# JohnGoertz/Gumbi

Measured on AMD Instinct MI355X. Metric: fit+predict achieved GFLOP/s (fp64 exact GP: one MAP objective + gradient evaluation at the model's starting hyper-parameters + grid prediction), higher is better.
Workload: dtype f64; 1 GPU; synthetic N=50k d=8 Matern-5/2 ARD fp64, M=10^4 grid; N=50000, d=8, kernel=Matern52, M=10000, parallelism=1 GPU, warmup_step=the same step (untimed)

## Files before the change

gumbi_amd/csrc/engine.hip:

```cpp
#include <hip/hip_runtime.h>

#include <algorithm>
#include <cmath>
#include <cstdarg>
#include <cstdio>
#include <cstdlib>
#include <cstring>
#include <string>
#include <functional>
#include <unordered_map>
#include <mutex>
#include <memory>
#include <vector>

#include "../../include/gumbi_hip.h"
#include "covariance.hpp"
#include "gemm_f64.hpp"
#include "gradient.hpp"
#include "potrf_leaf.hpp"
#include "trsm_strip.hpp"
#include "chol_tiles.hpp"
#include "eval_tiles.hpp"
#include "predict_form.hpp"
#include "joint_predict.hpp"

using namespace gmb;

namespace {

constexpr int DIST_MAX_WORLD = 64;
constexpr int DIST_MAX_PAYLOAD = 7;
constexpr int DIST_HEADER = 3;

inline int64_t round_up(int64_t x, int64_t m) { return (x + m - 1) / m * m; }

enum EvKind : int {
  EV_CHOL_PANEL_GEMM = 0,
  EV_LEAF = 1,
  EV_CHOL_SOLVE_GEMM = 2,
  EV_PREDICT_GEMM = 3,
  EV_GRAD_GEMM = 4,
  EV_CHOL_STRIP = 5,
  EV_SOLVE_STRIP = 6,
  EV_CHOL_UPDATE = 7,
  EV_CHOL_TILES = 8,
  EV_EVAL_TILES = 9,
  EV_CHOL_TILES_PANEL = 10
};

struct EventPair {
  hipEvent_t a, b;
  EvKind kind;
  double flops;
  int mt, nt, k, flags;
  bool masked = false;
};

}

constexpr int GACC_REGION = 64 + MAX_TABS * GMB_MAX_LEVELS * GMB_MAX_LEVELS + 64;
constexpr int GACC_DOUBLES = (1 + GMB_MAX_COREG) * GACC_REGION;
constexpr int SCAL_INFO_AT = 64, SCAL_GACC_AT = 72, SCAL_DOUBLES = SCAL_GACC_AT + GACC_DOUBLES + 64;

struct FactorRef {
  double* A;
  int64_t ld;
  int64_t N, Np, Nr;
  double* dinv16;
  double* scal;
  uint32_t** ct;
  int64_t* cap_ct;
  int32_t* info() const { return reinterpret_cast<int32_t*>(scal + SCAL_INFO_AT); }
};

struct CholResult {
  bool tiles = false;
  bool traced = false;
  bool injected = false;
  int ntasks = 0;
};

struct gmb_engine {
  int device = 0;
  hipStream_t stream = nullptr;
  bool own_stream = false;
  std::string err;

  int64_t N = 0, Np = 0, Nr = 0, ld = 0;
  int32_t D = 0;
  double* dX = nullptr;
  double* dy = nullptr;
  double* dA = nullptr;
  double* dDinv16 = nullptr;
  int64_t cap_A = 0, cap_dinv16 = 0;

  gmb_kernel_spec spec{};
  bool have_spec = false, have_theta = false;
  std::vector<double> theta;
  int nc_pad = 1;
  int periodic = 0;
  double periods[8] = {};
  double* xs = nullptr;
  double* xl = nullptr;
  int32_t* cat = nullptr;
  int64_t cap_pts = 0;
  double* dtabs = nullptr;
  double* dnoise = nullptr;
  CovParams cp{};
  PrepArgs prep_proto{};
  struct Term {
    PrepArgs pa;
    CovParams cp;
    double eta;
    int n_tab_acc;
  };
  std::vector<Term> terms;
  std::vector<double> htabs;
  std::vector<double> hnoise;

  double* dscal = nullptr;
  int32_t* dinfo = nullptr;
  double* dv = nullptr;
  bool factored = false;
  enum { FK_NONE = 0, FK_SINGLE = 1, FK_REPLICATED = 2, FK_CAPACITY = 3 };
  int factor_kind = FK_NONE;
  bool factor_consumed = false;
  bool have_alpha = false;
  double* dDiagSave = nullptr;
  int64_t cap_diag = 0;
  int64_t notpd = -1;
  double logdet = 0.0, vnorm2 = 0.0;

  int64_t Mt_cap = 0;
  double* dV = nullptr;
  bool u_valid = false, linv_valid = false;
  int predict_form = -1;
  double* dV2 = nullptr;
  int64_t Mt2_cap = 0;
  JointState jt;
  double* dXs = nullptr;
  double* txs = nullptr;
  double* txl = nullptr;
  int32_t* tcat = nullptr;
  double* dkss = nullptr;
  double* dpart = nullptr;
  double* dmean = nullptr;
  double* dvar = nullptr;
  int64_t cap_part = 0;

  double* dW = nullptr;
  int64_t cap_W = 0;
  double* dalpha = nullptr;
  int64_t cap_pts_alpha = 0;
  double* dgpart = nullptr;
  int64_t cap_gpart = 0;
  double* dgred = nullptr;
  int64_t cap_gred = 0;
  double* dgbig = nullptr;
  int64_t cap_gbig = 0;

  struct InvLevelPlan {
    int variant[2] = {0, 0};
    int grid_x[2] = {0, 0};
    int count = 0;
    int64_t off[2] = {0, 0};
    int64_t toff = 0;
    int tr_rows = 0, tr_cols = 0;
    double flops[2] = {0.0, 0.0};
  };
  std::vector<InvLevelPlan> inv_plan;
  GemmArgs* dplan_gemm = nullptr;
  TransposeJob* dplan_tr = nullptr;
  int64_t plan_N = -1, plan_ld = -1, plan_Np = -1;
  const double* plan_W = nullptr;
  const double* plan_A = nullptr;
  bool batch_inverse = true;
  bool lpt_order = true;
  long long lpt_max_tiles = 16384;
  int cov_strip = 0;
  int tile_strip = 8;

  bool profiling = false;
  gmb_timings tm{};
  std::vector<EventPair> evs;
  bool naive_leaf = false;
  bool gemm_dma = true;
  bool small_tiles = true;
  int gemm_variant = 0;
  long long wg_slots = 512;
  bool force_variant = false;

  hipStream_t cur = nullptr;
  hipStream_t aux[3] = {nullptr, nullptr, nullptr};
  int chol_scheme = -1;
  uint32_t* dct = nullptr;
  int64_t cap_ct = 0;
  unsigned long long* dct_trace = nullptr;
  int64_t cap_ct_trace = 0;
  bool ct_trace = false;
  CholResult chol;
  bool tt_used = false;
  int ct_lose = 0;
  bool fact_in_flight = false;
  struct HostLanding {
    double scal[2];
    int32_t info;
    uint32_t abort;
    double gacc[GACC_DOUBLES];
  };
  HostLanding* hl = nullptr;
  HostLanding* hl_dev = nullptr;
  hipEvent_t fe[4] = {nullptr, nullptr, nullptr, nullptr};
  bool eval_call = false;
  bool light = false;
  bool gacc_zeroed = false;
  unsigned long long* prep_zero[2] = {nullptr, nullptr};
  int64_t prep_zero_words[2] = {0, 0};
  bool prezeroed = false;
  bool prep_deferred = false;
  int inline_prep_max_rows = 4096;
  bool fe_recorded = false;
  int grad_scheme = -1;
  int et_lag = -1;
  uint32_t* det_tasks = nullptr;
  int64_t cap_et_tasks = 0;
  int et_key[5] = {-1, -1, -1, -1, -1};
  int et_pairs = -1;
  int et_pairs_min_blocks = 72;
  int et_ntasks = 0;
  double* dUdiag = nullptr;
  int64_t cap_udiag = 0;
  double* dApart = nullptr;
  int64_t cap_apart = 0;
  bool et_fused = false;
  int et_min_blocks = 1;
  int panel_tiles_w = 16;
  bool panel_tiles_veto = false;
  int tiles_min_blocks = 6, tiles_max_blocks = 224;
  int tiles_trsm_min_blocks = 16;
  int masked_max_blocks = 128;
  std::vector<hipEvent_t> sync_pool;
  size_t sync_next = 0;
  bool lookahead = true;
  bool par_inverse = true;
  bool aux_shared = false;
  bool aux_borrowed = false;
  int part_cus = 0;
  double* dsend = nullptr;
  double* drecv = nullptr;
  int64_t cap_send = 0, cap_recv = 0;
  double* dsend2 = nullptr;
  double* drecv2 = nullptr;
  int64_t cap_send2 = 0, cap_recv2 = 0;
  int panel_blocks = 8;
  bool panel_auto = true;
  std::unordered_map<void*, size_t> allocs;
  int64_t bytes_resident = 0, bytes_peak = 0;
  int dist_mode = 0;
  double* dAown = nullptr;
  int64_t cap_Aown = 0;
  int64_t ld_own = 0;
  int own_world = -1, own_rank = -1;
  double* dPanel = nullptr;
  int64_t cap_panel = 0;
  std::function<int(double*, int64_t, int)> solve_hook;
  double* dstat = nullptr;
  uint64_t coll_count = 0, coll_hash = 0;
  std::vector<hipEvent_t> time_pool;
  size_t time_next = 0;
};

namespace {

int fail(gmb_engine* e, int code, const char* fmt, ...) {
  char buf[512];
  va_list ap;
  va_start(ap, fmt);
  vsnprintf(buf, sizeof buf, fmt, ap);
  va_end(ap);
  if (e) e->err = buf;
  return code;
}

#define HIP_TRY(e, call)                                                              \
  do {                                                                                \
    hipError_t _s = (call);                                                           \
    if (_s != hipSuccess)                                                             \
      return fail(e, GMB_EHIP, "%s failed: %s (%s:%d)", #call, hipGetErrorString(_s), \
                  __FILE__, __LINE__);                                                \
  } while (0)

void release(gmb_engine* e, void* p) {
  if (!p) return;
  if (e) {
    auto it = e->allocs.find(p);
    if (it != e->allocs.end()) {
      e->bytes_resident -= (int64_t)it->second;
      e->allocs.erase(it);
    }
  }
  (void)hipFree(p);
}

template <typename T>
int ensure(gmb_engine* e, T** p, int64_t* cap, int64_t need) {
  if (*cap >= need && *p) return GMB_OK;
  release(e, (void*)*p);
  *p = nullptr;
  *cap = 0;
  if (need < 1) need = 1;
  hipError_t s = hipMalloc((void**)p, (size_t)need * sizeof(T));
  if (s != hipSuccess)
    return fail(e, GMB_ENOMEM, "hipMalloc of %lld bytes failed: %s", (long long)(need * sizeof(T)),
                hipGetErrorString(s));
  *cap = need;
  if (e) {
    e->allocs[(void*)*p] = (size_t)need * sizeof(T);
    e->bytes_resident += (int64_t)((size_t)need * sizeof(T));
    e->bytes_peak = std::max(e->bytes_peak, e->bytes_resident);
  }
  return GMB_OK;
}

template <typename T>
int alloc(gmb_engine* e, T** p, int64_t need) {
  int64_t cap = 0;
  release(e, (void*)*p);
  *p = nullptr;
  return ensure(e, p, &cap, need);
}

int pick_nc(int n) { return n <= 1 ? 1 : n <= 2 ? 2 : n <= 4 ? 4 : n <= 8 ? 8 : 16; }

struct PhaseTimer {
  gmb_engine* e;
  hipEvent_t a = nullptr, b = nullptr;
  explicit PhaseTimer(gmb_engine* e_) : e(e_) {
    (void)hipEventCreate(&a);
    (void)hipEventCreate(&b);
    (void)hipEventRecord(a, e->stream);
  }
  void stop() { (void)hipEventRecord(b, e->stream); }
  double ms() {
    float t = 0.f;
    (void)hipEventElapsedTime(&t, a, b);
    return (double)t;
  }
  ~PhaseTimer() {
    (void)hipEventDestroy(a);
    (void)hipEventDestroy(b);
  }
};

void ev_begin(gmb_engine* e, EvKind kind, double flops, int mt = 0, int nt = 0, int k = 0, int flags = 0) {
  if (!e->profiling) return;
  EventPair p;
  p.mt = mt;
  p.nt = nt;
  p.k = k;
  p.flags = flags;
  (void)hipEventCreate(&p.a);
  (void)hipEventCreate(&p.b);
  p.kind = kind;
  p.flops = flops;
  p.masked = e->aux_shared && e->cur == e->aux[2];
  (void)hipEventRecord(p.a, e->cur);
  e->evs.push_back(p);
}
void ev_end(gmb_engine* e) {
  if (!e->profiling) return;
  (void)hipEventRecord(e->evs.back().b, e->cur);
}
void ev_collect(gmb_engine* e) {
  static FILE* trace = nullptr;
  if (!trace && !e->evs.empty()) {
    const char* path = getenv("GMB_TRACE_FILE");
    if (path && path[0]) trace = fopen(path, "a");
  }
  if (!e->evs.empty()) {
    auto interval_union = [&](auto pick) {
      std::vector<std::pair<float, float>> iv;
      for (auto& p : e->evs)
        if (pick(p.kind)) {
          float ta = 0.f, tb = 0.f;
          if (hipEventElapsedTime(&ta, e->evs[0].a, p.a) == hipSuccess && hipEventElapsedTime(&tb, e->evs[0].a, p.b) == hipSuccess)
            iv.emplace_back(ta, tb);
        }
      std::sort(iv.begin(), iv.end());
      float cur_lo = 0.f, cur_hi = -1.f;
      double uni = 0.0;
// ... 528 lines not shown
  if (c1 - c0 == 1) return chol_leaf(e, f, c0, rend);
  if (tile_panels && c1 - c0 <= e->panel_tiles_w) return chol_tiles_panel(e, f, c0, c1, rend, tile_panels);
  const int mid = c0 + (c1 - c0 + 1) / 2;
  int rc = chol_cols(e, f, c0, mid, rend, update_kind, tile_panels);
  if (rc) return rc;
  GemmArgs g{};
  g.C = f.A + (int64_t)mid * TILE + (int64_t)mid * TILE * f.ld;
  g.ldc = f.ld;
  g.A = f.A + (int64_t)mid * TILE + (int64_t)c0 * TILE * f.ld;
  g.lda = f.ld;
  g.B = g.A;
  g.ldb = f.ld;
  g.mt = c1 - mid;
  g.nt = rend - mid;
  g.k = (mid - c0) * TILE;
  g.alpha = -1.0;
  g.beta = 1.0;
  g.tri = 1;
  rc = launch_gemm(e, g, update_kind);
  if (rc) return rc;
  return chol_cols(e, f, mid, c1, rend, update_kind, tile_panels);
}

double ragged_row_frac(const FactorRef& f) {
  const int64_t rv = f.N + 1 - (f.Nr - TILE);
  return rv >= TILE ? 1.0 : (double)((rv + 15) / 16) / 8.0;
}
double ragged_col_frac(const FactorRef& f) {
  const int64_t cv = f.N - (f.Np - TILE);
  return cv >= TILE ? 1.0 : (double)((cv + 15) / 16) / 8.0;
}
double chol_tiles_flops(const FactorRef& f, int nct, int nrt, bool to_last_row = true) {
  const double fr = to_last_row ? ragged_row_frac(f) : 1.0;
  double flops = 0.0;
  for (int j = 1; j < nct; ++j) {
    const double tiles = nrt - 1 > j ? (double)(nrt - j - 1) + fr : (double)(nrt - j);
    flops += 2.0 * TILE * TILE * TILE * (double)j * tiles;
  }
  return flops;
}

CholTilesArgs tiles_args(const FactorRef& f, int c0, int nct, int nrt, int ntasks, bool chol = true) {
  uint32_t* ct = *f.ct;
  CholTilesArgs a{};
  a.A = f.A + (int64_t)c0 * TILE * (f.ld + 1);
  a.ld = f.ld;
  a.nct = nct;
  a.nrt = nrt;
  a.N = f.N - (int64_t)c0 * TILE;
  a.row_base = (int64_t)c0 * TILE;
  a.dinv16 = f.dinv16 + (int64_t)c0 * 8 * 256;
  a.ctl = ct;
  a.flags = ct + 4;
  if (chol) {
    a.logdet = f.scal;
    a.info = f.info();
    a.half = ct + 4 + (int64_t)nrt * nct;
    a.prog = a.half + 2 * (int64_t)nct;
  }
  a.ntasks = ntasks;
  a.timeout_us = 4000000u;
  return a;
}

int tiles_lose_tickets(gmb_engine* e, uint32_t* ctl, int lose) {
  const uint32_t first = (uint32_t)lose;
  HIP_TRY(e, hipMemcpyAsync(ctl, &first, sizeof first, hipMemcpyHostToDevice, e->cur));
  HIP_TRY(e, hipStreamSynchronize(e->cur));
  return GMB_OK;
}

int tiles_trace_buffer(gmb_engine* e, CholTilesArgs& a) {
  int rc;
  if ((rc = ensure(e, &e->dct_trace, &e->cap_ct_trace, 4 * (int64_t)a.ntasks))) return rc;
  HIP_TRY(e, hipMemsetAsync(e->dct_trace, 0, (size_t)a.ntasks * 4 * sizeof(unsigned long long), e->cur));
  a.dbg = e->dct_trace;
  return GMB_OK;
}

int chol_tiles(gmb_engine* e, const FactorRef& f, bool trace, int lose, CholResult* res) {
  const int nct = (int)(f.Np / TILE), nrt = (int)(f.Nr / TILE);
  const int ntasks = ct_task_count(nct, nrt);
  const int64_t words = 4 + (int64_t)nrt * nct + 3 * (int64_t)nct;
  int rc;
  if ((rc = ensure(e, f.ct, f.cap_ct, words))) return rc;
  HIP_TRY(e, hipMemsetAsync(*f.ct, 0, (size_t)words * sizeof(uint32_t), e->cur));
  res->injected = lose > 0;
  if (lose > 0 && (rc = tiles_lose_tickets(e, *f.ct, lose))) return rc;
  CholTilesArgs a = tiles_args(f, 0, nct, nrt, ntasks);
  res->traced = trace;
  if (trace && (rc = tiles_trace_buffer(e, a))) return rc;
  const double flops = chol_tiles_flops(f, nct, nrt);
  int nw = 8;
#ifdef GMB_TUNING
  if (const char* cw = getenv("GMB_CT_WAVES")) nw = atoi(cw) == 4 ? 4 : 8;
#endif
  int grid = (int)std::min<long long>(ntasks, nw == 8 ? e->wg_slots / 2 : e->wg_slots);
#ifdef GMB_TUNING
  if (const char* cg = getenv("GMB_CT_GRID")) grid = std::max(1, std::min(grid, atoi(cg)));
#endif
  ev_begin(e, EV_CHOL_TILES, flops, nct, nrt, (int)f.Np, 0);
  if (nw == 8) hipLaunchKernelGGL(chol_tiles_kernel<8>, dim3(grid), dim3(512), 0, e->cur, a);
  else hipLaunchKernelGGL(chol_tiles_kernel<4>, dim3(grid), dim3(256), 0, e->cur, a);
  ev_end(e);
  HIP_TRY(e, hipGetLastError());
  res->tiles = true;
  res->ntasks = ntasks;
  return GMB_OK;
}

int chol_tiles_panel(gmb_engine* e, const FactorRef& f, int c0, int c1, int rend, CholResult* res) {
  const int nct = c1 - c0, nrt = rend - c0;
  const int ntasks = ct_task_count(nct, nrt);
  const int64_t words = 4 + (int64_t)nrt * nct + 3 * (int64_t)nct;
  int rc;
  if ((rc = ensure(e, f.ct, f.cap_ct, std::max<int64_t>(words, 4 + (int64_t)(e->panel_tiles_w + 3) * (f.Nr / TILE))))) return rc;
  HIP_TRY(e, hipMemsetAsync(*f.ct, 0, sizeof(uint32_t), e->cur));
  HIP_TRY(e, hipMemsetAsync(*f.ct + 2, 0, (size_t)(words - 2) * sizeof(uint32_t), e->cur));
  const CholTilesArgs a = tiles_args(f, c0, nct, nrt, ntasks);
  const double flops = chol_tiles_flops(f, nct, nrt, rend == (int)(f.Nr / TILE));
  const int grid = (int)std::min<long long>(ntasks, e->wg_slots / 2);
  ev_begin(e, EV_CHOL_TILES_PANEL, flops, nct, nrt, nct * TILE, 0);
  hipLaunchKernelGGL(chol_tiles_kernel<8>, dim3(grid), dim3(512), 0, e->cur, a);
  ev_end(e);
  HIP_TRY(e, hipGetLastError());
  res->tiles = true;
  return GMB_OK;
}

int trsm_tiles(gmb_engine* e, const FactorRef& f, double* V, int64_t ldv, int ntm, EvKind ev_kind) {
  const int nct = (int)(f.Np / TILE);
  const long long ntasks = (long long)ntm * nct;
  if (ntasks <= 0) return GMB_OK;
  const int64_t words = 4 + (int64_t)ntm * nct;
  int rc;
  if ((rc = ensure(e, f.ct, f.cap_ct, words))) return rc;
  HIP_TRY(e, hipMemsetAsync(*f.ct, 0, (size_t)words * sizeof(uint32_t), e->cur));
  CholTilesArgs a = tiles_args(f, 0, nct, nct, (int)ntasks, false);
  a.V = V;
  a.ldv = ldv;
  a.ntm = ntm;
  double flops = 0.0;
  for (int c = 0; c < nct; ++c)
    flops += (double)ntm * (2.0 * TILE * TILE * TILE * c * (c == nct - 1 ? ragged_col_frac(f) : 1.0) + (double)TILE * TILE * TILE);
  const int grid = (int)std::min<long long>(ntasks, e->wg_slots / 2);
  ev_begin(e, ev_kind, flops, nct, ntm, (int)f.Np, 0);
  hipLaunchKernelGGL(trsm_tiles_kernel<8>, dim3(grid), dim3(512), 0, e->cur, a);
  ev_end(e);
  HIP_TRY(e, hipGetLastError());
  e->tt_used = true;
  return GMB_OK;
}

int grad_workspace(gmb_engine* e);
int64_t eval_tiles_words(int nct, int nrt) { return 4 + (int64_t)nrt * nct + 3 * (int64_t)nct + (int64_t)nct * nct + nct; }

bool eval_will_fuse(const gmb_engine* e) {
  const int nblocks = (int)(e->Np / TILE);
  return !e->naive_leaf && (e->chol_scheme == 3 || e->chol_scheme < 0) && e->grad_scheme != 0 && e->grad_scheme != 1 &&
         nblocks <= e->tiles_max_blocks && (e->grad_scheme == 2 ? nblocks >= 1 : nblocks >= e->et_min_blocks);
}

int eval_tiles(gmb_engine* e, bool with_chol) {
  const FactorRef f = train_factor(e);
  const int nct = (int)(e->Np / TILE), nrt = (int)(e->Nr / TILE);
  int rc;
  const int lag = e->et_lag >= 0 ? e->et_lag : std::max(2, std::min(24, nct / 4));
  int nw = 8;
#ifdef GMB_TUNING
  if (const char* cw = getenv("GMB_ET_WAVES")) nw = atoi(cw) == 4 ? 4 : 8;
#endif
  const int pairs = (nw == 8 && !e->ct_trace && (e->et_pairs > 0 || (e->et_pairs < 0 && nct >= e->et_pairs_min_blocks))) ? 1 : 0;
  if (e->et_key[0] != nct || e->et_key[1] != nrt || e->et_key[2] != (int)with_chol || e->et_key[3] != lag || e->et_key[4] != pairs) {
    std::vector<uint32_t> list;
    et_build_tasks(nct, nrt, with_chol, lag, list, pairs != 0);
    if ((rc = ensure(e, &e->det_tasks, &e->cap_et_tasks, (int64_t)list.size()))) return rc;
    HIP_TRY(e, hipMemcpy(e->det_tasks, list.data(), list.size() * sizeof(uint32_t), hipMemcpyHostToDevice));
    e->et_key[0] = nct;
    e->et_key[1] = nrt;
    e->et_key[2] = (int)with_chol;
    e->et_key[3] = lag;
    e->et_key[4] = pairs;
    e->et_ntasks = (int)list.size();
  }
  const int ntasks = e->et_ntasks;
  const int64_t chol_words = (int64_t)nrt * nct + 3 * (int64_t)nct;
  const int64_t words = eval_tiles_words(nct, nrt);
  if ((rc = ensure(e, &e->dct, &e->cap_ct, words + 2))) return rc;
  if ((rc = ensure(e, &e->dW, &e->cap_W, e->Np * e->Np))) return rc;
  e->u_valid = e->linv_valid = false;
  if ((rc = ensure(e, &e->dUdiag, &e->cap_udiag, (int64_t)nct * TILE * TILE))) return rc;
  if ((rc = ensure(e, &e->dApart, &e->cap_apart, (int64_t)nct * nct * TILE + nct))) return rc;
  if ((rc = grad_workspace(e))) return rc;
  if (!(with_chol && e->prezeroed)) HIP_TRY(e, hipMemsetAsync(e->dct, 0, (size_t)words * sizeof(uint32_t), e->cur));
  if (!with_chol) HIP_TRY(e, hipMemsetAsync(e->dct + 4, 1, (size_t)nrt * nct * sizeof(uint32_t), e->cur));
  const int lose = with_chol ? e->ct_lose : 0;
  e->chol.injected = lose > 0;
  if (lose > 0) {
    e->ct_lose = 0;
    if ((rc = tiles_lose_tickets(e, e->dct, lose))) return rc;
  }
  CholTilesArgs a = tiles_args(f, 0, nct, nrt, ntasks);
  e->chol.traced = e->ct_trace;
  if (e->ct_trace && (rc = tiles_trace_buffer(e, a))) return rc;
  EvalTilesArgs x{};
  x.tasks = e->det_tasks;
  x.ntasks = ntasks;
  x.uflags = e->dct + 4 + chol_words;
  x.udiag = e->dUdiag;
  x.Z = e->dW;
  x.ldz = e->Np;
  x.apart = e->dApart;
  x.yb = (int)(e->N / TILE);
  x.rowdone = x.uflags + (int64_t)nct * nct;
  x.alpha = e->dalpha;
  x.v = e->dv;
  x.vpart = e->dApart + (int64_t)nct * nct * TILE;
  x.scal = e->dscal + 1;
  x.with_v = with_chol ? 1 : 0;
  double flops = with_chol ? chol_tiles_flops(f, nct, nrt) : 0.0;
  for (int c = 0; c < nct; ++c)
    flops += 2.0 * TILE * TILE * TILE * 0.5 * (double)c * (double)(c + 1) * (c == nct - 1 ? ragged_col_frac(f) : 1.0);
  for (int I = 0; I < nct; ++I) flops += 2.0 * TILE * TILE * TILE * (double)(nct - I) * (double)(I + 1);
  const int grid = (int)std::min<long long>(ntasks, nw == 8 ? e->wg_slots / 2 : e->wg_slots);
  ev_begin(e, EV_EVAL_TILES, flops, nct, nrt, (int)e->Np, with_chol ? 1 : 0);
  if (nw == 8) hipLaunchKernelGGL(eval_tiles_kernel<8>, dim3(grid), dim3(512), 0, e->cur, a, x);
#ifdef GMB_TUNING
  else hipLaunchKernelGGL(eval_tiles_kernel<4>, dim3(grid), dim3(256), 0, e->cur, a, x);
#endif
  ev_end(e);
  HIP_TRY(e, hipGetLastError());
  e->chol.tiles = true;
  e->chol.ntasks = ntasks;
  return GMB_OK;
}

hipEvent_t next_sync_event(gmb_engine* e) {
  if (e->sync_next == e->sync_pool.size()) {
    hipEvent_t ev = nullptr;
    (void)hipEventCreateWithFlags(&ev, hipEventDisableTiming);
    e->sync_pool.push_back(ev);
  }
  return e->sync_pool[e->sync_next++];
}
hipEvent_t next_time_event(gmb_engine* e) {
  if (e->time_next == e->time_pool.size()) {
    hipEvent_t ev = nullptr;
    (void)hipEventCreate(&ev);
    e->time_pool.push_back(ev);
  }
  return e->time_pool[e->time_next++];
}
int order_after(gmb_engine* e, hipStream_t from, hipStream_t to) {
  if (from == to) return GMB_OK;
  hipEvent_t ev = next_sync_event(e);
  HIP_TRY(e, hipEventRecord(ev, from));
  HIP_TRY(e, hipStreamWaitEvent(to, ev, 0));
  return GMB_OK;
}

int chol_lookahead_masked(gmb_engine* e, const FactorRef& f) {
  const int nct = (int)(f.Np / TILE), nrt = (int)(f.Nr / TILE);
  const int w = e->panel_blocks;
  hipStream_t mainS = e->stream, bulkS = e->aux[2];
  e->sync_next = 0;
  int rc;
  e->cur = mainS;
  if ((rc = chol_cols(e, f, 0, std::min(w, nct), nrt, EV_CHOL_PANEL_GEMM))) return rc;
  for (int c0 = 0; c0 < nct; c0 += w) {
    const int c1 = std::min(c0 + w, nct);
    const int n0 = c1, n1 = std::min(c1 + w, nct);
    if (n0 >= nct) break;
    auto update = [&](int col_lo, int col_hi) {
      GemmArgs g{};
      g.C = f.A + (int64_t)col_lo * TILE + (int64_t)col_lo * TILE * f.ld;
      g.ldc = f.ld;
      g.A = f.A + (int64_t)col_lo * TILE + (int64_t)c0 * TILE * f.ld;
      g.lda = f.ld;
      g.B = g.A;
      g.ldb = f.ld;
      g.mt = col_hi - col_lo;
      g.nt = nrt - col_lo;
      g.k = (c1 - c0) * TILE;
      g.alpha = -1.0;
      g.beta = 1.0;
      g.tri = 1;
      return launch_gemm(e, g, EV_CHOL_UPDATE);
    };
    e->cur = mainS;
    if ((rc = order_after(e, bulkS, mainS))) return rc;
    if ((rc = update(n0, n1))) return rc;
    if ((rc = order_after(e, mainS, bulkS))) return rc;
    e->cur = bulkS;
    rc = (n1 < nct) ? update(n1, nct) : 0;
    e->cur = mainS;
    if (rc) return rc;
    if ((rc = chol_cols(e, f, n0, n1, nrt, EV_CHOL_PANEL_GEMM))) return rc;
  }
  e->cur = mainS;
  return order_after(e, bulkS, mainS);
}

struct CholOpts {
  bool masked_ok = false;
  bool trace = false;
  int lose = 0;
};

int chol_factor(gmb_engine* e, const FactorRef& f, const CholOpts& o, CholResult* res) {
  const int nblocks = (int)(f.Np / TILE), nrt = (int)(f.Nr / TILE);
  const bool tiles = !e->naive_leaf && (e->chol_scheme == 3 || (e->chol_scheme < 0 && nblocks >= e->tiles_min_blocks &&
                                                                 nblocks <= e->tiles_max_blocks));
  const bool masked = o.masked_ok && !tiles && e->lookahead && e->aux_shared && nblocks > e->panel_blocks &&
                      (e->chol_scheme == 2 || (e->chol_scheme < 0 && nblocks <= e->masked_max_blocks));
  e->cur = e->stream;
  if (tiles) return chol_tiles(e, f, o.trace, o.lose, res);
  if (masked) return chol_lookahead_masked(e, f);
  const bool tile_panels = !e->naive_leaf && !e->panel_tiles_veto && e->panel_tiles_w >= 2 && e->chol_scheme != 0;
  if (tile_panels) {
    int rc;
    if ((rc = ensure(e, f.ct, f.cap_ct, 4 + (int64_t)(e->panel_tiles_w + 3) * nrt))) return rc;
    HIP_TRY(e, hipMemsetAsync(*f.ct, 0, 4 * sizeof(uint32_t), e->stream));
  }
  return chol_cols(e, f, 0, nblocks, nrt, EV_CHOL_UPDATE, tile_panels ? res : nullptr);
}

int trsm_cols(gmb_engine* e, const FactorRef& f, double* V, int64_t ldz, int ntm, int c0, int c1, EvKind kind_gemm, EvKind kind_strip,
              int lfirst = -1, int lstride = 0) {
  if (c1 - c0 == 1)
    return launch_trsm_strip(e, V + (int64_t)c0 * TILE * ldz, ldz, (int64_t)ntm * TILE,
                             f.A + (int64_t)c0 * TILE * (f.ld + 1), f.ld, f.dinv16 + (int64_t)c0 * 8 * 256,
                             (int)std::min<int64_t>(TILE, f.N - (int64_t)c0 * TILE), kind_strip);
  const int mid = c0 + (c1 - c0 + 1) / 2;
  int rc = trsm_cols(e, f, V, ldz, ntm, c0, mid, kind_gemm, kind_strip, lfirst, lstride);
  if (rc) return rc;
  GemmArgs g{};
  g.C = V + (int64_t)mid * TILE * ldz;
  g.ldc = ldz;
  g.A = f.A + (int64_t)mid * TILE + (int64_t)c0 * TILE * f.ld;
  g.lda = f.ld;
  g.B = V + (int64_t)c0 * TILE * ldz;
  g.ldb = ldz;
  g.mt = c1 - mid;
  g.nt = ntm;
  g.k = (mid - c0) * TILE;
  g.alpha = -1.0;
  g.beta = 1.0;
  if (lstride > 0) {
    g.klo_n = 1;
    g.krow_stride = lstride;
    g.krow_off = (lfirst - c0) * TILE;
  }
  rc = launch_gemm(e, g, kind_gemm);
  if (rc) return rc;
  return trsm_cols(e, f, V, ldz, ntm, mid, c1, kind_gemm, kind_strip, lfirst, lstride);
}

int launch_transpose(gmb_engine* e, const double* src, int64_t lds_, double* dst, int64_t ldd, int rows,
                     int cols) {
  hipLaunchKernelGGL(transpose_kernel, dim3((rows + 31) / 32, (cols + 31) / 32), dim3(256), 0, e->cur, src,
                     lds_, dst, ldd, rows, cols);
  HIP_TRY(e, hipGetLastError());
  return GMB_OK;
}

int winv_node(gmb_engine* e, int c0, int c1, bool recurse);

int winv_cols(gmb_engine* e, int c0, int c1) { return winv_node(e, c0, c1, true); }

struct InvNode {
  int c0, c1;
};
void collect_inv_nodes(int c0, int c1, int depth, std::vector<std::vector<InvNode>>& levels) {
  if ((int)levels.size() <= depth) levels.resize(depth + 1);
  levels[depth].push_back(InvNode{c0, c1});
  if (c1 - c0 > 1) {
    const int mid = c0 + (c1 - c0 + 1) / 2;
    collect_inv_nodes(c0, mid, depth + 1, levels);
    collect_inv_nodes(mid, c1, depth + 1, levels);
  }
}
int build_inv_plan(gmb_engine* e, const std::vector<std::vector<InvNode>>& levels);
int winv_level_batched(gmb_engine* e, const gmb_engine::InvLevelPlan& lp);

int winv_levels(gmb_engine* e, int nt) {
  std::vector<std::vector<InvNode>> levels;
  collect_inv_nodes(0, nt, 0, levels);
  hipStream_t streams[4] = {e->stream, e->aux[0], e->aux[1], e->aux_shared ? e->aux[0] : e->aux[2]};
  if (nt <= 64) streams[1] = streams[2] = streams[3] = e->stream;
  int rc;
  for (int a = 1; a < 4; ++a)
    if ((rc = order_after(e, streams[0], streams[a]))) return rc;
  const bool batched = e->batch_inverse && build_inv_plan(e, levels) == GMB_OK;
  bool aux_behind = false;
  for (int depth = (int)levels.size() - 1; depth >= 0; --depth) {
    if (batched && e->inv_plan[depth].count > 0) {
      e->cur = e->stream;
      if ((rc = winv_level_batched(e, e->inv_plan[depth]))) return rc;
      aux_behind = true;
      continue;
    }
    if (aux_behind) {
      for (int a = 1; a < 4; ++a)
        if ((rc = order_after(e, streams[0], streams[a]))) return rc;
      aux_behind = false;
    }
    int idx = 0;
    for (const InvNode& nd : levels[depth]) {
      e->cur = streams[levels[depth].size() > 1 ? (idx++ & 3) : 0];
      if ((rc = winv_node(e, nd.c0, nd.c1, false))) {
        e->cur = e->stream;
        return rc;
      }
    }
    e->cur = e->stream;
    for (int a = 1; a < 4; ++a)
      if ((rc = order_after(e, streams[a], streams[0]))) return rc;
    if (depth > 0)
      for (int a = 1; a < 4; ++a)
        if ((rc = order_after(e, streams[0], streams[a]))) return rc;
  }
  return GMB_OK;
}

void winv_node_products(gmb_engine* e, int c0, int c1, GemmArgs& gt, GemmArgs& gw, TransposeJob& tr) {
  const int64_t ldw = e->Np, lda = e->ld;
  double* W = e->dW;
  double* A = e->dA;
  const int mid = c0 + (c1 - c0 + 1) / 2;
  const int n1 = mid - c0, n2 = c1 - mid;
  gt = GemmArgs{};
  gt.C = W + (int64_t)c0 * TILE + (int64_t)mid * TILE * ldw;
  gt.ldc = ldw;
  gt.A = A + (int64_t)mid * TILE + (int64_t)c0 * TILE * lda;
  gt.lda = lda;
  gt.B = A + (int64_t)c0 * TILE + (int64_t)c0 * TILE * lda;
  gt.ldb = lda;
  gt.mt = n2;
  gt.nt = n1;
  gt.k = n1 * TILE;
  gt.klo_n = 1;
  gt.alpha = 1.0;
  gt.beta = 0.0;
  gt.nblk_stride = 1;
  gw = GemmArgs{};
  gw.C = W + (int64_t)mid * TILE + (int64_t)c0 * TILE * ldw;
  gw.ldc = ldw;
  gw.A = W + (int64_t)c0 * TILE + (int64_t)mid * TILE * ldw;
  gw.lda = ldw;
  gw.B = W + (int64_t)mid * TILE + (int64_t)mid * TILE * ldw;
  gw.ldb = ldw;
  gw.mt = n1;
  gw.nt = n2;
  gw.k = n2 * TILE;
  gw.khi_n = 1;
  gw.alpha = -1.0;
  gw.beta = 0.0;
  gw.nblk_stride = 1;
  tr.src = W + (int64_t)mid * TILE + (int64_t)c0 * TILE * ldw;
  tr.dst = A + (int64_t)c0 * TILE + (int64_t)mid * TILE * lda;
  tr.rows = n2 * TILE;
  tr.cols = n1 * TILE;
}

int winv_node(gmb_engine* e, int c0, int c1, bool recurse) {
  if (c1 - c0 == 1) return GMB_OK;
  const int mid = c0 + (c1 - c0 + 1) / 2;
  int rc;
  if (recurse) {
    if ((rc = winv_node(e, c0, mid, true))) return rc;
    if ((rc = winv_node(e, mid, c1, true))) return rc;
  }
  GemmArgs gt, gw;
  TransposeJob tr;
  winv_node_products(e, c0, c1, gt, gw, tr);
  if ((rc = launch_gemm(e, gt, EV_GRAD_GEMM))) return rc;
  if ((rc = launch_gemm(e, gw, EV_GRAD_GEMM))) return rc;
  return launch_transpose(e, tr.src, e->Np, tr.dst, e->ld, tr.rows, tr.cols);
}

constexpr int MIN_BATCH_NODES = 4;

int build_inv_plan(gmb_engine* e, const std::vector<std::vector<InvNode>>& levels) {
  if (e->plan_N == e->N && e->plan_ld == e->ld && e->plan_Np == e->Np && e->plan_W == e->dW && e->plan_A == e->dA)
    return GMB_OK;
  std::vector<GemmArgs> hg;
  std::vector<TransposeJob> ht;
  e->inv_plan.assign(levels.size(), gmb_engine::InvLevelPlan{});
  static const int BMs[3] = {128, 64, 128}, BNs[3] = {128, 64, 64};
  static const double rate[3] = {73.0, 63.0, 65.0};
  static const int per128[3] = {1, 4, 2};
  for (size_t depth = 0; depth < levels.size(); ++depth) {
    std::vector<InvNode> nodes;
    for (const InvNode& nd : levels[depth])
      if (nd.c1 - nd.c0 > 1) nodes.push_back(nd);
    if ((int)nodes.size() < MIN_BATCH_NODES) continue;
    gmb_engine::InvLevelPlan& lp = e->inv_plan[depth];
    lp.count = (int)nodes.size();
    std::vector<GemmArgs> gs[2];
    lp.toff = (int64_t)ht.size();
    for (const InvNode& nd : nodes) {
      GemmArgs gt, gw;
      TransposeJob tr;
      winv_node_products(e, nd.c0, nd.c1, gt, gw, tr);
      gs[0].push_back(gt);
      gs[1].push_back(gw);
      ht.push_back(tr);
      lp.tr_rows = std::max(lp.tr_rows, tr.rows);
      lp.tr_cols = std::max(lp.tr_cols, tr.cols);
    }
    for (int b = 0; b < 2; ++b) {
      long long nact = 0;
      for (const GemmArgs& g : gs[b]) nact += gemm_nact128(g);
      int variant = 0;
      double best = 0.0;
      for (int v = 0; v < 3; ++v) {
        const double t = (double)(nact * per128[v]);
        const double sc = rate[v] * per128[v] / std::max(1.0, t / (double)e->wg_slots + 0.5);
        if (sc > best) {
          best = sc;
          variant = v;
        }
      }
      lp.variant[b] = variant;
      lp.off[b] = (int64_t)hg.size();
      for (GemmArgs g : gs[b]) {
        g.mt = g.mt * TILE / BMs[variant];
        g.nt = g.nt * TILE / BNs[variant];
        g.order = e->lpt_order ? (b == 0 ? 1 : 2) : 0;
        double fl = 0.0;
        const int nb = gemm_schedule(g, BMs[variant], BNs[variant], &fl);
            lp.grid_x[b] = std::max(lp.grid_x[b], nb);
        lp.flops[b] += fl;
        hg.push_back(g);
      }
    }
  }
  if (e->dplan_gemm) (void)hipFree(e->dplan_gemm);
  if (e->dplan_tr) (void)hipFree(e->dplan_tr);
  e->dplan_gemm = nullptr;
  e->dplan_tr = nullptr;
  e->plan_N = -1;
  if (!hg.empty()) {
    HIP_TRY(e, hipMalloc((void**)&e->dplan_gemm, hg.size() * sizeof(GemmArgs)));
    HIP_TRY(e, hipMalloc((void**)&e->dplan_tr, ht.size() * sizeof(TransposeJob)));
    HIP_TRY(e, hipMemcpy(e->dplan_gemm, hg.data(), hg.size() * sizeof(GemmArgs), hipMemcpyHostToDevice));
    HIP_TRY(e, hipMemcpy(e->dplan_tr, ht.data(), ht.size() * sizeof(TransposeJob), hipMemcpyHostToDevice));
  }
  e->plan_N = e->N;
  e->plan_ld = e->ld;
  e->plan_Np = e->Np;
  e->plan_W = e->dW;
  e->plan_A = e->dA;
  return GMB_OK;
}

int winv_level_batched(gmb_engine* e, const gmb_engine::InvLevelPlan& lp) {
  for (int b = 0; b < 2; ++b) {
    if (lp.grid_x[b] <= 0) continue;
    const GemmArgs* batch = e->dplan_gemm + lp.off[b];
    const dim3 grid(lp.grid_x[b], lp.count);
    ev_begin(e, EV_GRAD_GEMM, lp.flops[b], lp.count, 0, 0, (lp.variant[b] << 8) | 64);
    switch (lp.variant[b]) {
      case 0: hipLaunchKernelGGL((gemm_f64_batched_kernel<2, 2, 4, 4, 2>), grid, dim3(256), 0, e->cur, batch); break;
      case 1: hipLaunchKernelGGL((gemm_f64_batched_kernel<2, 2, 2, 2, 2>), grid, dim3(256), 0, e->cur, batch); break;
      default: hipLaunchKernelGGL((gemm_f64_batched_kernel<2, 2, 4, 2, 2>), grid, dim3(256), 0, e->cur, batch); break;
    }
    ev_end(e);
    HIP_TRY(e, hipGetLastError());
  }
  hipLaunchKernelGGL(transpose_batched_kernel, dim3((lp.tr_rows + 31) / 32, (lp.tr_cols + 31) / 32, lp.count),
                     dim3(256), 0, e->cur, e->dplan_tr + lp.toff, e->Np, e->ld);
  HIP_TRY(e, hipGetLastError());
  return GMB_OK;
}

template <int KIND>
int launch_grad_nc(gmb_engine* e, const GradArgs& a_in, int nblocks) {
  const dim3 grid(nblocks), block(256);
  const size_t lds = grad_lds_bytes(e->nc_pad, a_in.p.n_lin, a_in.p.n_tab);
  GradArgs a = a_in;
  a.part_block0 = 0;
  const int gs = a.gsplit > 1 ? a.gsplit : 1;
  const dim3 grid0((a.split ? a.general_tiles : nblocks) * gs);
  switch (e->nc_pad) {
    case 1: hipLaunchKernelGGL((grad_tile_kernel<KIND, 1>), grid0, block, lds, e->stream, a); break;
    case 2: hipLaunchKernelGGL((grad_tile_kernel<KIND, 2>), grid0, block, lds, e->stream, a); break;
    case 4: hipLaunchKernelGGL((grad_tile_kernel<KIND, 4>), grid0, block, lds, e->stream, a); break;
    case 8: hipLaunchKernelGGL((grad_tile_kernel<KIND, 8>), grid0, block, lds, e->stream, a); break;
    default: hipLaunchKernelGGL((grad_tile_kernel<KIND, 16>), grid0, block, lds, e->stream, a); break;
  }
  if constexpr (KIND <= 2) {
    if (a.split) {
      a.part_block0 = a.general_tiles * gs;
      switch (e->nc_pad) {
        case 1: hipLaunchKernelGGL((grad_interior_kernel<KIND, 1>), grid, block, 0, e->stream, a); break;
        case 2: hipLaunchKernelGGL((grad_interior_kernel<KIND, 2>), grid, block, 0, e->stream, a); break;
        case 4: hipLaunchKernelGGL((grad_interior_kernel<KIND, 4>), grid, block, 0, e->stream, a); break;
        case 8: hipLaunchKernelGGL((grad_interior_kernel<KIND, 8>), grid, block, 0, e->stream, a); break;
        default: hipLaunchKernelGGL((grad_interior_kernel<KIND, 16>), grid, block, 0, e->stream, a); break;
      }
    }
  }
  HIP_TRY(e, hipGetLastError());
  return GMB_OK;
}

int grad_workspace(gmb_engine* e) {
  int rc;
  if (e->cap_pts_alpha < 3 * e->Np) {
    if ((rc = alloc(e, &e->dalpha, 3 * e->Np))) return rc;
    e->cap_pts_alpha = 3 * e->Np;
  }
  return GMB_OK;
}

int grad_sigma_inv_rows(gmb_engine* e, int shard, int nshards, double* Z, int64_t ldz, bool packed) {
  const int nt = (int)(e->Np / TILE);
  const int owned = shard < nt ? (nt - shard + nshards - 1) / nshards : 0;
  GemmArgs g{};
  g.C = packed ? Z : Z + (int64_t)shard * TILE;
  g.ldc = ldz;
  g.A = e->dA;
  g.lda = e->ld;
  g.B = e->dA + (int64_t)shard * TILE;
  g.ldb = e->ld;
  g.mt = nt;
  g.nt = owned;
  g.k = (int)e->Np;
  g.klo_n = 1;
  g.krow_off = shard * TILE;
  g.tri = 1;
  g.tri_off = shard * TILE;
  g.nblk_stride = nshards;
  g.cblk_stride = packed ? 1 : 0;
  g.alpha = 1.0;
  g.beta = 0.0;
  return launch_gemm(e, g, EV_GRAD_GEMM);
}

int grad_reduce(gmb_engine* e, int shard, int nshards, const double* Z, int64_t ldz, bool packed,
                std::vector<double>& h) {
  const gmb_kernel_spec& s = e->spec;
  const int nt = (int)(e->Np / TILE);
  int rc;
  if (!e->gacc_zeroed) HIP_TRY(e, hipMemsetAsync(e->dgpart, 0, (GACC_DOUBLES + 64) * sizeof(double), e->stream));
  e->gacc_zeroed = false;
  const int n_ls = s.ard ? s.n_cont : 1;
  long long total = 0;
  for (int i = shard; i < nt; i += nshards) total += i + 1;
  const long long want = std::max<long long>(1, 3 * e->wg_slots);
  const int per = (int)std::max<long long>(1, (total + want - 1) / want);
  const int grid = (int)((total + per - 1) / per);
  const int ncp = e->nc_pad;
  bool merged = false;
  GradFinishArgs fin{};
  for (size_t t = 0; t < e->terms.size(); ++t) {
    const gmb_engine::Term& tr = e->terms[t];
    if (t > 0 && (rc = prep_points(e, e->dX, e->N, e->D, e->Nr, e->xs, e->xl, e->cat, &tr.pa))) return rc;
    GradArgs a{};
    a.p = tr.cp;
    a.pts = train_set(e);
    a.Z = Z;
    a.ldz = ldz;
    a.z_packed = packed ? 1 : 0;
    a.alpha = e->dalpha;
    a.tiles = nt;
    a.ard = s.ard;
    const int ncols = e->periodic ? 2 * s.n_cont : s.n_cont;
    const double true_inv = e->periodic == 2 ? 2.0 : 1.0;
    a.nc_real = ncols;
    for (int k = 0; k < 16; ++k) a.inv_ls[k] = k < ncols ? true_inv * tr.pa.inv_ls[k] : 0.0;
    a.eta = tr.eta;
    a.row_first = shard;
    a.row_stride = nshards;
    a.total_tiles = total;
    a.per = per;
    const int n_small = ncp + 2 + tr.cp.n_lin;
    a.part_stride = n_small + tr.cp.n_tab * 64;
    double* acc = e->dgpart + (int64_t)t * GACC_REGION;
    int tab_acc_off[MAX_TABS] = {0};
    int off = 64, big = 0;
    for (int j = 0; j < tr.cp.n_tab; ++j) {
      tab_acc_off[j] = off;
      const int LL = tr.cp.tab_levels[j] * tr.cp.tab_levels[j];
      off += LL;
      a.big_off[j] = big;
      if (tr.cp.tab_levels[j] > 8) big += LL;
    }
    a.big_stride = big;
    a.split = (tr.cp.kind == GMB_EXPQUAD || tr.cp.kind == GMB_MATERN52 || tr.cp.kind == GMB_MATERN32) && tr.cp.n_lin == 0 &&
                      tr.cp.n_tab == 0 && !e->naive_leaf
                  ? 1 : 0;
    a.n_owned_rows = shard < nt ? (nt - shard + nshards - 1) / nshards : 0;
    const bool last_ragged_owned = e->Np > e->N && (nt - 1 - shard) % nshards == 0 && nt - 1 >= shard;
    a.general_tiles = a.n_owned_rows + (last_ragged_owned ? nt - 1 : 0);
    if (a.general_tiles == 0) a.split = 0;
    if (total <= 128) a.split = 0;
    const int ndirect = a.split ? a.general_tiles : grid;
    a.gsplit = ndirect <= 512 ? 4 : 1;
    const int nvec = a.split ? ndirect * a.gsplit + grid : ndirect * a.gsplit;
    if (grid > 0) {
      if ((rc = ensure(e, &e->dgred, &e->cap_gred, (int64_t)nvec * a.part_stride))) return rc;
      a.part = e->dgred;
      if (big > 0) {
        if ((rc = ensure(e, &e->dgbig, &e->cap_gbig, (int64_t)ndirect * a.gsplit * 4 * big))) return rc;
        HIP_TRY(e, hipMemsetAsync(e->dgbig, 0, (size_t)ndirect * a.gsplit * 4 * big * sizeof(double), e->stream));
        a.big = e->dgbig;
      }
      switch (tr.cp.kind) {
        case GMB_EXPQUAD: rc = launch_grad_nc<0>(e, a, grid); break;
        case GMB_MATERN52: rc = launch_grad_nc<1>(e, a, grid); break;
        case GMB_MATERN32: rc = launch_grad_nc<2>(e, a, grid); break;
        case GMB_MATERN12: rc = launch_grad_nc<3>(e, a, grid); break;
        default: rc = launch_grad_nc<4>(e, a, grid); break;
      }
      if (rc) return rc;
      GradRanges r{};
      auto add = [&](int dense, int count, int dst) {
        r.dense[r.n] = dense;
        r.count[r.n] = count;
        r.dst[r.n] = dst;
        ++r.n;
      };
      double* tmp = e->dgpart + GACC_DOUBLES;
      merged = e->light && e->terms.size() == 1 && s.ard && !e->periodic && big == 0 && nvec <= 8192 && e->N <= 16384;
// ... 238 lines not shown
    const bool is_out = (j == s.n_coreg);
    const int L = is_out ? s.n_out : s.coreg_levels[j];
    std::vector<double> G((size_t)L * L, 0.0);
    if (!s.additive) {
      const double* src = table_slot(0, j);
      for (int i = 0; i < L * L; ++i) G[i] = src[i];
    } else if (!is_out) {
      const double* src = table_slot(1 + j, 0);
      for (int i = 0; i < L * L; ++i) G[i] = src[i];
    } else {
      for (size_t t = 0; t < e->terms.size(); ++t) {
        const double* src = table_slot(t, e->terms[t].cp.n_tab - 1);
        for (int i = 0; i < L * L; ++i) G[i] += src[i];
      }
    }
    table_grad(G, L, th + k, grad + k);
    k += 3 * L;
  }
  int diag_off = 64;
  for (int j = 0; j < e->terms[0].cp.n_tab; ++j) diag_off += e->terms[0].cp.tab_levels[j] * e->terms[0].cp.tab_levels[j];
  const double* hd = region(0) + diag_off;
  grad[i_sigma] = hd[0];
  if (s.out_col >= 0 && s.hetero_noise) {
    const int P = s.n_out;
    const double* W = th + k;
    for (int x = 0; x < P; ++x) {
      const double gd = hd[1 + x];
      grad[k + 2 * x] = 2.0 * gd * W[2 * x];
      grad[k + 2 * x + 1] = 2.0 * gd * W[2 * x + 1];
      grad[k + 2 * P + x] = gd;
    }
    k += 3 * P;
  }
  if (s.additive)
    for (int j = 0; j < s.n_coreg; ++j) {
      k += kernel_block(1 + j, grad + k);
      if (s.n_lin > 0) {
        for (int i = 0; i < s.n_lin; ++i) grad[k++] = region(1 + j)[n_ls + 2 + i];
        grad[k++] = region(1 + j)[n_ls + 1];
      }
    }
  if (k != (int)e->theta.size()) return fail(e, GMB_EINVAL, "internal: gradient packing mismatch");
  return GMB_OK;
}

inline bool chol_scheme_valid(int s) { return s == -1 || s == 0 || s == 2 || s == 3 || s == 4; }

int require_ready(gmb_engine* e, bool need_factor) {
  if (!e) return GMB_EINVAL;
  if (e->N <= 0) return fail(e, GMB_EINVAL, "gmb_set_data has not been called");
  if (!e->have_spec) return fail(e, GMB_EINVAL, "gmb_set_kernel has not been called");
  if (!e->have_theta) return fail(e, GMB_EINVAL, "gmb_set_theta has not been called");
  if (need_factor && !e->factored)
    return fail(e, GMB_EINVAL, "no valid factorisation: call gmb_factorize first");
  return GMB_OK;
}

int require_full_factor(gmb_engine* e, const char* what) {
  if (e->factor_kind == gmb_engine::FK_CAPACITY || !e->dA || e->cap_A <= 0)
    return fail(e, GMB_EINVAL, "%s needs the complete factor on this device, but the resident factorisation is a capacity-mode one "
                               "(gmb_dist_set_mode(e, 1): no rank holds the factor) -- use the gmb_dist_* calls, or gmb_factorize first", what);
  return GMB_OK;
}

int require_capacity_factor(gmb_engine* e, const char* what) {
  if (e->factor_kind != gmb_engine::FK_CAPACITY || !e->dAown)
    return fail(e, GMB_EINVAL, "%s in capacity mode needs a factorisation made by gmb_dist_factorize in capacity mode; the resident "
                               "one was made by %s", what, e->factor_kind == gmb_engine::FK_SINGLE ? "gmb_factorize / gmb_evaluate" : "the replicated multi-GPU driver");
  return GMB_OK;
}

}

namespace {

hipStream_t shared_masked_stream(int device, int part_cus, int* ncu_out) {
  static std::mutex mu;
  static hipStream_t streams[64] = {};
  static int ncus[64] = {};
  std::lock_guard<std::mutex> lock(mu);
  hipStream_t& st = streams[device & 63];
  if (!st) {
    hipDeviceProp_t prop;
    if (hipGetDeviceProperties(&prop, device) != hipSuccess) return nullptr;
    const int ncu = prop.multiProcessorCount;
    std::vector<uint32_t> mask((ncu + 31) / 32, 0u);
    for (int i = part_cus; i < ncu; ++i) mask[i / 32] |= 1u << (i % 32);
    if (hipExtStreamCreateWithCUMask(&st, (uint32_t)mask.size(), mask.data()) != hipSuccess) {
      st = nullptr;
      (void)hipGetLastError();
      return nullptr;
    }
    ncus[device & 63] = ncu;
  }
  if (ncu_out) *ncu_out = ncus[device & 63];
  return st;
}

int gmb_create_impl(gmb_engine** out, int32_t device, void* stream, const gmb_engine* peer = nullptr) {
  if (!out) return GMB_EINVAL;
  *out = nullptr;
  int n = gmb_device_count();
  if (n < 0) return GMB_ENODEVICE;
  if (device < 0 || device >= n) return GMB_EINVAL;
  if (hipSetDevice(device) != hipSuccess) return GMB_EHIP;
  gmb_engine* e = new gmb_engine();
  e->device = device;
  if (stream) {
    e->stream = (hipStream_t)stream;
  } else {
    if (hipStreamCreateWithFlags(&e->stream, hipStreamNonBlocking) != hipSuccess) {
      delete e;
      return GMB_EHIP;
    }
    e->own_stream = true;
  }
  auto flag = [](const char* name, bool dflt) {
    const char* v = getenv(name);
    return v && v[0] ? v[0] != '0' : dflt;
  };
  e->naive_leaf = flag("GMB_LEAF_NAIVE", false);
  e->gemm_dma = flag("GMB_GEMM_DMA", true);
  const char* cs = getenv("GMB_CHOL_SCHEME");
  if (cs && cs[0]) {
    const int v = atoi(cs);
    if (chol_scheme_valid(v)) e->chol_scheme = v;
    else fprintf(stderr, "[gumbi_hip] GMB_CHOL_SCHEME=%s ignored: valid schemes are -1 (by size), 0, 2, 3, 4\n", cs);
  }
  int part = 32;
#ifdef GMB_TUNING
  e->small_tiles = flag("GMB_SMALL_TILES", true);
  const char* gv = getenv("GMB_GEMM_VARIANT");
  if (gv && gv[0] >= '0' && gv[0] <= '4') {
    e->gemm_variant = gv[0] - '0';
    e->force_variant = true;
  }
  e->lookahead = flag("GMB_LOOKAHEAD", true);
  e->lpt_order = flag("GMB_LPT_ORDER", true);
  if (const char* lm = getenv("GMB_LPT_MAX_TILES")) e->lpt_max_tiles = atoll(lm);
  const char* ts = getenv("GMB_TILE_STRIP");
  if (ts) e->tile_strip = std::max(0, atoi(ts));
  const char* cst = getenv("GMB_COV_STRIP");
  if (cst) e->cov_strip = std::max(0, std::min(64, atoi(cst)));
  e->batch_inverse = flag("GMB_BATCH_INVERSE", true);
  e->par_inverse = flag("GMB_PAR_INVERSE", true);
  const char* pb = getenv("GMB_PANEL_BLOCKS");
  if (pb && atoi(pb) > 0) {
    e->panel_blocks = atoi(pb);
    e->panel_auto = false;
  }
  const char* mb = getenv("GMB_MASKED_MAX_BLOCKS");
  if (mb) e->masked_max_blocks = atoi(mb);
  if (const char* pw = getenv("GMB_PANEL_TILES_W")) e->panel_tiles_w = std::max(0, std::min(64, atoi(pw)));
  const char* pc = getenv("GMB_PART_CUS");
  if (pc) part = atoi(pc);
#endif
  e->cur = e->stream;
  int prio_lo = 0, prio_hi = 0;
  (void)hipDeviceGetStreamPriorityRange(&prio_lo, &prio_hi);
  for (int a = 0; a < 3 && peer; ++a) {
    e->aux[a] = peer->aux[a];
    e->aux_borrowed = true;
    e->aux_shared = peer->aux_shared;
    e->part_cus = peer->part_cus;
  }
  for (int a = 0; a < 3 && !peer; ++a) {
    hipError_t st2 = hipSuccess;
    int ncu = 0;
    hipStream_t masked = (a == 2 && part > 0) ? shared_masked_stream(device, part, &ncu) : nullptr;
    if (masked) {
      e->aux[a] = masked;
      e->aux_shared = true;
      e->part_cus = part;
    } else {
      st2 = hipStreamCreateWithPriority(&e->aux[a], hipStreamNonBlocking, a == 2 ? prio_lo : prio_hi);
    }
    if (st2 != hipSuccess) {
      gmb_destroy(e);
      return GMB_EHIP;
    }
  }
  hipDeviceProp_t prop;
  if (hipGetDeviceProperties(&prop, device) == hipSuccess) e->wg_slots = 2LL * prop.multiProcessorCount;
  if (hipMalloc((void**)&e->dscal, (size_t)SCAL_DOUBLES * sizeof(double)) != hipSuccess ||
      hipMalloc((void**)&e->dstat, (size_t)(DIST_HEADER + DIST_MAX_PAYLOAD) * (1 + DIST_MAX_WORLD) * sizeof(double)) != hipSuccess) {
    gmb_destroy(e);
    return GMB_ENOMEM;
  }
  e->dinfo = reinterpret_cast<int32_t*>(e->dscal + SCAL_INFO_AT);
  e->dgpart = e->dscal + SCAL_GACC_AT;
  *out = e;
  return GMB_OK;
}

}

extern "C" {

int gmb_abi_version(void) { return GMB_ABI_VERSION; }

int gmb_device_count(void) {
  int n = 0;
  hipError_t s = hipGetDeviceCount(&n);
  if (s != hipSuccess || n <= 0) return GMB_ENODEVICE;
  return n;
}

int gmb_create(gmb_engine** out, int32_t device, void* stream) { return gmb_create_impl(out, device, stream); }

int gmb_create_sibling(gmb_engine** out, const gmb_engine* peer) {
  if (!peer) return GMB_EINVAL;
  return gmb_create_impl(out, peer->device, (void*)peer->stream, peer);
}

void gmb_destroy(gmb_engine* e) {
  if (!e) return;
  (void)hipSetDevice(e->device);
  if (e->stream) (void)hipStreamSynchronize(e->stream);
  for (int a = 0; a < 3; ++a)
    if (e->aux[a]) (void)hipStreamSynchronize(e->aux[a]);
  void* ptrs[] = {e->dct, e->dct_trace, e->dstat, e->dDiagSave, e->dsend, e->drecv, e->dplan_gemm, e->dplan_tr, e->dDinv16, e->dX, e->dy, e->dA, e->xs, e->xl, e->cat, e->dtabs,
                  e->dnoise, e->dscal, e->dv, e->dV, e->dXs, e->txs, e->txl,
                  e->tcat, e->dkss, e->dpart, e->dmean, e->dvar, e->dW, e->dalpha, e->dgred, e->dgbig, e->det_tasks, e->dUdiag, e->dApart,
                  e->dAown, e->dPanel, e->dV2, e->dsend2, e->drecv2,
                  e->jt.dC, e->jt.dDinv16, e->jt.dscal, e->jt.dct, e->jt.dzero, e->jt.dstage};
  for (void* p : ptrs)
    if (p) (void)hipFree(p);
  for (int a = 0; a < 3; ++a)
    if (e->aux[a] && !e->aux_borrowed && !(a == 2 && e->aux_shared)) (void)hipStreamDestroy(e->aux[a]);
  for (auto ev : e->fe)
    if (ev) (void)hipEventDestroy(ev);
  if (e->hl) (void)hipHostFree(e->hl);
  for (auto ev : e->sync_pool) (void)hipEventDestroy(ev);
  for (auto ev : e->time_pool) (void)hipEventDestroy(ev);
  if (e->own_stream && e->stream) (void)hipStreamDestroy(e->stream);
  delete e;
}

const char* gmb_last_error(const gmb_engine* e) { return e ? e->err.c_str() : "null engine"; }
void* gmb_stream(const gmb_engine* e) { return e ? (void*)e->stream : nullptr; }

int gmb_theta_size(const gmb_kernel_spec* s) {
  if (!s) return GMB_EINVAL;
  int n = (s->ard ? s->n_cont : 1) + 2;
  if (s->n_lin > 0) n += s->n_lin + 1;
  for (int t = 0; t < s->n_coreg; ++t) n += 3 * s->coreg_levels[t];
  if (s->out_col >= 0) {
    n += 3 * s->n_out;
    if (s->hetero_noise) n += 3 * s->n_out;
  }
  if (s->additive) {
    const int blk = (s->ard ? s->n_cont : 1) + 1 + (s->n_lin > 0 ? s->n_lin + 1 : 0);
    n += s->n_coreg * blk;
  }
  return n;
}

int gmb_set_data(gmb_engine* e, const double* X, int64_t N, int32_t D, int64_t ldx, const double* y,
                 int32_t memspace) {
  if (!e) return GMB_EINVAL;
  if (!X || !y || N < 1 || D < 1 || ldx < D) return fail(e, GMB_EINVAL, "bad X/y/N/D/ldx");
  if (e->have_spec) {
    int rc = validate_spec(e, e->spec, D);
    if (rc) return rc;
  }
  HIP_TRY(e, hipSetDevice(e->device));
  e->factored = false;
  e->factor_kind = gmb_engine::FK_NONE;
  e->have_theta = false;
  e->N = 0;
  e->cap_pts = 0;
  e->Mt_cap = 0;
  e->Mt2_cap = 0;
  e->u_valid = e->linv_valid = false;
  e->cap_part = 0;
  e->plan_N = -1;
  e->D = D;
  e->Np = round_up(N, TILE);
  e->Nr = round_up(N + 1, TILE);
  e->ld = e->Nr;
#ifdef GMB_TUNING
  if (const char* lp = getenv("GMB_LD_PAD")) e->ld = e->Nr + atoi(lp);
#endif
  int rc;
  if ((rc = alloc(e, &e->dX, N * (int64_t)D))) return rc;
  if ((rc = alloc(e, &e->dy, e->Np))) return rc;
  if (e->cap_A < e->ld * e->Np && e->dA) {
    release(e, e->dA);
    e->dA = nullptr;
    e->cap_A = 0;
  }
  if ((rc = ensure(e, &e->dDinv16, &e->cap_dinv16, (e->Np / TILE) * (int64_t)8 * 256))) return rc;
  if ((rc = alloc(e, &e->dv, e->Np))) return rc;
  const hipMemcpyKind kind = memspace == GMB_DEVICE ? hipMemcpyDeviceToDevice : hipMemcpyHostToDevice;
  HIP_TRY(e, hipMemcpy2DAsync(e->dX, D * sizeof(double), X, ldx * sizeof(double), D * sizeof(double), N,
                              kind, e->stream));
  HIP_TRY(e, hipMemsetAsync(e->dy, 0, e->Np * sizeof(double), e->stream));
  HIP_TRY(e, hipMemcpyAsync(e->dy, y, N * sizeof(double), kind, e->stream));
  HIP_TRY(e, hipStreamSynchronize(e->stream));
  e->N = N;
  return GMB_OK;
}

int gmb_set_y(gmb_engine* e, const double* y, int32_t memspace) {
  if (!e) return GMB_EINVAL;
  if (e->N <= 0) return fail(e, GMB_EINVAL, "gmb_set_data must precede gmb_set_y");
  if (!y) return fail(e, GMB_EINVAL, "y is null");
  HIP_TRY(e, hipSetDevice(e->device));
  const hipMemcpyKind kind = memspace == GMB_DEVICE ? hipMemcpyDeviceToDevice : hipMemcpyHostToDevice;
  e->factored = false;
  e->factor_kind = gmb_engine::FK_NONE;
  HIP_TRY(e, hipMemcpyAsync(e->dy, y, e->N * sizeof(double), kind, e->stream));
  HIP_TRY(e, hipStreamSynchronize(e->stream));
  return GMB_OK;
}

int gmb_set_kernel(gmb_engine* e, const gmb_kernel_spec* spec) {
  if (!e || !spec) return GMB_EINVAL;
  int rc = validate_spec(e, *spec, e->D);
  if (rc) return rc;
  e->spec = *spec;
  e->have_spec = true;
  e->have_theta = false;
  e->factored = false;
  e->factor_kind = gmb_engine::FK_NONE;
  e->nc_pad = pick_nc(spec->n_cont);
  e->periodic = 0;
  e->cap_pts = 0;
  return GMB_OK;
}

int gmb_set_periodic(gmb_engine* e, int32_t mode, const double* periods, int32_t n) {
  if (!e) return GMB_EINVAL;
  if (!e->have_spec) return fail(e, GMB_EINVAL, "gmb_set_kernel must precede gmb_set_periodic");
  const gmb_kernel_spec& s = e->spec;
  if (mode < 0 || mode > 2) return fail(e, GMB_EINVAL, "gmb_set_periodic: mode %d must be 0 (off), 1 (<kind>+Periodic) or 2 (Periodic)", mode);
  if (n != s.n_cont) return fail(e, GMB_EINVAL, "gmb_set_periodic: %d periods for %d continuous dimensions", n, s.n_cont);
  if (mode != 0) {
    if (s.n_cont > GMB_MAX_DIMS / 2)
      return fail(e, GMB_EINVAL, "gmb_set_periodic: a periodic model has at most %d continuous dimensions (two prepared columns each), got %d",
                  GMB_MAX_DIMS / 2, s.n_cont);
    if (mode == 2 && s.kind != GMB_EXPQUAD) return fail(e, GMB_EINVAL, "gmb_set_periodic: mode 2 (Periodic) needs kind ExpQuad, got %d", s.kind);
    if (!periods) return fail(e, GMB_EINVAL, "gmb_set_periodic: periods is null");
    for (int i = 0; i < n; ++i)
      if (!std::isfinite(periods[i]) || !(periods[i] > 0.0))
        return fail(e, GMB_EINVAL, "gmb_set_periodic: period %d = %g must be finite and positive", i, periods[i]);
  }
  e->periodic = mode;
  for (int i = 0; i < 8; ++i) e->periods[i] = (mode != 0 && i < n) ? periods[i] : 0.0;
  e->nc_pad = pick_nc(mode != 0 ? 2 * s.n_cont : s.n_cont);
  e->have_theta = false;
  e->factored = false;
  e->factor_kind = gmb_engine::FK_NONE;
  e->u_valid = e->linv_valid = false;
  return GMB_OK;
}

int gmb_set_theta(gmb_engine* e, const double* theta, int32_t n) {
  if (!e || !theta) return GMB_EINVAL;
  if (!e->have_spec) return fail(e, GMB_EINVAL, "gmb_set_kernel must precede gmb_set_theta");
  if (e->N <= 0) return fail(e, GMB_EINVAL, "gmb_set_data must precede gmb_set_theta");
  if (n != gmb_theta_size(&e->spec))
    return fail(e, GMB_EINVAL, "theta has %d entries, kernel needs %d", n, gmb_theta_size(&e->spec));
  for (int i = 0; i < n; ++i)
    if (!std::isfinite(theta[i])) return fail(e, GMB_EINVAL, "theta[%d] is not finite", i);
  HIP_TRY(e, hipSetDevice(e->device));
  e->theta.assign(theta, theta + n);
  e->factored = false;
  e->factor_kind = gmb_engine::FK_NONE;
  int rc = apply_theta(e);
  if (rc) return rc;
  if (e->cap_pts < e->Nr) {
    if ((rc = alloc(e, &e->xs, (int64_t)17 * e->Nr))) return rc;
    if ((rc = alloc(e, &e->xl, (int64_t)MAX_LIN * e->Nr))) return rc;
// ... 166 lines not shown
  if (!rc2) rc2 = factorize_finish(e);
  e->chol_scheme = scheme;
  return rc2;
}

int gmb_factorize(gmb_engine* e) {
  int rc = factorize_enqueue(e);
  if (!rc) rc = factorize_retry_after_abort(e, factorize_finish(e));
  return rc;
}

int gmb_evaluate(gmb_engine* e, const double* theta, int32_t n, double* nlml, double* grad) {
  if (!e || !nlml) return GMB_EINVAL;
  e->eval_call = grad != nullptr;
  int rc = gmb_set_theta(e, theta, n);
  if (rc) {
    e->eval_call = false;
    return rc;
  }
  rc = factorize_enqueue(e, grad != nullptr);
  e->eval_call = false;
  e->prezeroed = false;
  if (e->prep_deferred) {
    const int rc2 = flush_deferred_prep(e);
    if (!rc) rc = rc2;
  }
  if (rc) {
    e->light = false;
    return rc;
  }
  int rc_grad = GMB_OK;
  std::vector<double> h;
  if (grad) {
    e->factored = true;
    const bool light = e->light;
    rc_grad = grad_accumulate(e, h);
    e->light = false;
    if (rc_grad && light) {
      (void)hipStreamSynchronize(e->stream);
      e->factored = false;
      e->fact_in_flight = false;
      e->et_fused = false;
      return rc_grad;
    }
  }
  if ((rc = factorize_finish(e))) {
    e->have_alpha = false;
    e->u_valid = e->linv_valid = false;
    e->factor_consumed = false;
    e->et_fused = false;
    if (factorize_retry_after_abort(e, rc) != GMB_OK) return rc;
    rc_grad = grad ? grad_accumulate(e, h) : GMB_OK;
  }
  if (rc_grad) return rc_grad;
  *nlml = 0.5 * (double)e->N * std::log(2.0 * M_PI) + e->logdet + 0.5 * e->vnorm2;
  return grad ? grad_chain_rule(e, h, grad) : GMB_OK;
}

}

namespace {

int64_t predict_tile_rows(const gmb_engine* e, int64_t M) {
  int64_t mt_max = (int64_t)(8.0 * 1024 * 1024 * 1024 / 8.0 / (double)e->Np);
  mt_max = std::max<int64_t>(TILE, std::min<int64_t>(mt_max / TILE * TILE, 32768));
  return std::min<int64_t>(round_up(M, TILE), mt_max);
}

int predict_workspace(gmb_engine* e, int64_t Mt) {
  int rc;
  if (e->Mt_cap < Mt) {
    e->Mt_cap = 0;
    if ((rc = alloc(e, &e->dV, Mt * e->Np))) return rc;
    if ((rc = alloc(e, &e->dXs, Mt * (int64_t)e->D))) return rc;
    if ((rc = alloc(e, &e->txs, (int64_t)17 * Mt))) return rc;
    if ((rc = alloc(e, &e->txl, (int64_t)MAX_LIN * Mt))) return rc;
    if ((rc = alloc(e, &e->tcat, (int64_t)MAX_TABS * Mt))) return rc;
    if ((rc = alloc(e, &e->dkss, Mt))) return rc;
    if ((rc = alloc(e, &e->dmean, Mt))) return rc;
    if ((rc = alloc(e, &e->dvar, Mt))) return rc;
    e->Mt_cap = Mt;
  }
  const int nchunk = (int)((e->N + RED_CHUNK - 1) / RED_CHUNK);
  return ensure(e, &e->dpart, &e->cap_part, (int64_t)2 * nchunk * e->Mt_cap);
}


bool predict_takes_gemm_form(const gmb_engine* e) {
  return !e->solve_hook && e->predict_form != 0 && e->u_valid && e->have_alpha && e->factor_kind == gmb_engine::FK_SINGLE &&
         e->dW && e->dUdiag && e->cap_W >= e->Np * e->Np;
}

int predict_gemm_form_workspace(gmb_engine* e, int64_t Mt) {
  int rc;
  if (e->Mt2_cap < Mt) {
    e->Mt2_cap = 0;
    if ((rc = alloc(e, &e->dV2, Mt * e->Np))) return rc;
    e->Mt2_cap = Mt;
  }
  return GMB_OK;
}

int predict_cross_cov(gmb_engine* e, const double* Xs, int64_t mc, int64_t mpad, int64_t ldxs, int32_t with_noise,
                      hipMemcpyKind in_kind) {
  int rc;
  HIP_TRY(e, hipMemcpy2DAsync(e->dXs, e->D * sizeof(double), Xs, ldxs * sizeof(double),
                              e->D * sizeof(double), mc, in_kind, e->stream));
  if ((rc = prep_points(e, e->dXs, mc, e->D, mpad, e->txs, e->txl, e->tcat))) return rc;
  const PointSet test{e->txs, e->txl, e->tcat, mc, mpad};
  {
    CovTileArgs a{};
    a.p = e->cp;
    a.rows = test;
    a.cols = train_set(e);
    a.out = e->dV;
    a.ldo = mpad;
    a.ti = (int)(mpad / TILE);
    a.tj = (int)(e->Np / TILE);
    a.mode = COV_CROSS;
    if ((rc = launch_cov(e, a))) return rc;
  }
  KssArgs k{};
  k.p = e->cp;
  k.pts = test;
  k.with_noise = with_noise;
  k.kss = e->dkss;
  hipLaunchKernelGGL(kss_kernel, dim3((unsigned)((mpad + 255) / 256)), dim3(256), 0, e->stream, k);
  for (size_t t = 1; t < e->terms.size(); ++t) {
    const gmb_engine::Term& tr = e->terms[t];
    if ((rc = prep_points(e, e->dX, e->N, e->D, e->Nr, e->xs, e->xl, e->cat, &tr.pa))) return rc;
    if ((rc = prep_points(e, e->dXs, mc, e->D, mpad, e->txs, e->txl, e->tcat, &tr.pa))) return rc;
    CovTileArgs a{};
    a.p = tr.cp;
    a.rows = test;
    a.cols = train_set(e);
    a.out = e->dV;
    a.ldo = mpad;
    a.ti = (int)(mpad / TILE);
    a.tj = (int)(e->Np / TILE);
    a.mode = COV_CROSS;
    a.accumulate = 1;
    if ((rc = launch_cov(e, a))) return rc;
    k.p = tr.cp;
    k.with_noise = 0;
    k.accumulate = 1;
    hipLaunchKernelGGL(kss_kernel, dim3((unsigned)((mpad + 255) / 256)), dim3(256), 0, e->stream, k);
  }
  if (e->terms.size() > 1 &&
      (rc = prep_points(e, e->dX, e->N, e->D, e->Nr, e->xs, e->xl, e->cat, &e->terms[0].pa)))
    return rc;
  return GMB_OK;
}

int predict_solve_v(gmb_engine* e, int64_t mpad, bool use_gemm_form) {
  int rc;
  const int nblocks = (int)(e->Np / TILE);
  const int ntm = (int)(mpad / TILE);
  const bool by_size = nblocks >= e->tiles_trsm_min_blocks && nblocks <= e->tiles_max_blocks &&
                       (ntm >= 32 || (long long)ntm * nblocks >= 576);
  const bool tiles = !e->naive_leaf && ntm <= 96 && (e->chol_scheme == 3 || (e->chol_scheme < 0 && by_size));
  e->cur = e->stream;
  e->tt_used = false;
  if (e->solve_hook) {
    if ((rc = e->solve_hook(e->dV, mpad, (int)(mpad / TILE)))) return rc;
  } else if (use_gemm_form) {
    if (!e->linv_valid) {
      LinvArgs la{};
      la.U = e->dA;
      la.ldu = e->ld;
      la.udiag = e->dUdiag;
      la.W = e->dW;
      la.ldw = e->Np;
      la.nct = nblocks;
      hipLaunchKernelGGL(linv_from_u_kernel, dim3((unsigned)((long long)nblocks * (nblocks + 1) / 2)), dim3(256), 0, e->stream, la);
      HIP_TRY(e, hipGetLastError());
      e->linv_valid = true;
    }
    GemmArgs g{};
    g.C = e->dV2;
    g.ldc = e->Np;
    g.A = e->dV;
    g.lda = mpad;
    g.B = e->dW;
    g.ldb = e->Np;
    g.mt = ntm;
    g.nt = nblocks;
    g.k = (int)e->Np;
    g.alpha = 1.0;
    g.beta = 0.0;
    g.khi_n = 1;
    if ((rc = launch_gemm(e, g, EV_PREDICT_GEMM))) return rc;
  } else if ((rc = tiles ? trsm_tiles(e, train_factor(e), e->dV, mpad, (int)(mpad / TILE), EV_PREDICT_GEMM)
                         : trsm_cols(e, train_factor(e), e->dV, mpad, (int)(mpad / TILE), 0, nblocks, EV_PREDICT_GEMM, EV_SOLVE_STRIP)))
    return rc;
  if (e->tt_used) {
    uint32_t ab = 0;
    HIP_TRY(e, hipMemcpyAsync(&ab, e->dct + 1, sizeof(uint32_t), hipMemcpyDeviceToHost, e->stream));
    HIP_TRY(e, hipStreamSynchronize(e->stream));
    if (ab != 0) return fail(e, GMB_EHIP, "tile triangular solve: a workgroup waited longer than its time-out for a tile (launch abandoned)");
  }
  return GMB_OK;
}

int predict_reduce(gmb_engine* e, int64_t mc, int64_t mpad, bool gemm_form) {
  const int nchunk = (int)((e->N + RED_CHUNK - 1) / RED_CHUNK);
  if (gemm_form) {
    hipLaunchKernelGGL(predict_rows_kernel, dim3((unsigned)mc), dim3(256), 0, e->stream, e->dV2, e->Np, e->N, e->dkss, e->dvar);
    hipLaunchKernelGGL(predict_mean_partial_kernel, dim3((unsigned)(mpad / 256 + (mpad % 256 ? 1 : 0)), nchunk),
                       dim3(256), 0, e->stream, e->dV, mpad, e->dalpha, e->N, e->dpart, mpad);
    hipLaunchKernelGGL(predict_mean_final_kernel, dim3((unsigned)((mc + 255) / 256)), dim3(256), 0, e->stream, e->dpart, nchunk,
                       mpad, mc, e->dmean);
    HIP_TRY(e, hipGetLastError());
  } else {
    double* pmu = e->dpart;
    double* ps = e->dpart + (int64_t)nchunk * mpad;
    hipLaunchKernelGGL(predict_partial_kernel, dim3((unsigned)(mpad / 256 + (mpad % 256 ? 1 : 0)), nchunk),
                       dim3(256), 0, e->stream, e->dV, mpad, e->dv, e->N, pmu, ps, mpad);
    hipLaunchKernelGGL(predict_final_kernel, dim3((unsigned)((mc + 255) / 256)), dim3(256), 0, e->stream,
                       pmu, ps, nchunk, mpad, e->dkss, mc, e->dmean, e->dvar);
    HIP_TRY(e, hipGetLastError());
  }
  return GMB_OK;
}


FactorRef joint_factor_ref(JointState& jt) { return FactorRef{jt.dC, jt.Mr, jt.M, jt.Mp, jt.Mr, jt.dDinv16, jt.dscal, &jt.dct, &jt.cap_ct}; }

int joint_ready(gmb_engine* e, const char* what) {
  int rc = require_ready(e, true);
  if (rc) return rc;
  if (e->solve_hook || e->dist_mode != 0 || e->factor_kind != gmb_engine::FK_SINGLE)
    return fail(e, GMB_EINVAL, "%s is not available on distributed engines (gmb_dist_*, capacity mode): factorise with gmb_factorize on one device", what);
  if ((rc = require_full_factor(e, what))) return rc;
  if (e->factor_consumed) return fail(e, GMB_EINVAL, "the factor was consumed by a gradient call: call gmb_factorize again");
  return GMB_OK;
}

int joint_workspace(gmb_engine* e, const char* what, int64_t M, bool gemm_form, double stage) {
  JointState& jt = e->jt;
  const double Mr = (double)round_up(M + 1, TILE), Mp = (double)round_up(M, TILE), Np = (double)e->Np;
  const int nchunk = (int)((e->N + RED_CHUNK - 1) / RED_CHUNK);
  const double per_row = 8.0 * (Np + e->D + 17 + MAX_LIN + 3) + 4.0 * MAX_TABS;
  const double v_bytes = 8.0 * Mr * Np, c_bytes = 8.0 * Mr * Mp, stage_bytes = 8.0 * stage;
  const double total = per_row * Mr + 16.0 * nchunk * Mr + (gemm_form ? v_bytes : 0.0) + c_bytes + stage_bytes;
  double fresh = 0.0;
  if ((double)e->Mt_cap < Mr) fresh += per_row * (Mr - (double)e->Mt_cap);
  if ((double)e->cap_part < 2.0 * nchunk * Mr) fresh += 8.0 * (2.0 * nchunk * Mr - (double)e->cap_part);
  if (gemm_form && (double)e->Mt2_cap < Mr) fresh += 8.0 * Np * (Mr - (double)e->Mt2_cap);
  if ((double)jt.cap_C < Mr * Mp) fresh += 8.0 * (Mr * Mp - (double)jt.cap_C);
  if ((double)jt.cap_stage < stage) fresh += 8.0 * (stage - (double)jt.cap_stage);
  size_t free_b = 0, total_b = 0;
  HIP_TRY(e, hipMemGetInfo(&free_b, &total_b));
  if (fresh > (double)free_b || Mr > 1073741824.0)
    return fail(e, GMB_ENOMEM, "%s: M = %lld behind N = %lld needs %.0f bytes on the device (V: %.0f%s, C: %.0f), %.0f more than it holds "
                               "for the engine now; %.0f bytes are free -- nothing was computed",
                what, (long long)M, (long long)e->N, total, v_bytes, gemm_form ? " twice" : "", c_bytes, fresh, (double)free_b);
  const int64_t mr = round_up(M + 1, TILE), mp = round_up(M, TILE);
  int rc;
  if ((rc = predict_workspace(e, mr))) return rc;
  if (gemm_form && (rc = predict_gemm_form_workspace(e, mr))) return rc;
  if ((rc = ensure(e, &jt.dC, &jt.cap_C, mr * mp))) return rc;
  if ((rc = ensure(e, &jt.dDinv16, &jt.cap_dinv16, (mp / TILE) * (int64_t)8 * 256))) return rc;
  if (!jt.dscal) {
    int64_t cap = 0;
    if ((rc = ensure(e, &jt.dscal, &cap, (int64_t)SCAL_GACC_AT))) return rc;
  }
  if (jt.cap_zero < mr) {
    if ((rc = ensure(e, &jt.dzero, &jt.cap_zero, mr))) return rc;
    HIP_TRY(e, hipMemsetAsync(jt.dzero, 0, (size_t)jt.cap_zero * sizeof(double), e->stream));
  }
  if (stage > 0.0 && (rc = ensure(e, &jt.dstage, &jt.cap_stage, (int64_t)stage))) return rc;
  jt.M = M, jt.Mp = mp, jt.Mr = mr;
  return GMB_OK;
}

int joint_covariance(gmb_engine* e, const double* Xs, int64_t M, int64_t ldxs, int32_t with_noise, double jitter, bool gemm_form,
                     hipMemcpyKind in_kind) {
  JointState& jt = e->jt;
  const int64_t Mr = jt.Mr, Mp = jt.Mp;
  int rc;
  if ((rc = predict_cross_cov(e, Xs, M, Mr, ldxs, with_noise, in_kind))) return rc;
  if ((rc = predict_solve_v(e, Mr, gemm_form))) return rc;
  if ((rc = predict_reduce(e, M, Mr, gemm_form))) return rc;
  if (gemm_form && (rc = launch_transpose(e, e->dV2, e->Np, e->dV, Mr, (int)e->Np, (int)Mr))) return rc;
  if (e->Np > e->N)
    HIP_TRY(e, hipMemsetAsync(e->dV + e->N * Mr, 0, (size_t)((e->Np - e->N) * Mr) * sizeof(double), e->stream));

  const bool additive = e->terms.size() > 1;
  if (additive && (rc = prep_points(e, e->dXs, M, e->D, Mr, e->txs, e->txl, e->tcat, &e->terms[0].pa))) return rc;
  const PointSet test{e->txs, e->txl, e->tcat, M, Mr};
  CovTileArgs a{};
  a.p = e->cp;
  a.p.sigma2 = with_noise ? e->cp.sigma2 : 0.0;
  a.p.jitter = jitter;
  a.rows = test;
  a.cols = test;
  a.out = jt.dC;
  a.ldo = Mr;
  a.ti = (int)(Mr / TILE);
  a.tj = (int)(Mp / TILE);
  a.mode = COV_TRAIN;
  a.lower_only = 1;
  a.tri_grid = 1;
  a.y = jt.dzero;
  if ((rc = launch_cov(e, a))) return rc;
  for (size_t t = 1; t < e->terms.size(); ++t) {
    if ((rc = prep_points(e, e->dXs, M, e->D, Mr, e->txs, e->txl, e->tcat, &e->terms[t].pa))) return rc;
    a.p = e->terms[t].cp;
    a.accumulate = 1;
    if ((rc = launch_cov(e, a))) return rc;
  }

  GemmArgs g{};
  g.C = jt.dC;
  g.ldc = Mr;
  g.A = e->dV;
  g.lda = Mr;
  g.B = e->dV;
  g.ldb = Mr;
  g.mt = (int)(Mp / TILE);
  g.nt = (int)(Mr / TILE);
  g.k = (int)e->Np;
  g.alpha = -1.0;
  g.beta = 1.0;
  g.tri = 1;
  e->cur = e->stream;
  return launch_gemm(e, g, EV_PREDICT_GEMM);
}

int joint_factor(gmb_engine* e) {
  JointState& jt = e->jt;
  HIP_TRY(e, hipMemsetAsync(jt.dscal, 0, (size_t)SCAL_GACC_AT * sizeof(double), e->stream));
  const FactorRef f = joint_factor_ref(jt);
  CholResult res;
  int rc = chol_factor(e, f, CholOpts{}, &res);
  if (rc) return rc;
  int32_t info = 0;
  uint32_t ab = 0;
  HIP_TRY(e, hipMemcpyAsync(&info, f.info(), sizeof info, hipMemcpyDeviceToHost, e->stream));
  if (res.tiles) HIP_TRY(e, hipMemcpyAsync(&ab, jt.dct + 1, sizeof ab, hipMemcpyDeviceToHost, e->stream));
  HIP_TRY(e, hipStreamSynchronize(e->stream));
  if (ab != 0)
    return fail(e, GMB_EHIP, "joint posterior: the tile Cholesky of the predictive covariance waited longer than its time-out for a tile (launch abandoned)");
  if (info != 0) {
    e->notpd = (int64_t)info - 1;
    return fail(e, GMB_ENOTPD, "the posterior covariance of the test points is not positive definite at row %lld (raise the jitter)",
                (long long)e->notpd);
  }
  return GMB_OK;
}

int launch_draw(gmb_engine* e, const DrawArgs& a) {
  const unsigned nrb = (unsigned)((a.M + 15) / 16);
  if (a.S <= 16) hipLaunchKernelGGL(joint_draw_kernel<1>, dim3(nrb, 1), dim3(256), 0, e->stream, a);
  else if (a.S <= 32) hipLaunchKernelGGL(joint_draw_kernel<2>, dim3(nrb, 1), dim3(256), 0, e->stream, a);
  else hipLaunchKernelGGL(joint_draw_kernel<4>, dim3(nrb, (unsigned)((a.S + 63) / 64)), dim3(256), 0, e->stream, a);
  HIP_TRY(e, hipGetLastError());
  return GMB_OK;
}

}

extern "C" {

int gmb_nlml(gmb_engine* e, double* nlml, double* grad) {
  int rc = require_ready(e, true);
  if (rc) return rc;
  if (!nlml) return fail(e, GMB_EINVAL, "nlml output pointer is null");
  *nlml = 0.5 * (double)e->N * std::log(2.0 * M_PI) + e->logdet + 0.5 * e->vnorm2;
  if (grad) {
    if ((rc = require_full_factor(e, "gmb_nlml with a gradient"))) return rc;
    std::vector<double> h;
    if ((rc = grad_accumulate(e, h))) return rc;
    return grad_chain_rule(e, h, grad);
  }
  return GMB_OK;
}

int gmb_predict(gmb_engine* e, const double* Xs, int64_t M, int64_t ldxs, int32_t with_noise,
                double* mean, double* var, int32_t memspace) {
  int rc = require_ready(e, true);
  if (rc) return rc;
  if (M < 0 || (M > 0 && (!Xs || !mean || !var)) || ldxs < e->D)
    return fail(e, GMB_EINVAL, "bad Xs/M/ldxs/mean/var");
  if (M == 0) return GMB_OK;
  if ((rc = e->solve_hook ? require_capacity_factor(e, "gmb_predict") : require_full_factor(e, "gmb_predict"))) return rc;
  if (e->factor_consumed)
    return fail(e, GMB_EINVAL, "the factor was consumed by a gradient call: call gmb_factorize again");
  HIP_TRY(e, hipSetDevice(e->device));
  gmb_timings& tm = e->tm;
  tm.predict_ms = tm.predict_gemm_ms = tm.predict_gemm_flops = 0.0;
  tm.predict_gemm_launches = 0;

  const int64_t Mt = predict_tile_rows(e, M);
  if ((rc = predict_workspace(e, Mt))) return rc;
  const bool use_gemm_form = predict_takes_gemm_form(e);
  if (use_gemm_form && (rc = predict_gemm_form_workspace(e, Mt))) return rc;
  tm.predict_gemm_form = use_gemm_form ? 1 : 0;

  const hipMemcpyKind in_kind = memspace == GMB_DEVICE ? hipMemcpyDeviceToDevice : hipMemcpyHostToDevice;
  const hipMemcpyKind out_kind = memspace == GMB_DEVICE ? hipMemcpyDeviceToDevice : hipMemcpyDeviceToHost;
  PhaseTimer tp(e);
  for (int64_t m0 = 0; m0 < M; m0 += Mt) {
    const int64_t mc = std::min<int64_t>(Mt, M - m0);
    const int64_t mpad = round_up(mc, TILE);
    if ((rc = predict_cross_cov(e, Xs + m0 * ldxs, mc, mpad, ldxs, with_noise, in_kind))) return rc;
    if ((rc = predict_solve_v(e, mpad, use_gemm_form))) return rc;
    if ((rc = predict_reduce(e, mc, mpad, use_gemm_form))) return rc;
    HIP_TRY(e, hipMemcpyAsync(mean + m0, e->dmean, mc * sizeof(double), out_kind, e->stream));
    HIP_TRY(e, hipMemcpyAsync(var + m0, e->dvar, mc * sizeof(double), out_kind, e->stream));
  }
  tp.stop();
  HIP_TRY(e, hipStreamSynchronize(e->stream));
  tm.predict_ms = tp.ms();
  ev_collect(e);
  return GMB_OK;
}

int gmb_predict_joint(gmb_engine* e, const double* Xs, int64_t M, int64_t ldxs, int32_t with_noise, double jitter,
                      double* mean, double* cov, int64_t ldc, int32_t memspace) {
  int rc = joint_ready(e, "gmb_predict_joint");
  if (rc) return rc;
  if (M < 0 || (M > 0 && (!Xs || !mean || !cov)) || ldxs < e->D || ldc < M || !(jitter >= 0.0))
    return fail(e, GMB_EINVAL, "bad Xs/M/ldxs/mean/cov/ldc/jitter");
  if (M == 0) return GMB_OK;
  HIP_TRY(e, hipSetDevice(e->device));
  const bool host = memspace != GMB_DEVICE;
  const bool gemm_form = predict_takes_gemm_form(e);
  if ((rc = joint_workspace(e, "gmb_predict_joint", M, gemm_form, host ? (double)M * (double)M : 0.0))) return rc;
  gmb_timings& tm = e->tm;
  tm.predict_ms = tm.predict_gemm_ms = tm.predict_gemm_flops = 0.0;
  tm.predict_gemm_launches = 0;
  tm.predict_gemm_form = gemm_form ? 1 : 0;
  PhaseTimer tp(e);
  if ((rc = joint_covariance(e, Xs, M, ldxs, with_noise, jitter, gemm_form, host ? hipMemcpyHostToDevice : hipMemcpyDeviceToDevice)))
    return rc;
  SymArgs sa{};
  sa.C = e->jt.dC;
  sa.ldc = e->jt.Mr;
  sa.out = host ? e->jt.dstage : cov;
  sa.ldo = host ? M : ldc;
  sa.M = M;
  const unsigned nb = (unsigned)((M + 31) / 32);
  hipLaunchKernelGGL(joint_symmetrise_kernel, dim3(nb, nb), dim3(256), 0, e->stream, sa);
  HIP_TRY(e, hipGetLastError());
  HIP_TRY(e, hipMemcpyAsync(mean, e->dmean, M * sizeof(double), host ? hipMemcpyDeviceToHost : hipMemcpyDeviceToDevice, e->stream));
  if (host)
    HIP_TRY(e, hipMemcpy2DAsync(cov, ldc * sizeof(double), e->jt.dstage, M * sizeof(double), M * sizeof(double), M,
                                hipMemcpyDeviceToHost, e->stream));
  tp.stop();
  HIP_TRY(e, hipStreamSynchronize(e->stream));
  tm.predict_ms = tp.ms();
  ev_collect(e);
  return GMB_OK;
}

int gmb_draw_joint(gmb_engine* e, const double* Xs, int64_t M, int64_t ldxs, int32_t with_noise, double jitter,
                   const double* Z, int64_t S, int64_t ldz, double* Y, int64_t ldy, double* mean, int32_t memspace) {
  int rc = joint_ready(e, "gmb_draw_joint");
  if (rc) return rc;
  if (M < 0 || S < 0 || S > 0x7fffffff || (M > 0 && S > 0 && (!Xs || !Z || !Y)) || ldxs < e->D || ldz < M || ldy < M || !(jitter >= 0.0))
    return fail(e, GMB_EINVAL, "bad Xs/M/ldxs/Z/S/ldz/Y/ldy/jitter");
  if (M == 0 || S == 0) return GMB_OK;
  HIP_TRY(e, hipSetDevice(e->device));
  const bool host = memspace != GMB_DEVICE;
  const bool gemm_form = predict_takes_gemm_form(e);
  if ((rc = joint_workspace(e, "gmb_draw_joint", M, gemm_form, host ? 2.0 * (double)S * (double)M : 0.0))) return rc;
  gmb_timings& tm = e->tm;
  tm.predict_ms = tm.predict_gemm_ms = tm.predict_gemm_flops = 0.0;
  tm.predict_gemm_launches = 0;
  tm.predict_gemm_form = gemm_form ? 1 : 0;
  PhaseTimer tp(e);
  if ((rc = joint_covariance(e, Xs, M, ldxs, with_noise, jitter, gemm_form, host ? hipMemcpyHostToDevice : hipMemcpyDeviceToDevice)))
    return rc;
  if ((rc = joint_factor(e))) {
    ev_collect(e);
    return rc;
  }
  DrawArgs da{};
  da.L = e->jt.dC;
  da.ldl = e->jt.Mr;
  da.mean = e->dmean;
  da.M = M;
  da.S = (int32_t)S;
  if (host) {
    double* dZ = e->jt.dstage;
    double* dY = e->jt.dstage + S * M;
    HIP_TRY(e, hipMemcpy2DAsync(dZ, M * sizeof(double), Z, ldz * sizeof(double), M * sizeof(double), S, hipMemcpyHostToDevice, e->stream));
    da.Z = dZ, da.ldz = M, da.Y = dY, da.ldy = M;
  } else {
    da.Z = Z, da.ldz = ldz, da.Y = Y, da.ldy = ldy;
  }
  if ((rc = launch_draw(e, da))) return rc;
  if (host)
    HIP_TRY(e, hipMemcpy2DAsync(Y, ldy * sizeof(double), da.Y, M * sizeof(double), M * sizeof(double), S, hipMemcpyDeviceToHost, e->stream));
  if (mean)
    HIP_TRY(e, hipMemcpyAsync(mean, e->dmean, M * sizeof(double), host ? hipMemcpyDeviceToHost : hipMemcpyDeviceToDevice, e->stream));
  tp.stop();
  HIP_TRY(e, hipStreamSynchronize(e->stream));
  tm.predict_ms = tp.ms();
  ev_collect(e);
  return GMB_OK;
}

int gmb_copy_factor(const gmb_engine* ce, int64_t r0, int64_t nr, int64_t c0, int64_t nc, double* out) {
  gmb_engine* e = const_cast<gmb_engine*>(ce);
  if (!e || !out) return GMB_EINVAL;
  if (e->factored && require_full_factor(e, "gmb_copy_factor")) return GMB_EINVAL;
  if (!e->dA || e->cap_A <= 0 || r0 < 0 || c0 < 0 || nr < 0 || nc < 0 || r0 + nr > e->Nr || c0 + nc > e->Np)
    return fail(e, GMB_EINVAL, "factor window out of range");
  if (nr == 0 || nc == 0) return GMB_OK;
  std::vector<double> tmp((size_t)nr * nc);
  HIP_TRY(e, hipMemcpy2D(tmp.data(), nr * sizeof(double), e->dA + r0 + c0 * e->ld, e->ld * sizeof(double),
                         nr * sizeof(double), nc, hipMemcpyDeviceToHost));
  for (int64_t i = 0; i < nr; ++i)
    for (int64_t j = 0; j < nc; ++j) out[i * nc + j] = tmp[(size_t)j * nr + i];
  return GMB_OK;
}

int gmb_copy_v(const gmb_engine* ce, double* out) {
  gmb_engine* e = const_cast<gmb_engine*>(ce);
  int rc = require_ready(e, true);
  if (rc) return rc;
  HIP_TRY(e, hipMemcpy(out, e->dv, e->N * sizeof(double), hipMemcpyDeviceToHost));
  return GMB_OK;
}

int gmb_copy_alpha(const gmb_engine* ce, double* out) {
  gmb_engine* e = const_cast<gmb_engine*>(ce);
  int rc = require_ready(e, false);
  if (rc) return rc;
  if (!out) return fail(e, GMB_EINVAL, "null output");
  if (!e->have_alpha || !e->dalpha)
    return fail(e, GMB_EINVAL, "alpha exists only after a gradient evaluation (gmb_nlml with grad)");
  HIP_TRY(e, hipMemcpy(out, e->dalpha, e->N * sizeof(double), hipMemcpyDeviceToHost));
  return GMB_OK;
}

int gmb_ls_limits(int32_t device, const double* X, int64_t N, int32_t n_cols, int64_t ldx, int32_t ard,
                  double* lower, double* upper) {
  if (!X || !lower || !upper || N < 1 || n_cols < 1 || n_cols > GMB_MAX_DIMS || ldx < n_cols)
    return GMB_EINVAL;
  int nd = gmb_device_count();
  if (nd < 0) return GMB_ENODEVICE;
  if (device < 0 || device >= nd) return GMB_EINVAL;
  if (hipSetDevice(device) != hipSuccess) return GMB_EHIP;
  const int64_t npad = round_up(N, TILE);
  const int ngroups = ard ? n_cols : 1, gw = ard ? 1 : n_cols;
  std::vector<double> soa((size_t)n_cols * npad, 0.0);
  for (int64_t i = 0; i < N; ++i)
    for (int k = 0; k < n_cols; ++k) soa[(size_t)k * npad + i] = X[i * ldx + k];
  double* dpts = nullptr;
  unsigned long long *dmn = nullptr, *dmx = nullptr;
  int rc = GMB_OK;
  std::vector<unsigned long long> hmn(ngroups, ~0ull), hmx(ngroups, 0ull);
  if (hipMalloc((void**)&dpts, soa.size() * sizeof(double)) != hipSuccess ||
      hipMalloc((void**)&dmn, ngroups * sizeof(unsigned long long)) != hipSuccess ||
      hipMalloc((void**)&dmx, ngroups * sizeof(unsigned long long)) != hipSuccess) {
    rc = GMB_ENOMEM;
  } else if (hipMemcpy(dpts, soa.data(), soa.size() * sizeof(double), hipMemcpyHostToDevice) != hipSuccess ||
// ... 35 lines not shown
  if (nd < 0) return GMB_ENODEVICE;
  if (device < 0 || device >= nd) return GMB_EINVAL;
  if (hipSetDevice(device) != hipSuccess) return GMB_EHIP;
  double* sink = nullptr;
  if (hipMalloc((void**)&sink, 16) != hipSuccess) return GMB_ENOMEM;
  hipEvent_t a, b;
  (void)hipEventCreate(&a);
  (void)hipEventCreate(&b);
  const int blocks = 256 * 2;
  hipLaunchKernelGGL(mfma_f64_peak_kernel, dim3(blocks), dim3(256), 0, 0, sink, 100, 1.0);
  const double flops = (double)blocks * 4.0 * (double)iters * 16.0 * 2.0 * 16 * 16 * 4;
  double sum_ms = 0.0, worst_ms = 0.0, sum_mhz = 0.0, sum_cyc = 0.0;
  int64_t n = 0;
  int rc = GMB_OK;
  do {
    (void)hipEventRecord(a, 0);
    hipLaunchKernelGGL(mfma_f64_peak_kernel, dim3(blocks), dim3(256), 0, 0, sink, iters, 1.0);
    (void)hipEventRecord(b, 0);
    if (hipEventSynchronize(b) != hipSuccess || hipGetLastError() != hipSuccess) {
      rc = GMB_EHIP;
      break;
    }
    float ms = 0.f;
    (void)hipEventElapsedTime(&ms, a, b);
    double hsink[2] = {0.0, 0.0};
    if (hipMemcpy(hsink, sink, 16, hipMemcpyDeviceToHost) != hipSuccess) {
      rc = GMB_EHIP;
      break;
    }
    sum_ms += ms;
    worst_ms = std::max(worst_ms, (double)ms);
    sum_mhz += 2.0 * hsink[1] / ((double)ms * 1e3);
    sum_cyc += hsink[1] / ((double)iters * 16.0);
    ++n;
  } while (sum_ms < seconds * 1e3);
  (void)hipEventDestroy(a);
  (void)hipEventDestroy(b);
  (void)hipFree(sink);
  if (rc) return rc;
  if (mean_tf) *mean_tf = flops * (double)n / (sum_ms * 1e-3) / 1e12;
  if (min_tf) *min_tf = flops / (worst_ms * 1e-3) / 1e12;
  if (mhz) *mhz = sum_mhz / (double)n;
  if (cyc_per_mfma) *cyc_per_mfma = sum_cyc / (double)n;
  if (launches) *launches = n;
  return GMB_OK;
}

int gmb_mfma_f64_peak(int32_t device, double* tflops, double* cycles_per_mfma) {
  if (!tflops) return GMB_EINVAL;
  return mfma_f64_run(device, 0.0, 2000, tflops, nullptr, nullptr, cycles_per_mfma, nullptr);
}

int gmb_mfma_f64_sustained(int32_t device, double seconds, double* mean_tflops, double* min_tflops, double* shader_mhz,
                           int64_t* launches) {
  if (!mean_tflops || !(seconds >= 0.0) || seconds > 60.0) return GMB_EINVAL;
  return mfma_f64_run(device, seconds, 40000, mean_tflops, min_tflops, shader_mhz, nullptr, launches);
}

int64_t gmb_debug_tile_list(int32_t mt, int32_t nt, int32_t bm, int32_t bn, int32_t k, int32_t tri, int32_t tri_off,
                            int32_t nblk_stride, int32_t klo_n, int32_t khi_n, int32_t order, int32_t strip,
                            int32_t* out, int64_t cap, int32_t* grid) {
  if (mt < 1 || nt < 1 || k < KT || nblk_stride < 1 || (bm != 128 && bm != 64) || (bn != 128 && bn != 64 && bn != 32))
    return GMB_EINVAL;
  GemmArgs g{};
  g.mt = mt;
  g.nt = nt;
  g.k = k;
  g.tri = tri;
  g.tri_off = tri_off;
  g.nblk_stride = nblk_stride;
  g.klo_n = klo_n;
  g.khi_n = khi_n;
  g.order = order;
  g.strip = order == 0 ? strip : 0;
  double flops = 0.0;
  const int nblocks = gemm_schedule(g, bm, bn, &flops);
  if (grid) *grid = nblocks;
  int64_t n = 0;
  for (int b = 0; b < nblocks; ++b) {
    int tm = -1, tn = -1;
    if (!gemm_decode_tile(g, bm, bn, b, tm, tn)) continue;
    if (out && n < cap) {
      out[3 * n] = b;
      out[3 * n + 1] = tm;
      out[3 * n + 2] = tn;
    }
    ++n;
  }
  return n;
}

int64_t gmb_debug_cov_grid(int32_t ti, int32_t tj, int32_t strip, int32_t tri_grid, int32_t row_first, int32_t row_stride,
                           int32_t keep_order, int32_t* out, int64_t cap, int64_t* grid) {
  if (ti < 1 || tj < 1 || strip < 1 || row_first < 0 || row_stride < 0) return GMB_EINVAL;
  const long long nb = cov_grid_blocks(ti, tj, strip, tri_grid, row_first, row_stride);
  if (grid) *grid = nb;
  int64_t n = 0;
  for (long long b = 0; b < nb; ++b) {
    int tix, lo, hi;
    if (!cov_decode_block(ti, tj, strip, tri_grid, row_first, row_stride, keep_order != 0, b, &tix, &lo, &hi)) continue;
    for (int t = lo; t < hi; ++t) {
      if (out && n < cap) {
        out[3 * n] = (int32_t)b;
        out[3 * n + 1] = tix;
        out[3 * n + 2] = t;
      }
      ++n;
    }
  }
  return n;
}

int64_t gmb_debug_chol_task(int32_t t, int32_t nct, int32_t nrt, int32_t* I, int32_t* J) {
  if (nct < 1 || nrt < nct) return GMB_EINVAL;
  const int n = ct_task_count(nct, nrt);
  int i = -1, j = -1;
  if (t >= 0 && t < n) ct_decode(t, nct, nrt, i, j);
  if (I) *I = i;
  if (J) *J = j;
  return n;
}

int64_t gmb_chol_task_trace(gmb_engine* e, int32_t enable, uint64_t* out, int64_t cap_tasks) {
  if (!e) return GMB_EINVAL;
  if (enable >= 0) e->ct_trace = enable != 0;
  const int64_t n = (e->chol.tiles && e->chol.traced && e->dct_trace && e->cap_ct_trace >= 4 * (int64_t)e->chol.ntasks) ? e->chol.ntasks : 0;
  if (out && n > 0) {
    HIP_TRY(e, hipSetDevice(e->device));
    HIP_TRY(e, hipStreamSynchronize(e->stream));
    HIP_TRY(e, hipMemcpy(out, e->dct_trace, (size_t)std::min<int64_t>(n, cap_tasks) * 4 * sizeof(uint64_t), hipMemcpyDeviceToHost));
  }
  return n;
}

int gmb_debug_chol_lose_tickets(gmb_engine* e, int32_t n) {
  if (!e || n < 0) return GMB_EINVAL;
  e->ct_lose = n;
  return GMB_OK;
}

int gmb_debug_assume_factored(gmb_engine* e) {
  if (!e) return GMB_EINVAL;
  const char* door = getenv("GUMBI_HIP_DEBUG_DOORS");
  if (!door || door[0] != '1') return fail(e, GMB_EINVAL, "gmb_debug_assume_factored needs GUMBI_HIP_DEBUG_DOORS=1 in the environment");
  if (e->factor_kind == gmb_engine::FK_NONE || !e->have_theta) return fail(e, GMB_EINVAL, "no factorisation has been attempted at this theta");
  e->factored = true;
  e->factor_consumed = false;
  e->notpd = -1;
  if (!std::isfinite(e->logdet)) e->logdet = 0.0;
  if (!std::isfinite(e->vnorm2)) e->vnorm2 = 0.0;
  return GMB_OK;
}

int gmb_set_chol_scheme(gmb_engine* e, int32_t scheme) {
  if (!e) return GMB_EINVAL;
  if (!chol_scheme_valid(scheme)) return fail(e, GMB_EINVAL, "Cholesky scheme %d: valid are -1 (by size), 0, 2, 3, 4", scheme);
  const int old = e->chol_scheme;
  e->chol_scheme = scheme;
  return old + 1;
}

int gmb_set_grad_scheme(gmb_engine* e, int32_t scheme, int32_t lag) {
  if (!e || scheme < -1 || scheme > 2) return GMB_EINVAL;
  const int old = e->grad_scheme;
  e->grad_scheme = scheme;
  if (lag >= 0) e->et_lag = lag;
  return old + 1;
}

int gmb_reserve(gmb_engine* e, int32_t gradient, int64_t M) {
  int rc = require_ready(e, false);
  if (rc) return rc;
  if (M < 0) return fail(e, GMB_EINVAL, "M must be >= 0");
  HIP_TRY(e, hipSetDevice(e->device));
  if ((rc = ensure_factor_buffer(e))) return rc;
  if (gradient) {
    if ((rc = ensure(e, &e->dW, &e->cap_W, e->Np * e->Np))) return rc;
    if ((rc = grad_workspace(e))) return rc;
  }
  if (M > 0 && (rc = predict_workspace(e, predict_tile_rows(e, M)))) return rc;
  HIP_TRY(e, hipDeviceSynchronize());
  return GMB_OK;
}

int gmb_set_predict_form(gmb_engine* e, int32_t form) {
  if (!e || form < -1 || form > 1) return GMB_EINVAL;
  const int old = e->predict_form;
  e->predict_form = form;
  return old + 1;
}

int gmb_set_eval_pairs(gmb_engine* e, int32_t mode) {
  if (!e || mode < -1 || mode > 1) return GMB_EINVAL;
  const int old = e->et_pairs;
  e->et_pairs = mode;
  return old + 1;
}

int64_t gmb_debug_eval_tasks(int32_t nct, int32_t nrt, int32_t with_chol, int32_t lag, uint32_t* out, int64_t cap) {
  if (nct < 1 || nrt < nct || nrt > 0x3fff || lag < 0 || with_chol < 0 || with_chol > 3) return GMB_EINVAL;
  std::vector<uint32_t> list;
  et_build_tasks(nct, nrt, (with_chol & 1) != 0, lag, list, (with_chol & 2) != 0);
  if (out)
    for (int64_t i = 0; i < (int64_t)list.size() && i < cap; ++i) out[i] = list[(size_t)i];
  return (int64_t)list.size();
}

int gmb_blk_covariance(gmb_engine* e, double* out, int64_t ldo) {
  int rc = require_ready(e, false);
  if (rc) return rc;
  if (!out || ldo < e->Nr) return fail(e, GMB_EINVAL, "gmb_blk_covariance: out is null or ldo < %lld", (long long)e->Nr);
  if ((((uintptr_t)out) | (uintptr_t)(ldo * (int64_t)sizeof(double))) & 15u)
    return fail(e, GMB_EINVAL, "gmb_blk_covariance: out must be 16-byte aligned and ldo even (16-byte stores)");
  HIP_TRY(e, hipSetDevice(e->device));
  if ((rc = build_sigma(e, out, ldo))) return rc;
  HIP_TRY(e, hipStreamSynchronize(e->stream));
  return GMB_OK;
}

int gmb_blk_potrf(gmb_engine* e, double* Akk, int64_t lda, int32_t nvalid, double* dinv16,
                  double* logdet_accum, int32_t* info) {
  if (!e || !Akk || nvalid < 1 || nvalid > TILE || lda < TILE) return fail(e, GMB_EINVAL, "bad potrf block");
  HIP_TRY(e, hipSetDevice(e->device));
  LeafArgs a{};
  a.A = Akk;
  a.lda = lda;
  a.nvalid = nvalid;
  a.dinv16 = dinv16;
  a.logdet = logdet_accum;
  a.info = info ? info : e->dinfo;
  a.row0 = 0;
#ifdef GMB_TUNING
  a.dbg = getenv("GMB_LEAF_DBG") ? logdet_accum + 1 : nullptr;
#else
  a.dbg = nullptr;
#endif
  return launch_leaf(e, a);
}

int gmb_blk_invert(gmb_engine* e, const double* Lkk, int64_t lda, int32_t nvalid, const double* dinv16,
                   double* invLkk) {
  if (!e || !Lkk || !dinv16 || !invLkk || nvalid < 1 || nvalid > TILE || lda < TILE)
    return fail(e, GMB_EINVAL, "bad invert block");
  HIP_TRY(e, hipSetDevice(e->device));
  InvArgs ia{};
  ia.L = Lkk;
  ia.lda = lda;
  ia.blk_stride = 0;
  ia.dinv16 = dinv16;
  ia.invL = invLkk;
  ia.n = nvalid;
  hipLaunchKernelGGL(leaf_invert_kernel, dim3(1), dim3(256), 0, e->stream, ia);
  HIP_TRY(e, hipGetLastError());
  return GMB_OK;
}

int gmb_blk_trsm(gmb_engine* e, double* B, int64_t ldb, int64_t nrows, const double* Lkk, int64_t ldl,
                 const double* dinv16, int32_t nvalid) {
  if (!e || !B || !Lkk || !dinv16 || nrows < 0 || nrows % 16 || ldb < nrows || ldl < TILE || nvalid < 1 ||
      nvalid > TILE)
    return fail(e, GMB_EINVAL, "bad trsm arguments (rows must be a multiple of 16)");
  HIP_TRY(e, hipSetDevice(e->device));
  return launch_trsm_strip(e, B, ldb, nrows, Lkk, ldl, dinv16, nvalid, EV_CHOL_STRIP);
}

int gmb_blk_gemm_nt(gmb_engine* e, double* C, int64_t ldc, const double* A, int64_t lda, const double* B,
                    int64_t ldb, int64_t m, int64_t n, int64_t k, double alpha, double beta, int32_t tri,
                    int64_t tri_shift) {
  if (!e || !C || !A || !B) return fail(e, GMB_EINVAL, "null gemm operand");
  if (m % TILE || n % TILE || k % KT || m < 0 || n < 0 || k < 0)
    return fail(e, GMB_EINVAL, "gemm sizes must be multiples of 128 (m, n) and 16 (k)");
  HIP_TRY(e, hipSetDevice(e->device));
  GemmArgs g{};
  g.C = C;
  g.ldc = ldc;
  g.A = A;
  g.lda = lda;
  g.B = B;
  g.ldb = ldb;
  g.mt = (int)(m / TILE);
  g.nt = (int)(n / TILE);
  g.k = (int)k;
  g.alpha = alpha;
  g.beta = beta;
  g.tri = tri;
  g.tri_off = (int)(tri_shift * TILE);
  return launch_gemm(e, g, EV_CHOL_PANEL_GEMM);
}

}

#include "dist_driver.hpp"
#include "dist_capacity.hpp"

extern "C" {

int gmb_dist_set_mode(gmb_engine* e, int32_t mode) {
  if (!e || mode < 0 || mode > 1) return GMB_EINVAL;
  const int old = e->dist_mode;
  if (old != mode) {
    e->factored = false;
    e->factor_kind = gmb_engine::FK_NONE;
  }
  e->dist_mode = mode;
  if (mode == 1) {
    if (e->dA && e->cap_A > 0) {
// ... 36 lines not shown
```

gumbi_amd/csrc/gemm_f64.hpp:

```cpp
#pragma once
#include <hip/hip_runtime.h>
#include <algorithm>
#include <stdint.h>

namespace gmb {

typedef double d4 __attribute__((ext_vector_type(4)));
typedef double d2 __attribute__((ext_vector_type(2)));

constexpr int TILE = 128;
constexpr int KT = 16;
constexpr int PITCH = TILE + 16;

struct GemmArgs {
  double* C;
  int64_t ldc;
  const double* A;
  int64_t lda;
  const double* B;
  int64_t ldb;
  int32_t mt, nt;
  int32_t k;
  double alpha, beta;
  int32_t tri;
  int32_t tri_off;
  int32_t nblk_stride;
  int32_t cblk_stride;
  int32_t klo_m, klo_n, khi_n;
  int32_t krow_off;
  int32_t krow_stride;
  int32_t xstart[9];
  int32_t order;
  int32_t strip;
  int32_t xs_t0[8], xs_base[8];
};

__host__ __device__ __forceinline__ int xcd_remap(int bid, int nwg) {
  const int q = nwg >> 3, r = nwg & 7;
  const int xcd = bid & 7, idx = bid >> 3;
  const int base = (xcd < r) ? xcd * (q + 1) : r * (q + 1) + (xcd - r) * q;
  return base + idx;
}

__host__ __device__ __forceinline__ int64_t gemm_noff(int tn, int bn, int stride) {
  const int64_t e = (int64_t)tn * bn;
  return (e >> 7) * stride * 128 + (e & 127);
}
__host__ __device__ __forceinline__ int gemm_first_tn(int64_t T, int bn, int stride) {
  if (T <= 0) return 0;
  const int per = 128 / bn;
  if (T < 0x7fffffff) {
    const uint32_t S = (uint32_t)stride * 128u, t = (uint32_t)T;
    const uint32_t q = t / S, r = t - q * S;
    if (r == 0) return (int)(q * per);
    if (r > (uint32_t)(128 - bn)) return (int)((q + 1) * per);
    return (int)(q * per + (r + bn - 1) / (uint32_t)bn);
  }
  const int64_t S = (int64_t)stride * 128;
  const int64_t q = T / S, r = T % S;
  if (r == 0) return (int)(q * per);
  if (r > 128 - bn) return (int)((q + 1) * per);
  return (int)(q * per + (r + bn - 1) / bn);
}

__host__ __device__ inline bool gemm_decode_tile(const GemmArgs& g, const int BM, const int BN, const int vbid, int& tm,
                                                 int& tn) {
  const int xcd = vbid & 7;
  int ci = g.xstart[xcd] + (vbid >> 3);
  if (g.order == 0 && g.strip > 0) {
    if (ci >= g.xstart[xcd + 1]) return false;
    auto first_of = [&](int t) {
      if (!g.tri) return 0;
      const int f = gemm_first_tn((int64_t)t * BM - g.tri_off - (BN - 1), BN, g.nblk_stride);
      return f > g.nt ? g.nt : f;
    };
    int t0 = g.xs_t0[xcd];
    ci -= g.xs_base[xcd];
    for (;;) {
      const int t1 = t0 + g.strip < g.mt ? t0 + g.strip : g.mt;
      int cnt = 0;
      for (int t = t0; t < t1; ++t) cnt += g.nt - first_of(t);
      if (ci < cnt) break;
      ci -= cnt;
      t0 = t1;
      if (t0 >= g.mt) return false;
    }
    const int t1 = t0 + g.strip < g.mt ? t0 + g.strip : g.mt, sz = t1 - t0;
    const int f_hi = first_of(t1 - 1);
    tn = first_of(t0);
    int have = 1;
    while (tn < f_hi) {
      while (have < sz && first_of(t0 + have) <= tn) ++have;
      if (ci < have) break;
      ci -= have;
      ++tn;
    }
    if (tn >= f_hi) {
      tn += ci / sz;
      ci -= (ci / sz) * sz;
    }
    tm = t0 + ci;
    return true;
  }
  if (g.order == 0) {
    if (ci >= g.xstart[xcd + 1]) return false;
    if (!g.tri) {
      tm = ci / g.nt;
      tn = ci - tm * g.nt;
      return true;
    }
    tm = 0;
    for (;;) {
      int first = gemm_first_tn((int64_t)tm * BM - g.tri_off - (BN - 1), BN, g.nblk_stride);
      first = first > g.nt ? g.nt : first;
      const int cnt = g.nt - first;
      if (ci < cnt) {
        tn = first + ci;
        return true;
      }
      ci -= cnt;
      ++tm;
    }
  }
  ci = vbid;
  const int step = g.order == 1 ? 1 : -1;
  tn = g.order == 1 ? 0 : g.nt - 1;
  for (;;) {
    if (tn < 0 || tn >= g.nt) return false;
    int cnt = g.mt;
    if (g.tri) {
      const int lim = (tn * BN + BN - 1 + g.tri_off) / BM + 1;
      cnt = lim < cnt ? lim : cnt;
    }
    if (ci < cnt) {
      tm = ci;
      return true;
    }
    ci -= cnt;
    tn += step;
  }
}

template <int WGM, int WGN, int WTM, int WTN, bool PFC = false>
__device__ __forceinline__ void gemm_f64_body(const GemmArgs& g, const int vbid) {
  constexpr int NT = 64 * WGM * WGN;
  constexpr int BM = 16 * WTM * WGM, BN = 16 * WTN * WGN;
  constexpr int PA = BM + 16, PB = BN + 16;
  constexpr int LA = BM / 2, RA = NT / LA, NA = KT / RA;
  constexpr int LB_ = BN / 2, RB = NT / LB_, NB = KT / RB;
  static_assert(NA >= 1 && NB >= 1 && NA * RA == KT && NB * RB == KT, "staging must tile the k-tile");
  __shared__ double lds[2][KT * (PA + PB)];

  int tm, tn;
  if (!gemm_decode_tile(g, BM, BN, vbid, tm, tn)) return;

  const int tid = threadIdx.x;
  const int lane = tid & 63;
  const int wave = tid >> 6;
  const int wm = wave / WGN, wn = wave % WGN;
  const int r16 = lane & 15, kq = lane >> 4;

  const int krow = (int)gemm_noff(tn, BN, g.krow_stride > 0 ? g.krow_stride : g.nblk_stride) + g.krow_off;
  int k_lo = g.klo_m * tm * BM + g.klo_n * krow;
  int k_hi = g.k;
  if (g.khi_n) k_hi = min(k_hi, krow + BN);
  if (k_lo < 0) k_lo = 0;
  if (k_lo > k_hi) k_lo = k_hi;

  const int a_row = tid / LA, a_col = 2 * (tid % LA);
  const int b_row = tid / LB_, b_col = 2 * (tid % LB_);
  const double* __restrict__ Ag = g.A + (int64_t)tm * BM + a_col;
  const int64_t noff = gemm_noff(tn, BN, g.nblk_stride);
  const double* __restrict__ Bg = g.B + noff + b_col;

  d4 acc[WTM][WTN];
#pragma unroll
  for (int i = 0; i < WTM; ++i)
#pragma unroll
    for (int j = 0; j < WTN; ++j) acc[i][j] = d4{0.0, 0.0, 0.0, 0.0};

  d2 ra[NA], rb[NB];
  const int kt0 = k_lo / KT, kt1 = k_hi / KT;

  constexpr bool PREFETCH_C = PFC && WTM * WTN <= 8;
  double cpre[PREFETCH_C ? WTM * 4 * WTN : 1];
  const bool prefetch_c = PREFETCH_C && g.beta != 0.0;
  if constexpr (PREFETCH_C) {
    if (prefetch_c) {
      const double* __restrict__ Cp = g.C + (g.cblk_stride > 0 ? gemm_noff(tn, BN, g.cblk_stride) : noff) + wn * (16 * WTN) + r16;
      const int64_t mp = (int64_t)tm * BM + wm * (16 * WTM) + kq;
#pragma unroll
      for (int i = 0; i < WTM; ++i)
#pragma unroll
        for (int r = 0; r < 4; ++r)
#pragma unroll
          for (int j = 0; j < WTN; ++j) cpre[(i * 4 + r) * WTN + j] = Cp[(mp + i * 16 + 4 * r) * g.ldc + j * 16];
    }
  }

  auto gload = [&](int kt) {
#pragma unroll
    for (int p = 0; p < NA; ++p)
      ra[p] = *reinterpret_cast<const d2*>(Ag + ((int64_t)kt * KT + a_row + RA * p) * g.lda);
#pragma unroll
    for (int p = 0; p < NB; ++p)
      rb[p] = *reinterpret_cast<const d2*>(Bg + ((int64_t)kt * KT + b_row + RB * p) * g.ldb);
  };
  auto lstore = [&](int st) {
    double* As = &lds[st][0];
    double* Bs = &lds[st][KT * PA];
#pragma unroll
    for (int p = 0; p < NA; ++p) *reinterpret_cast<d2*>(&As[(a_row + RA * p) * PA + a_col]) = ra[p];
#pragma unroll
    for (int p = 0; p < NB; ++p) *reinterpret_cast<d2*>(&Bs[(b_row + RB * p) * PB + b_col]) = rb[p];
  };

  auto compute = [&](int st) {
    const double* As = &lds[st][0];
    const double* Bs = &lds[st][KT * PA];
#pragma unroll
    for (int k4 = 0; k4 < KT; k4 += 4) {
      double a[WTM], b[WTN];
#pragma unroll
      for (int i = 0; i < WTM; ++i) a[i] = As[(k4 + kq) * PA + wm * (16 * WTM) + i * 16 + r16];
#pragma unroll
      for (int j = 0; j < WTN; ++j) b[j] = Bs[(k4 + kq) * PB + wn * (16 * WTN) + j * 16 + r16];
#pragma unroll
      for (int i = 0; i < WTM; ++i)
#pragma unroll
        for (int j = 0; j < WTN; ++j)
          acc[i][j] = __builtin_amdgcn_mfma_f64_16x16x4f64(a[i], b[j], acc[i][j], 0, 0, 0);
    }
  };

  if (kt0 < kt1) {
    gload(kt0);
    lstore(0);
    __syncthreads();
    int st = 0;
    constexpr int NMFMA = WTM * WTN * (KT / 4), NMEM = NA + NB;
    constexpr int SLOT = NMFMA / (4 * NMEM) > 0 ? NMFMA / (4 * NMEM) : 1;
    static_assert(2 * SLOT * NMEM <= NMFMA, "not enough MFMAs to interleave the staging with");
    for (int kt = kt0; kt + 1 < kt1; ++kt) {
      gload(kt + 1);
      compute(st);
      lstore(st ^ 1);
#pragma unroll
      for (int q = 0; q < NMEM; ++q) {
        __builtin_amdgcn_sched_group_barrier(0x008, SLOT, 0);
        __builtin_amdgcn_sched_group_barrier(0x020, 1, 0);
      }
      __builtin_amdgcn_sched_group_barrier(0x008, NMFMA - 2 * SLOT * NMEM, 0);
#pragma unroll
      for (int q = 0; q < NMEM; ++q) {
        __builtin_amdgcn_sched_group_barrier(0x008, SLOT, 0);
        __builtin_amdgcn_sched_group_barrier(0x200, 1, 0);
      }
      __syncthreads();
      st ^= 1;
    }
    compute(st);
  }


  double* __restrict__ Cg = g.C + (g.cblk_stride > 0 ? gemm_noff(tn, BN, g.cblk_stride) : noff) + wn * (16 * WTN) + r16;
  const int64_t m0 = (int64_t)tm * BM + wm * (16 * WTM) + kq;
  if (g.beta == 0.0) {
#pragma unroll
    for (int i = 0; i < WTM; ++i)
#pragma unroll
      for (int r = 0; r < 4; ++r) {
        double* row = Cg + (m0 + i * 16 + 4 * r) * g.ldc;
#pragma unroll
        for (int j = 0; j < WTN; ++j) row[j * 16] = g.alpha * acc[i][j][r];
      }
  } else {
#pragma unroll
    for (int i = 0; i < WTM; ++i)
#pragma unroll
      for (int r = 0; r < 4; ++r) {
        double* row = Cg + (m0 + i * 16 + 4 * r) * g.ldc;
        double c[WTN];
#pragma unroll
        for (int j = 0; j < WTN; ++j) {
          if constexpr (PREFETCH_C) c[j] = prefetch_c ? cpre[(i * 4 + r) * WTN + j] : row[j * 16];
          else c[j] = row[j * 16];
        }
#pragma unroll
        for (int j = 0; j < WTN; ++j) row[j * 16] = g.beta * c[j] + g.alpha * acc[i][j][r];
      }
  }
}

template <bool DUMMY = false>
__device__ __forceinline__ void gemm_f64_dma_body(const GemmArgs& g, const int vbid) {
  constexpr int WGN = 2, WTM = 4, WTN = 4;
  constexpr int BM = 128, BN = 128, PA = BM + 16, PB = BN + 16;
  constexpr int KD = 8, NS = 4;
  constexpr int STAGE = KD * (PA + PB);
  typedef __attribute__((address_space(3))) double lds_double;
  typedef __attribute__((address_space(3))) void lds_void;
  typedef const __attribute__((address_space(1))) void g_void;
  __shared__ __attribute__((aligned(16))) double lds_[NS * STAGE];
  lds_double* const lds = (lds_double*)lds_;

  int tm, tn;
  if (!gemm_decode_tile(g, BM, BN, vbid, tm, tn)) return;
  const int tid = threadIdx.x;
  const int lane = tid & 63;
  const int wave = __builtin_amdgcn_readfirstlane(tid >> 6);
  const int wm = wave / WGN, wn = wave % WGN;
  const int r16 = lane & 15, kq = lane >> 4;

  const int krow = (int)gemm_noff(tn, BN, g.krow_stride > 0 ? g.krow_stride : g.nblk_stride) + g.krow_off;
  int k_lo = g.klo_m * tm * BM + g.klo_n * krow;
  int k_hi = g.k;
  if (g.khi_n) k_hi = min(k_hi, krow + BN);
  if (k_lo < 0) k_lo = 0;
  if (k_lo > k_hi) k_lo = k_hi;
  const int64_t noff = gemm_noff(tn, BN, g.nblk_stride);
  const int kt0 = k_lo / KD, kt1 = k_hi / KD;

  d4 acc[WTM][WTN];
#pragma unroll
  for (int i = 0; i < WTM; ++i)
#pragma unroll
    for (int j = 0; j < WTN; ++j) acc[i][j] = d4{0.0, 0.0, 0.0, 0.0};

  const double* pa = g.A + (int64_t)tm * BM + ((int64_t)kt0 * KD + wave) * g.lda;
  const double* pb = g.B + noff + ((int64_t)kt0 * KD + wave) * g.ldb;
  const int lane2 = 2 * lane;
  int issued = kt0;
  auto dma = [&](const int stage) {
    lds_double* As = lds + stage * STAGE + wave * PA;
    lds_double* Bs = lds + stage * STAGE + KD * PA + wave * PB;
    __builtin_amdgcn_global_load_lds((g_void*)(pa + lane2), (lds_void*)As, 16, 0, 0);
    __builtin_amdgcn_global_load_lds((g_void*)(pb + lane2), (lds_void*)Bs, 16, 0, 0);
    __builtin_amdgcn_global_load_lds((g_void*)(pa + 4 * g.lda + lane2), (lds_void*)(As + 4 * PA), 16, 0, 0);
    __builtin_amdgcn_global_load_lds((g_void*)(pb + 4 * g.ldb + lane2), (lds_void*)(Bs + 4 * PB), 16, 0, 0);
    if (issued + 1 < kt1) {
      pa += (int64_t)KD * g.lda;
      pb += (int64_t)KD * g.ldb;
      ++issued;
    }
  };
  double fa[2][WTM], fb[2][WTN];
  auto frags = [&](const int kt, const int k4, const int buf) {
    const lds_double* As = lds + (kt & (NS - 1)) * STAGE + (4 * k4 + kq) * PA + r16;
    const lds_double* Bs = lds + (kt & (NS - 1)) * STAGE + KD * PA + (4 * k4 + kq) * PB + r16;
#pragma unroll
    for (int i = 0; i < WTM; ++i) fa[buf][i] = As[wm * (16 * WTM) + i * 16];
#pragma unroll
    for (int j = 0; j < WTN; ++j) fb[buf][j] = Bs[wn * (16 * WTN) + j * 16];
  };
  auto mfmas = [&](const int buf) {
#pragma unroll
    for (int i = 0; i < WTM; ++i)
#pragma unroll
      for (int j = 0; j < WTN; ++j) acc[i][j] = __builtin_amdgcn_mfma_f64_16x16x4f64(fa[buf][i], fb[buf][j], acc[i][j], 0, 0, 0);
  };
  auto pin_step = [&]() {
#pragma unroll
    for (int q = 0; q < 4; ++q) {
      __builtin_amdgcn_sched_group_barrier(0x008, 2, 0);
      __builtin_amdgcn_sched_group_barrier(0x100, 1, 0);
    }
    __builtin_amdgcn_sched_group_barrier(0x008, WTM * WTN - 8, 0);
  };

  if (kt0 < kt1) {
    dma(kt0 & (NS - 1));
    dma((kt0 + 1) & (NS - 1));
    dma((kt0 + 2) & (NS - 1));
    dma((kt0 + 3) & (NS - 1));
    asm volatile("s_waitcnt vmcnt(12)" ::: "memory");
    __builtin_amdgcn_s_barrier();
    frags(kt0, 0, 0);
    for (int kt = kt0; kt < kt1; ++kt) {
      frags(kt, 1, 1);
      mfmas(0);
      pin_step();
      asm volatile("s_waitcnt vmcnt(8) lgkmcnt(0)" ::: "memory");
      __builtin_amdgcn_s_barrier();
      dma(kt & (NS - 1));
      frags(kt + 1, 0, 0);
      mfmas(1);
      pin_step();
    }
    asm volatile("s_waitcnt vmcnt(0)" ::: "memory");
  }

  double* __restrict__ Cg = g.C + (g.cblk_stride > 0 ? gemm_noff(tn, BN, g.cblk_stride) : noff) + wn * (16 * WTN) + r16;
  const int64_t m0 = (int64_t)tm * BM + wm * (16 * WTM) + kq;
  if (g.beta == 0.0) {
#pragma unroll
    for (int i = 0; i < WTM; ++i)
#pragma unroll
      for (int r = 0; r < 4; ++r) {
        double* row = Cg + (m0 + i * 16 + 4 * r) * g.ldc;
#pragma unroll
        for (int j = 0; j < WTN; ++j) row[j * 16] = g.alpha * acc[i][j][r];
      }
  } else {
#pragma unroll
    for (int i = 0; i < WTM; ++i)
#pragma unroll
      for (int r = 0; r < 4; ++r) {
        double* row = Cg + (m0 + i * 16 + 4 * r) * g.ldc;
        double c[WTN];
#pragma unroll
        for (int j = 0; j < WTN; ++j) c[j] = row[j * 16];
#pragma unroll
        for (int j = 0; j < WTN; ++j) row[j * 16] = g.beta * c[j] + g.alpha * acc[i][j][r];
      }
  }
}

__global__ __launch_bounds__(256, 2) void gemm_f64_dma_kernel(GemmArgs g) {
  gemm_f64_dma_body<>(g, blockIdx.x);
}

__global__ __launch_bounds__(256, 2) void gemm_f64_dma_chol_update_kernel(GemmArgs g) {
  gemm_f64_dma_body<>(g, blockIdx.x);
}

template <int WGM, int WGN, int WTM, int WTN, int OCC, bool PFC = false>
__global__ __launch_bounds__(64 * WGM * WGN, OCC) void gemm_f64_kernel(GemmArgs g) {
  gemm_f64_body<WGM, WGN, WTM, WTN, PFC>(g, blockIdx.x);
}

template <int WGM, int WGN, int WTM, int WTN, int OCC>
__global__ __launch_bounds__(64 * WGM * WGN, OCC) void gemm_f64_batched_kernel(const GemmArgs* __restrict__ batch) {
  const GemmArgs g = batch[blockIdx.y];
  gemm_f64_body<WGM, WGN, WTM, WTN>(g, blockIdx.x);
}

__global__ __launch_bounds__(256, 2) void mfma_f64_peak_kernel(double* sink, int iters, double scale) {
  d4 acc[4][4];
#pragma unroll
  for (int i = 0; i < 4; ++i)
#pragma unroll
    for (int j = 0; j < 4; ++j) acc[i][j] = d4{0.0, 0.0, 0.0, 0.0};
  double a[4], b[4];
#pragma unroll
  for (int i = 0; i < 4; ++i) {
    a[i] = scale * (1.0 + 1e-9 * (threadIdx.x + i));
    b[i] = scale * (1.0 - 1e-9 * (threadIdx.x + 7 * i));
  }
  const long long t0 = __builtin_readcyclecounter();
  for (int it = 0; it < iters; ++it) {
#pragma unroll
    for (int i = 0; i < 4; ++i)
#pragma unroll
      for (int j = 0; j < 4; ++j)
        acc[i][j] = __builtin_amdgcn_mfma_f64_16x16x4f64(a[i], b[j], acc[i][j], 0, 0, 0);
  }
  double s = 0.0;
#pragma unroll
  for (int i = 0; i < 4; ++i)
#pragma unroll
    for (int j = 0; j < 4; ++j) s += acc[i][j][0] + acc[i][j][1] + acc[i][j][2] + acc[i][j][3];
  const long long t1 = __builtin_readcyclecounter();
  if (s == 12345.678) sink[0] = s;
  if (blockIdx.x == 0 && threadIdx.x == 0) sink[1] = (double)(t1 - t0);
}

inline int gemm_schedule(GemmArgs& g, int bm, int bn, double* flops) {
  const int KU = g.k / KT;
  auto first_of = [&](int tm) {
    if (!g.tri) return 0;
    const int f = gemm_first_tn((int64_t)tm * bm - g.tri_off - (bn - 1), bn, g.nblk_stride);
    return f > g.nt ? g.nt : f;
  };
  auto kunits = [&](int tm, int tn) {
    const int kstride = g.krow_stride > 0 ? g.krow_stride : (g.nblk_stride < 1 ? 1 : g.nblk_stride);
    const int krow = (int)gemm_noff(tn, bn, kstride) + g.krow_off;
    const int lo = std::max(0, g.klo_m * tm * bm + g.klo_n * krow) / KT;
    int hi = KU;
    if (g.khi_n && (krow + bn) / KT < hi) hi = (krow + bn) / KT;
    return hi > lo ? hi - lo : 0;
  };
  if (g.order != 0) {
    long long nact = 0, funits = 0;
    for (int tn = 0; tn < g.nt; ++tn) {
      long long cnt = g.mt;
      if (g.tri) cnt = std::min<long long>(cnt, ((long long)tn * bn + bn - 1 + g.tri_off) / bm + 1);
      nact += cnt;
      funits += cnt * kunits(0, tn);
    }
    if (flops) *flops = 2.0 * bm * bn * KT * (double)funits;
    for (int i = 0; i <= 8; ++i) g.xstart[i] = 0;
    return (int)nact;
  }
  static thread_local long long* P = nullptr;
  static thread_local long long* F = nullptr;
  static thread_local int cap = 0;
  if (cap < g.nt + 1) {
    delete[] P;
    delete[] F;
    cap = g.nt + 1;
    P = new long long[cap];
    F = new long long[cap];
  }
  const int fixed = 4;
  P[0] = F[0] = 0;
  for (int tn = 0; tn < g.nt; ++tn) {
    const int w = kunits(0, tn);
    P[tn + 1] = P[tn] + w + fixed;
    F[tn + 1] = F[tn] + w;
  }
  long long total = 0, funits = 0, nact = 0;
  for (int tm = 0; tm < g.mt; ++tm) {
    const int f = first_of(tm);
    total += P[g.nt] - P[f];
    funits += F[g.nt] - F[f];
    nact += g.nt - f;
  }
  if (g.klo_m) {
    funits = 0;
    for (int tm = 0; tm < g.mt; ++tm)
      for (int tn = first_of(tm); tn < g.nt; ++tn) funits += kunits(tm, tn);
  }
  if (flops) *flops = 2.0 * bm * bn * KT * (double)funits;
  if (g.strip > 0) {
    g.xstart[0] = 0;
    for (int i = 0; i < 8; ++i) g.xs_t0[i] = g.xs_base[i] = 0;
    long long acc = 0, ci = 0;
    int x = 1;
    for (int t0 = 0; t0 < g.mt && x < 8; t0 += g.strip) {
      const int t1 = std::min(t0 + g.strip, g.mt), sz = t1 - t0;
      long long sw = 0, sc = 0;
      for (int t = t0; t < t1; ++t) {
        const int f = first_of(t);
        sw += P[g.nt] - P[f];
        sc += g.nt - f;
      }
      if ((acc + sw) * 8 >= (long long)x * total) {
        long long a2 = acc, c2 = ci;
        int have = 1;
        for (int tn = first_of(t0); tn < g.nt && x < 8; ++tn) {
          while (have < sz && first_of(t0 + have) <= tn) ++have;
          const long long w1 = P[tn + 1] - P[tn];
          for (int q = 0; q < have && x < 8; ++q) {
            if ((a2 + w1) * 8 >= (long long)x * total) {
              g.xs_t0[x] = t0;
              g.xs_base[x] = (int)ci;
              g.xstart[x++] = (int)(c2 + 1);
            }
            a2 += w1;
            ++c2;
          }
        }
      }
      acc += sw;
      ci += sc;
// ... 40 lines not shown
```

gumbi_amd/csrc/gradient.hpp:

```cpp
#pragma once
#include <hip/hip_runtime.h>
#include <stdint.h>

#include "covariance.hpp"

namespace gmb {

struct GradArgs {
  CovParams p;
  PointSet pts;
  const double* Z;
  int64_t ldz;
  const double* alpha;
  int32_t tiles;
  int32_t ard;
  int32_t nc_real;
  double inv_ls[16];
  double eta;
  double* part;
  int32_t part_stride;
  int64_t total_tiles;
  int32_t per;
  double* big;
  int32_t big_stride;
// ... 503 lines not shown
  int tix = a.row_first + m * a.row_stride;
  int tjx = (int)(tile - before(m));
  while (tile < t_end) {
    const long long left_in_row = (long long)(tix - tjx + 1);
    const long long nseg = left_in_row < t_end - tile ? left_in_row : t_end - tile;
    const int tj1 = (int)(tjx + nseg) < tix ? (int)(tjx + nseg) : tix;
    if (tjx < tj1 && (int64_t)(tix + 1) * TILE <= a.pts.n) grad_interior_segment<KIND, NC>(a, tix, tjx, tj1, lds, g_ls2, g_eta2);
    tile += nseg;
    tjx += (int)nseg;
    if (tjx > tix) {
      tix += a.row_stride;
      tjx = 0;
    }
  }
  auto wave_sum = [&](double v) {
#pragma unroll
    for (int off = 32; off > 0; off >>= 1) v += __shfl_down(v, off);
    return v;
  };
#pragma unroll
  for (int k = 0; k < NC; ++k) {
    const double v = wave_sum(-2.0 * a.inv_ls[k] * g_ls2[k]);
    if ((tid & 63) == 0) swave[wave][k] = v;
  }
  {
    const double v = wave_sum((2.0 / a.eta) * g_eta2);
    if ((tid & 63) == 0) {
      swave[wave][NC] = v;
      swave[wave][NC + 1] = 0.0;
    }
  }
  __syncthreads();
  double* out = a.part + ((int64_t)a.part_block0 + blockIdx.x) * a.part_stride;
  if (tid < NC + 2) out[tid] = (swave[0][tid] + swave[1][tid]) + (swave[2][tid] + swave[3][tid]);
}

struct GradRanges {
  int32_t n;
  int32_t dense[MAX_TABS + 2], count[MAX_TABS + 2], dst[MAX_TABS + 2];
};
__global__ __launch_bounds__(256) void grad_sum_partials_kernel(const double* __restrict__ part, int nparts, int64_t stride,
                                                                GradRanges r, double* __restrict__ acc) {
  __shared__ double red[256];
  const int q = blockIdx.x;
  double s = 0.0;
  for (int b = threadIdx.x; b < nparts; b += 256) s += part[(int64_t)b * stride + q];
  red[threadIdx.x] = s;
  __syncthreads();
  for (int h = 128; h > 0; h >>= 1) {
    if ((int)threadIdx.x < h) red[threadIdx.x] += red[threadIdx.x + h];
    __syncthreads();
  }
  if (threadIdx.x != 0) return;
  for (int i = 0; i < r.n; ++i)
    if (q >= r.dense[i] && q < r.dense[i] + r.count[i]) {
      acc[r.dst[i] + (q - r.dense[i])] = red[0];
      return;
    }
}
__global__ void grad_fold_ls_kernel(double* acc, int n, const double* tmp) {
  if (threadIdx.x || blockIdx.x) return;
  double s = 0.0;
  for (int k = 0; k < n; ++k) s += tmp[k];
  acc[0] = s;
}

__global__ void grad_fold_periodic_kernel(double* acc, int n, int ard, const double* tmp) {
  if (threadIdx.x || blockIdx.x) return;
  double s = 0.0;
  for (int d = 0; d < n; ++d) {
    const double p = tmp[2 * d] + tmp[2 * d + 1];
    if (ard) acc[d] = p;
    else s += p;
  }
  if (!ard) acc[0] = s;
}

__global__ __launch_bounds__(1024) void grad_diag_kernel(const double* Z, int64_t ldz,
                                                         const double* alpha, PointSet pts,
                                                         CovParams p, double sigma, double* out, int row_first,
                                                         int row_stride, int z_packed = 0) {
  __shared__ double red[16];
  __shared__ double tab[16][32];
  const int wave = threadIdx.x >> 6;
  for (int idx = threadIdx.x; idx < 16 * 32; idx += 1024) (&tab[0][0])[idx] = 0.0;
  __syncthreads();
  double gs = 0.0;
  for (int64_t i = threadIdx.x; i < pts.n; i += 1024) {
    if ((int)((i >> 7) % row_stride) != row_first) continue;
    const double a = alpha[i];
    const int64_t zr = z_packed ? (((i >> 7) - row_first) / row_stride) * TILE + (i & 127) : i;
    const double m = 0.5 * (Z[zr + i * ldz] - a * a);
    double mult = 1.0;
    if (p.noise_tab >= 0) {
      const int c = pts.cat[(int64_t)p.noise_tab * pts.npad + i];
      mult = p.noise_mult[c];
      atomicAdd(&tab[wave][c], m * sigma * sigma);
    }
    gs = fma(m, 2.0 * sigma * mult, gs);
  }
#pragma unroll
  for (int off = 32; off > 0; off >>= 1) gs += __shfl_down(gs, off);
  if ((threadIdx.x & 63) == 0) red[wave] = gs;
  __syncthreads();
  if (threadIdx.x == 0) {
    double s = 0.0;
    for (int w = 0; w < 16; ++w) s += red[w];
    out[0] = s;
  }
  if (p.noise_tab >= 0 && threadIdx.x < 32) {
    double s = 0.0;
    for (int w = 0; w < 16; ++w) s += tab[w][threadIdx.x];
    out[1 + threadIdx.x] = s;
  }
}

__global__ void reset_pad_rows_kernel(double* W, int64_t ld, int64_t n, int64_t npad) {
  const int64_t c = (int64_t)blockIdx.x * blockDim.x + threadIdx.x;
  if (c >= npad) return;
  for (int64_t r = n; r < npad; ++r) W[r + c * ld] = (r == c) ? 1.0 : 0.0;
}

__global__ __launch_bounds__(256) void transpose_kernel(const double* __restrict__ src, int64_t lds_,
                                                        double* __restrict__ dst, int64_t ldd, int rows,
                                                        int cols) {
  __shared__ double tile[32][33];
  const int r0 = blockIdx.x * 32, c0 = blockIdx.y * 32;
  const int tx = threadIdx.x & 31, ty = threadIdx.x >> 5;
  for (int j = ty; j < 32; j += 8)
    if (r0 + tx < rows && c0 + j < cols) tile[j][tx] = src[(r0 + tx) + (int64_t)(c0 + j) * lds_];
  __syncthreads();
  for (int j = ty; j < 32; j += 8)
    if (c0 + tx < cols && r0 + j < rows) dst[(c0 + tx) + (int64_t)(r0 + j) * ldd] = tile[tx][j];
}

__global__ void identity_rows_kernel(double* V, int64_t ldv, int first, int stride) {
  const int t = blockIdx.x, i = threadIdx.x;
  const int64_t col = ((int64_t)first + (int64_t)t * stride) * TILE + i;
  V[(int64_t)t * TILE + i + col * ldv] = 1.0;
}
__global__ __launch_bounds__(256) void urows_v_kernel(const double* __restrict__ V, int64_t ldv,
                                                      const double* __restrict__ v, int64_t n,
                                                      double* __restrict__ alpha_rows) {
  __shared__ double part[4][64];
  const int r = threadIdx.x & 63, ph = threadIdx.x >> 6;
  const int64_t row = (int64_t)blockIdx.x * 64 + r;
  double s = 0.0;
  for (int64_t k = ph; k < n; k += 4) s = fma(V[row + k * ldv], v[k], s);
  part[ph][r] = s;
  __syncthreads();
  if (ph == 0) alpha_rows[row] = (part[0][r] + part[1][r]) + (part[2][r] + part[3][r]);
}

struct TransposeJob {
  const double* src;
  double* dst;
  int32_t rows, cols;
};
__global__ __launch_bounds__(256) void transpose_batched_kernel(const TransposeJob* __restrict__ jobs, int64_t lds_,
                                                                int64_t ldd) {
  __shared__ double tile[32][33];
  const TransposeJob jb = jobs[blockIdx.z];
  const int r0 = blockIdx.x * 32, c0 = blockIdx.y * 32;
  if (r0 >= jb.rows || c0 >= jb.cols) return;
  const int tx = threadIdx.x & 31, ty = threadIdx.x >> 5;
  for (int j = ty; j < 32; j += 8)
    if (r0 + tx < jb.rows && c0 + j < jb.cols) tile[j][tx] = jb.src[(r0 + tx) + (int64_t)(c0 + j) * lds_];
  __syncthreads();
  for (int j = ty; j < 32; j += 8)
    if (c0 + tx < jb.cols && r0 + j < jb.rows) jb.dst[(c0 + tx) + (int64_t)(r0 + j) * ldd] = tile[tx][j];
}

__global__ void reset_pad_cols_kernel(double* U, int64_t ld, int64_t n, int64_t npad) {
  const int64_t i = (int64_t)blockIdx.x * blockDim.x + threadIdx.x;
  if (i >= npad) return;
  for (int64_t k = n; k < npad; ++k) U[i + k * ld] = (i == k) ? 1.0 : 0.0;
}

struct PackArgs {
  double* mat;
  int64_t ld;
  double* packed;
  int64_t ldp;
  int64_t seg_elems;
  int32_t ncols;
  int32_t to_packed;
  int32_t nseg;
  int32_t by_rank;
  int32_t first, count, stride;
  int32_t lo, hi;
};
__global__ __launch_bounds__(256) void pack_rows_kernel(PackArgs a) {
  const int seg = blockIdx.z;
  int first = a.first, count = a.count;
  if (a.by_rank) {
    const int G = a.stride;
    first = a.lo + (((seg - a.lo) % G) + G) % G;
    count = first < a.hi ? (a.hi - first + G - 1) / G : 0;
  }
  const int t = blockIdx.x;
  if (t >= count) return;
  const int c = blockIdx.y * 4 + (threadIdx.x >> 6);
  if (c >= a.ncols) return;
  const int r = (threadIdx.x & 63) * 2;
  double* m = a.mat + ((int64_t)first + (int64_t)t * a.stride) * 128 + r + (int64_t)c * a.ld;
  double* q = a.packed + (int64_t)seg * a.seg_elems + (int64_t)t * 128 + r + (int64_t)c * a.ldp;
  typedef double pk_d2 __attribute__((ext_vector_type(2)));
  if (a.to_packed) *reinterpret_cast<pk_d2*>(q) = *reinterpret_cast<const pk_d2*>(m);
  else *reinterpret_cast<pk_d2*>(m) = *reinterpret_cast<const pk_d2*>(q);
}

__global__ __launch_bounds__(256) void diag_blocks_copy_kernel(double* __restrict__ A, int64_t ld,
                                                               double* __restrict__ save, int to_save) {
  double* blk = A + (int64_t)blockIdx.x * 128 * (ld + 1);
  double* sv = save + (int64_t)blockIdx.x * 128 * 128;
  typedef double dg_d2 __attribute__((ext_vector_type(2)));
  const int r = (threadIdx.x & 63) * 2, c0 = threadIdx.x >> 6;
  for (int c = c0; c < 128; c += 4) {
    dg_d2* m = reinterpret_cast<dg_d2*>(blk + r + (int64_t)c * ld);
    dg_d2* q = reinterpret_cast<dg_d2*>(sv + r + c * 128);
    if (to_save) *q = *m;
    else *m = *q;
  }
}

__global__ __launch_bounds__(256) void wt_v_kernel(const double* W, int64_t ld, const double* v,
                                                   int64_t n, double* alpha) {
  const int wave = threadIdx.x >> 6, lane = threadIdx.x & 63;
  const int64_t j = (int64_t)blockIdx.x * 4 + wave;
  if (j >= n) return;
  const double* col = W + j * ld;
  double s = 0.0;
  for (int64_t k = j + lane; k < n; k += 64) s = fma(col[k], v[k], s);
#pragma unroll
  for (int off = 32; off > 0; off >>= 1) s += __shfl_down(s, off);
  if (lane == 0) alpha[j] = s;
}



struct TriOperand {
  const double* A;
  int64_t ld;
  const double* diag;
  int64_t ldd;
  int64_t dstride;
};

__device__ __forceinline__ double tri_at(const TriOperand& o, int64_t i, int64_t j) {
  const int64_t bi = i >> 7;
  return bi == (j >> 7) ? o.diag[bi * o.dstride + (i & 127) + (j & 127) * o.ldd] : o.A[i + j * o.ld];
}

__global__ __launch_bounds__(256) void lt_residual_kernel(TriOperand L, const double* __restrict__ v,
                                                          const double* __restrict__ alpha, int64_t n, double* __restrict__ t) {
  const int wave = threadIdx.x >> 6, lane = threadIdx.x & 63;
  const int64_t j = (int64_t)blockIdx.x * 4 + wave;
  if (j >= n) return;
  double s = 0.0;
  for (int64_t i = j + lane; i < n; i += 64) s = fma(tri_at(L, i, j), alpha[i], s);
#pragma unroll
  for (int off = 32; off > 0; off >>= 1) s += __shfl_down(s, off);
  if (lane == 0) t[j] = v[j] - s;
}

__global__ __launch_bounds__(256) void ut_tile_kernel(TriOperand U, const double* __restrict__ t, int64_t n,
                                                      double* __restrict__ part, int64_t ldp) {
  const int rt = blockIdx.x, ct = blockIdx.y;
  if (ct < rt) return;
  __shared__ double red[128];
  const int r = threadIdx.x & 127, h = threadIdx.x >> 7;
  const int64_t i = (int64_t)rt * 128 + r;
  const int64_t c0 = (int64_t)ct * 128 + h * 64;
  double s = 0.0;
  if (i < n)
    for (int k = 0; k < 64; ++k) {
      const int64_t c = c0 + k;
      if (c >= i && c < n) s = fma(tri_at(U, i, c), t[c], s);
    }
  if (h == 1) red[r] = s;
  __syncthreads();
  if (h == 0) part[(int64_t)ct * ldp + i] = s + red[r];
}

__global__ __launch_bounds__(256) void alpha_add_kernel(double* __restrict__ alpha, const double* __restrict__ part,
                                                        int64_t ldp, int np, int per_tile, int64_t n) {
  const int64_t i = (int64_t)blockIdx.x * 256 + threadIdx.x;
  if (i >= n) return;
  double s = 0.0;
  for (int p = per_tile ? (int)(i >> 7) : 0; p < np; ++p) s += part[(int64_t)p * ldp + i];
  alpha[i] += s;
}

}
```

gumbi_amd/engine.py:

```python

from __future__ import annotations

import ctypes as C
import os
from dataclasses import dataclass, field
from pathlib import Path

import numpy as np

__all__ = ["Engine", "KernelSpec", "GumbiHipError", "library_path", "load_library", "KERNEL_KINDS", "resolve_kernel_name",
           "PERIODIC_OFF", "PERIODIC_WARPED", "PERIODIC_PLAIN", "MAX_PERIODIC_DIMS",
           "ls_limits", "dist_plan", "GmbComm", "DistStep"]

GMB_MAX_DIMS, GMB_MAX_LIN, GMB_MAX_COREG, GMB_MAX_LEVELS = 16, 8, 4, 32
GMB_OK, GMB_EINVAL, GMB_ENOMEM, GMB_EHIP, GMB_ENOTPD, GMB_ENODEVICE = 0, -1, -2, -3, -4, -5
GMB_HOST, GMB_DEVICE = 0, 1

KERNEL_KINDS = {"ExpQuad": 0, "Matern52": 1, "Matern32": 2, "Matern12": 3, "Exponential": 4}


PERIODIC_OFF, PERIODIC_WARPED, PERIODIC_PLAIN = 0, 1, 2
MAX_PERIODIC_DIMS = GMB_MAX_DIMS // 2


# ... 98 lines not shown
class KernelSpec:

    D: int
    idx_cont: list
    kind: str | int = "ExpQuad"
    ard: bool = True
    idx_lin: list = field(default_factory=list)
    coreg: list = field(default_factory=list)
    out_col: int = -1
    n_out: int = 0
    hetero_noise: bool = True
    jitter: float = 1e-6
    additive: bool = False
    periodic: int = 0
    periods: list = field(default_factory=list)

    @property
    def kind_id(self) -> int:
        if isinstance(self.kind, str):
            if self.kind not in KERNEL_KINDS:
                raise ValueError(f"Continuous kernel must be one of {list(KERNEL_KINDS)}, got {self.kind!r}")
            return KERNEL_KINDS[self.kind]
        return int(self.kind)

    def as_dict(self) -> dict:
        return dict(D=int(self.D), kind=self.kind_id, ard=bool(self.ard),
                    idx_cont=[int(i) for i in self.idx_cont], idx_lin=[int(i) for i in self.idx_lin],
                    coreg=[(int(c), int(n)) for c, n in self.coreg], out_col=int(self.out_col),
                    n_out=int(self.n_out), hetero_noise=bool(self.hetero_noise), jitter=float(self.jitter),
                    additive=bool(self.additive), periodic=int(self.periodic), periods=[float(t) for t in self.periods])

    def theta_size(self) -> int:
        n = (len(self.idx_cont) if self.ard else 1) + 2
        if self.idx_lin:
            n += len(self.idx_lin) + 1
        n += sum(3 * L for _, L in self.coreg)
        if self.out_col >= 0:
            n += 3 * self.n_out * (2 if self.hetero_noise else 1)
        if self.additive:
            blk = (len(self.idx_cont) if self.ard else 1) + 1 + ((len(self.idx_lin) + 1) if self.idx_lin else 0)
            n += len(self.coreg) * blk
        return n

    def to_c(self) -> _Spec:
        if not 1 <= len(self.idx_cont) <= GMB_MAX_DIMS:
            raise ValueError(f"between 1 and {GMB_MAX_DIMS} continuous dimensions are supported")
        if len(self.idx_lin) > GMB_MAX_LIN:
            raise ValueError(f"at most {GMB_MAX_LIN} linear dimensions are supported")
        if len(self.coreg) > GMB_MAX_COREG:
            raise ValueError(f"at most {GMB_MAX_COREG} categorical dimensions are supported")
        if self.periodic:
            if self.periodic not in (PERIODIC_WARPED, PERIODIC_PLAIN):
                raise ValueError(f"periodic must be 0, 1 or 2, got {self.periodic!r}")
            if len(self.idx_cont) > MAX_PERIODIC_DIMS:
                raise ValueError(f"a periodic kernel supports at most {MAX_PERIODIC_DIMS} continuous dimensions")
            if len(self.periods) != len(self.idx_cont):
                raise ValueError(f"{len(self.periods)} periods for {len(self.idx_cont)} continuous dimensions")
        s = _Spec()
        s.kind, s.ard = self.kind_id, int(bool(self.ard))
        s.n_cont = len(self.idx_cont)
        for i, v in enumerate(self.idx_cont):
            s.idx_cont[i] = int(v)
        s.n_lin = len(self.idx_lin)
        for i, v in enumerate(self.idx_lin):
            s.idx_lin[i] = int(v)
        s.n_coreg = len(self.coreg)
        for i, (col, lev) in enumerate(self.coreg):
            s.coreg_col[i], s.coreg_levels[i] = int(col), int(lev)
        s.out_col, s.n_out = int(self.out_col), int(self.n_out)
        s.hetero_noise = int(bool(self.hetero_noise))
        s.additive = int(bool(self.additive))
        s.jitter = float(self.jitter)
        return s


_LIB = None
_DBL_P = C.POINTER(C.c_double)


def library_path() -> Path:
    override = os.environ.get("GUMBI_HIP_LIB")
    if override:
        return Path(override)
    return Path(__file__).resolve().parent / "lib" / "libgumbi_hip.so"


class GmbComm(C.Structure):

    ALL_GATHER = C.CFUNCTYPE(C.c_int32, C.c_void_p, C.c_void_p, C.c_void_p, C.c_int64, C.c_void_p)
    _fields_ = [("rank", C.c_int32), ("world", C.c_int32), ("ctx", C.c_void_p), ("all_gather", ALL_GATHER)]


class DistStep(C.Structure):

    _fields_ = [(n, C.c_int32) for n in ("op", "c0", "c1", "lo", "hi", "first", "count", "maxcount", "stream")] + [
        ("elems", C.c_int64)]
    OPS = ("KBUILD", "SQUARE", "PANEL", "UPDATE", "FORK", "JOIN", "SOLVE", "TAIL")

    def as_dict(self):
        d = {n: int(getattr(self, n)) for n, _ in self._fields_}
        d["op"] = self.OPS[d["op"]]
        return d


_SIGNATURES = {
    "gmb_abi_version": (C.c_int, []),
    "gmb_device_count": (C.c_int, []),
    "gmb_create": (C.c_int, [C.POINTER(C.c_void_p), C.c_int32, C.c_void_p]),
    "gmb_create_sibling": (C.c_int, [C.POINTER(C.c_void_p), C.c_void_p]),
    "gmb_destroy": (None, [C.c_void_p]),
    "gmb_last_error": (C.c_char_p, [C.c_void_p]),
    "gmb_stream": (C.c_void_p, [C.c_void_p]),
    "gmb_set_data": (C.c_int, [C.c_void_p, C.c_void_p, C.c_int64, C.c_int32, C.c_int64, C.c_void_p, C.c_int32]),
    "gmb_set_y": (C.c_int, [C.c_void_p, C.c_void_p, C.c_int32]),
    "gmb_set_kernel": (C.c_int, [C.c_void_p, C.POINTER(_Spec)]),
    "gmb_theta_size": (C.c_int, [C.POINTER(_Spec)]),
    "gmb_set_periodic": (C.c_int, [C.c_void_p, C.c_int32, _DBL_P, C.c_int32]),
    "gmb_set_theta": (C.c_int, [C.c_void_p, _DBL_P, C.c_int32]),
    "gmb_factorize": (C.c_int, [C.c_void_p]),
    "gmb_notpd_index": (C.c_int64, [C.c_void_p]),
    "gmb_factor_valid": (C.c_int, [C.c_void_p]),
    "gmb_nlml": (C.c_int, [C.c_void_p, _DBL_P, _DBL_P]),
    "gmb_evaluate": (C.c_int, [C.c_void_p, _DBL_P, C.c_int32, _DBL_P, _DBL_P]),
    "gmb_predict": (C.c_int, [C.c_void_p, C.c_void_p, C.c_int64, C.c_int64, C.c_int32, C.c_void_p,
                              C.c_void_p, C.c_int32]),
    "gmb_predict_joint": (C.c_int, [C.c_void_p, C.c_void_p, C.c_int64, C.c_int64, C.c_int32, C.c_double, C.c_void_p,
                                    C.c_void_p, C.c_int64, C.c_int32]),
    "gmb_draw_joint": (C.c_int, [C.c_void_p, C.c_void_p, C.c_int64, C.c_int64, C.c_int32, C.c_double, C.c_void_p, C.c_int64,
                                 C.c_int64, C.c_void_p, C.c_int64, C.c_void_p, C.c_int32]),
    "gmb_ls_limits": (C.c_int, [C.c_int32, _DBL_P, C.c_int64, C.c_int32, C.c_int64, C.c_int32, _DBL_P, _DBL_P]),
    "gmb_mfma_f64_peak": (C.c_int, [C.c_int32, _DBL_P, _DBL_P]),
    "gmb_mfma_f64_sustained": (C.c_int, [C.c_int32, C.c_double, _DBL_P, _DBL_P, _DBL_P, C.POINTER(C.c_int64)]),
    "gmb_set_profiling": (C.c_int, [C.c_void_p, C.c_int32]),
    "gmb_timings_get": (C.c_int, [C.c_void_p, C.POINTER(Timings)]),
    "gmb_copy_factor": (C.c_int, [C.c_void_p, C.c_int64, C.c_int64, C.c_int64, C.c_int64, _DBL_P]),
    "gmb_copy_v": (C.c_int, [C.c_void_p, _DBL_P]),
    "gmb_blk_potrf": (C.c_int, [C.c_void_p, C.c_void_p, C.c_int64, C.c_int32, C.c_void_p, C.c_void_p, C.c_void_p]),
    "gmb_copy_alpha": (C.c_int, [C.c_void_p, C.POINTER(C.c_double)]),
    "gmb_rccl_unique_id": (C.c_int, [C.c_char_p, C.c_void_p]),
    "gmb_rccl_comm_create": (C.c_int, [C.POINTER(C.POINTER(GmbComm)), C.c_char_p, C.c_void_p, C.c_int32, C.c_int32,
                                       C.c_int32]),
    "gmb_rccl_comm_destroy": (None, [C.POINTER(GmbComm)]),
    "gmb_rccl_comm_ranks": (C.c_int, [C.POINTER(GmbComm)]),
    "gmb_rccl_comm_split": (C.c_int, [C.POINTER(GmbComm)]),
    "gmb_rccl_last_error": (C.c_char_p, []),
    "gmb_dist_plan": (C.c_int64, [C.c_int64, C.c_int32, C.c_int32, C.c_int32, C.POINTER(DistStep), C.c_int64]),
    "gmb_dist_factorize": (C.c_int, [C.c_void_p, C.POINTER(GmbComm), C.c_int32]),
    "gmb_dist_nlml": (C.c_int, [C.c_void_p, C.POINTER(GmbComm), _DBL_P, _DBL_P]),
    "gmb_dist_predict": (C.c_int, [C.c_void_p, C.POINTER(GmbComm), C.c_void_p, C.c_int64, C.c_int64, C.c_int32,
                                   C.c_void_p, C.c_void_p, C.c_int32]),
    "gmb_debug_cov_grid": (C.c_int64, [C.c_int32] * 7 + [C.POINTER(C.c_int32), C.c_int64, C.POINTER(C.c_int64)]),
    "gmb_debug_tile_list": (C.c_int64, [C.c_int32] * 12 + [C.POINTER(C.c_int32), C.c_int64, C.POINTER(C.c_int32)]),
    "gmb_debug_chol_task": (C.c_int64, [C.c_int32, C.c_int32, C.c_int32, C.POINTER(C.c_int32), C.POINTER(C.c_int32)]),
    "gmb_chol_task_trace": (C.c_int64, [C.c_void_p, C.c_int32, C.c_void_p, C.c_int64]),
    "gmb_set_chol_scheme": (C.c_int, [C.c_void_p, C.c_int32]),
    "gmb_debug_assume_factored": (C.c_int, [C.c_void_p]),
    "gmb_set_eval_pairs": (C.c_int, [C.c_void_p, C.c_int32]),
    "gmb_set_predict_form": (C.c_int, [C.c_void_p, C.c_int32]),
    "gmb_reserve": (C.c_int, [C.c_void_p, C.c_int32, C.c_int64]),
    "gmb_set_grad_scheme": (C.c_int, [C.c_void_p, C.c_int32, C.c_int32]),
    "gmb_dist_set_mode": (C.c_int, [C.c_void_p, C.c_int32]),
    "gmb_resident_bytes": (C.c_int64, [C.c_void_p, C.c_int32]),
    "gmb_debug_eval_tasks": (C.c_int64, [C.c_int32, C.c_int32, C.c_int32, C.c_int32, C.POINTER(C.c_uint32), C.c_int64]),
    "gmb_debug_chol_lose_tickets": (C.c_int, [C.c_void_p, C.c_int32]),
    "gmb_blk_invert": (C.c_int, [C.c_void_p, C.c_void_p, C.c_int64, C.c_int32, C.c_void_p, C.c_void_p]),
    "gmb_blk_covariance": (C.c_int, [C.c_void_p, C.c_void_p, C.c_int64]),
    "gmb_blk_trsm": (C.c_int, [C.c_void_p, C.c_void_p, C.c_int64, C.c_int64, C.c_void_p, C.c_int64, C.c_void_p,
                               C.c_int32]),
    "gmb_blk_gemm_nt": (C.c_int, [C.c_void_p, C.c_void_p, C.c_int64, C.c_void_p, C.c_int64, C.c_void_p,
                                  C.c_int64, C.c_int64, C.c_int64, C.c_int64, C.c_double, C.c_double,
                                  C.c_int32, C.c_int64]),
}


def exported_symbols() -> list:
    return list(_SIGNATURES)


def _preload_hip_runtime():
    if os.environ.get("GUMBI_HIP_SYSTEM_RUNTIME") == "1":
        return
    try:
        import importlib.util

        spec = importlib.util.find_spec("torch")
        if spec is None or not spec.submodule_search_locations:
            return
        cand = Path(list(spec.submodule_search_locations)[0]) / "lib" / "libamdhip64.so"
        if cand.exists():
            C.CDLL(str(cand), mode=C.RTLD_GLOBAL)
    except OSError:
        pass


ABI_VERSION = 12


def load_library():
    global _LIB
    if _LIB is not None:
        return _LIB
    path = library_path()
    if not path.exists():
        raise GumbiHipError(
            f"{path} not found: the HIP engine is not built (run `python -c 'import __graft_entry__ as g; "
            f"g.build()'` or `make -C gumbi_amd/csrc`). gumbi_amd has no CPU fallback."
        )
    _preload_hip_runtime()
    lib = C.CDLL(str(path))
    for name, (restype, argtypes) in _SIGNATURES.items():
        fn = getattr(lib, name)
        fn.restype, fn.argtypes = restype, argtypes
    if lib.gmb_abi_version() != ABI_VERSION:
        raise GumbiHipError(f"{path} has ABI version {lib.gmb_abi_version()}, this binding needs {ABI_VERSION}: "
                            f"rebuild it (`python -m gumbi_amd.build`)")
    _LIB = lib
    return lib


def _ptr(arr):
    return arr.ctypes.data_as(C.c_void_p)


def _dptr(arr):
    return arr.ctypes.data_as(_DBL_P)


def device_count() -> int:
    n = load_library().gmb_device_count()
    return max(n, 0)


class Engine:

    host_blas_free = True

    def __init__(self, device: int = 0, stream: int | None = None, sibling_of: "Engine | None" = None):
        self._lib = load_library()
        self._h = C.c_void_p()
        self._peer = sibling_of
        if sibling_of is not None:
            rc = self._lib.gmb_create_sibling(C.byref(self._h), sibling_of._h)
        else:
            rc = self._lib.gmb_create(C.byref(self._h), int(device), C.c_void_p(stream) if stream else None)
        if rc == GMB_ENODEVICE:
            raise GumbiHipError("no HIP device visible: gumbi_amd needs an MI355X (gfx950); there is no CPU fallback")
        if rc != GMB_OK:
            raise GumbiHipError(f"gmb_create failed with status {rc}")
        self.spec = None
        self.N = 0
        self.D = 0

    def close(self):
        if getattr(self, "_h", None) and self._h.value:
            self._lib.gmb_destroy(self._h)
            self._h = C.c_void_p()

    def __del__(self):
        try:
            self.close()
        except Exception:
            pass

    def __enter__(self):
        return self

    def __exit__(self, *exc):
        self.close()

    def _check(self, rc, what):
        if rc == GMB_OK:
            return
        msg = self._lib.gmb_last_error(self._h)
        msg = msg.decode() if msg else ""
        if rc == GMB_EINVAL:
            raise ValueError(f"{what}: {msg}")
        if rc == GMB_ENOTPD:
            raise np.linalg.LinAlgError(f"{what}: {msg}")
        if rc == GMB_ENOMEM:
            raise MemoryError(f"{what}: {msg}")
        if rc == GMB_ENODEVICE:
            raise GumbiHipError(f"{what}: no HIP device (no CPU fallback exists)")
        raise GumbiHipError(f"{what}: status {rc}: {msg}")

    @property
    def stream(self) -> int:
        return int(self._lib.gmb_stream(self._h) or 0)

    def set_data(self, X, y):
        X = np.ascontiguousarray(X, dtype=np.float64)
        y = np.ascontiguousarray(y, dtype=np.float64)
        if X.ndim != 2 or y.ndim != 1 or X.shape[0] != y.shape[0]:
            raise ValueError(f"X must be (N, D) and y (N,), got {X.shape} and {y.shape}")
        self._check(self._lib.gmb_set_data(self._h, _ptr(X), X.shape[0], X.shape[1], X.shape[1], _ptr(y), GMB_HOST),
                    "gmb_set_data")
        self.N, self.D = X.shape

    def set_y(self, y):
        y = np.ascontiguousarray(y, dtype=np.float64)
        if y.shape != (self.N,):
            raise ValueError(f"y must be ({self.N},), got {y.shape}")
        self._check(self._lib.gmb_set_y(self._h, _ptr(y), GMB_HOST), "gmb_set_y")

    def set_data_device(self, x_ptr: int, N: int, D: int, ldx: int, y_ptr: int):
        self._check(self._lib.gmb_set_data(self._h, C.c_void_p(x_ptr), N, D, ldx, C.c_void_p(y_ptr), GMB_DEVICE),
                    "gmb_set_data")
        self.N, self.D = N, D

    def set_kernel(self, spec: KernelSpec):
        cs = spec.to_c()
        self._check(self._lib.gmb_set_kernel(self._h, C.byref(cs)), "gmb_set_kernel")
        if int(getattr(spec, "periodic", 0)) != 0:
            self.set_periodic(spec.periodic, spec.periods)
        self.spec = spec

    def set_periodic(self, mode: int, periods):
        periods = np.ascontiguousarray(periods, dtype=np.float64).ravel()
        self._check(self._lib.gmb_set_periodic(self._h, int(mode), _dptr(periods) if periods.size else None, periods.size),
                    "gmb_set_periodic")

    def set_theta(self, theta):
        theta = np.ascontiguousarray(theta, dtype=np.float64)
        self._check(self._lib.gmb_set_theta(self._h, _dptr(theta), theta.size), "gmb_set_theta")

    def factorize(self):
        self._check(self._lib.gmb_factorize(self._h), "gmb_factorize")

    def notpd_index(self) -> int:
        return int(self._lib.gmb_notpd_index(self._h))

    def factor_is_current(self) -> bool:
        return bool(self._lib.gmb_factor_valid(self._h))

    def nlml(self, grad: bool = False):
        val = C.c_double()
        if not grad:
            self._check(self._lib.gmb_nlml(self._h, C.byref(val), None), "gmb_nlml")
            return val.value
        g = np.empty(self.spec.theta_size(), dtype=np.float64)
        self._check(self._lib.gmb_nlml(self._h, C.byref(val), _dptr(g)), "gmb_nlml")
        return val.value, g

    def evaluate(self, theta, grad: bool = True):
        theta = np.ascontiguousarray(theta, dtype=np.float64)
        val = C.c_double()
        g = np.empty(self.spec.theta_size(), dtype=np.float64) if grad else None
        self._check(self._lib.gmb_evaluate(self._h, _dptr(theta), theta.size, C.byref(val), _dptr(g) if grad else None), "gmb_evaluate")
        return (val.value, g) if grad else val.value
# ... 59 lines not shown
    def timings(self) -> dict:
        t = Timings()
        self._check(self._lib.gmb_timings_get(self._h, C.byref(t)), "gmb_timings_get")
        return t.as_dict()

    CHOL_BY_SIZE, CHOL_RECURSION, CHOL_LOOKAHEAD, CHOL_TILES, CHOL_RECURSION_TILE_PANELS = -1, 0, 2, 3, 4

    def set_chol_scheme(self, scheme: int) -> int:
        prev = int(self._lib.gmb_set_chol_scheme(self._h, int(scheme)))
        if prev < 0:
            self._check(prev, "gmb_set_chol_scheme")
        return prev - 1

    GRAD_BY_SIZE, GRAD_LAUNCH_TREE, GRAD_TILES, GRAD_FUSED = -1, 0, 1, 2

    def set_grad_scheme(self, scheme: int, lag: int = -1) -> int:
        prev = int(self._lib.gmb_set_grad_scheme(self._h, int(scheme), int(lag)))
        if prev < 0:
            self._check(prev, "gmb_set_grad_scheme")
        return prev - 1

    def debug_lose_tickets(self, n: int):
        self._check(self._lib.gmb_debug_chol_lose_tickets(self._h, int(n)), "gmb_debug_chol_lose_tickets")

    def chol_task_trace(self, enable: int = -1):
        n = int(self._lib.gmb_chol_task_trace(self._h, int(enable), None, 0))
        if n <= 0:
            return None
        raw = np.zeros((n, 4), dtype=np.uint64)
        self._check(min(0, int(self._lib.gmb_chol_task_trace(self._h, -1, _ptr(raw), n))), "gmb_chol_task_trace")
        nct = (self.N + 127) // 128
        nrt = (self.N + 1 + 127) // 128
        tiles = np.array([chol_task(t, nct, nrt) for t in range(n)], dtype=np.int32)
        t0 = raw[raw > 0].min() if (raw > 0).any() else 0
        return tiles, (raw.astype(np.int64) - int(t0)) * 1e-8

    def eval_task_trace(self, with_chol: bool = True, lag: int = -1):
        n = int(self._lib.gmb_chol_task_trace(self._h, -1, None, 0))
        if n <= 0:
            return None
        nct = (self.N + 127) // 128
        nrt = (self.N + 1 + 127) // 128
        if lag < 0:
            lag = max(2, min(24, nct // 4))
        tasks = np.array(eval_task_list(nct, nrt, with_chol, lag), dtype=np.int32)
        if len(tasks) != n:
            return None
        raw = np.zeros((n, 4), dtype=np.uint64)
        self._check(min(0, int(self._lib.gmb_chol_task_trace(self._h, -1, _ptr(raw), n))), "gmb_chol_task_trace")
        t0 = raw[raw > 0].min() if (raw > 0).any() else 0
        return tasks, (raw.astype(np.int64) - int(t0)) * 1e-8

    def copy_factor(self, r0=0, nr=None, c0=0, nc=None):
        nr = self.N if nr is None else nr
        nc = self.N if nc is None else nc
        out = np.empty((nr, nc), dtype=np.float64)
        self._check(self._lib.gmb_copy_factor(self._h, r0, nr, c0, nc, _dptr(out)), "gmb_copy_factor")
        return out

    def copy_v(self):
        out = np.empty(self.N, dtype=np.float64)
        self._check(self._lib.gmb_copy_v(self._h, _dptr(out)), "gmb_copy_v")
        return out

    def copy_alpha(self):
        out = np.empty(self.N, dtype=np.float64)
        self._check(self._lib.gmb_copy_alpha(self._h, _dptr(out)), "gmb_copy_alpha")
        return out

    DIST_REPLICATED, DIST_CAPACITY = 0, 1

    def set_eval_pairs(self, mode: int) -> int:
        prev = int(self._lib.gmb_set_eval_pairs(self._h, int(mode)))
        if prev < 0:
            self._check(prev, "gmb_set_eval_pairs")
        return prev - 1

    def set_predict_form(self, form: int) -> int:
        prev = int(self._lib.gmb_set_predict_form(self._h, int(form)))
        if prev < 0:
            self._check(prev, "gmb_set_predict_form")
        return prev - 1

    def reserve(self, gradient: bool = True, M: int = 0):
        self._check(self._lib.gmb_reserve(self._h, int(bool(gradient)), int(M)), "gmb_reserve")

    def debug_assume_factored(self):
        self._check(self._lib.gmb_debug_assume_factored(self._h), "gmb_debug_assume_factored")

    def set_dist_mode(self, mode: int) -> int:
        prev = int(self._lib.gmb_dist_set_mode(self._h, int(mode)))
        if prev < 0:
            self._check(prev, "gmb_dist_set_mode")
        return prev

    def resident_bytes(self, peak: bool = False) -> int:
        return int(self._lib.gmb_resident_bytes(self._h, int(bool(peak))))

    def dist_factorize(self, comm, panel_blocks: int = 0):
        self._check(self._lib.gmb_dist_factorize(self._h, comm.handle, int(panel_blocks)), "gmb_dist_factorize")

    def dist_nlml(self, comm, grad: bool = False):
        val = C.c_double()
        if not grad:
            self._check(self._lib.gmb_dist_nlml(self._h, comm.handle, C.byref(val), None), "gmb_dist_nlml")
            return val.value
        g = np.empty(self.spec.theta_size(), dtype=np.float64)
        self._check(self._lib.gmb_dist_nlml(self._h, comm.handle, C.byref(val), _dptr(g)), "gmb_dist_nlml")
        return val.value, g

    def dist_predict(self, comm, Xs, with_noise=True):
        Xs = np.ascontiguousarray(Xs, dtype=np.float64)
        if Xs.ndim != 2 or Xs.shape[1] != self.D:
            raise ValueError(f"points_array must be (M, {self.D}), got {Xs.shape}")
        M = Xs.shape[0]
        mean = np.empty(M, dtype=np.float64)
        var = np.empty(M, dtype=np.float64)
        self._check(self._lib.gmb_dist_predict(self._h, comm.handle, _ptr(Xs), M, Xs.shape[1], int(bool(with_noise)),
                                               _ptr(mean), _ptr(var), GMB_HOST), "gmb_dist_predict")
        return mean, var

    def blk_potrf(self, a_ptr, lda, nvalid, dinv16_ptr, logdet_ptr=0, info_ptr=0):
        self._check(self._lib.gmb_blk_potrf(self._h, C.c_void_p(a_ptr), lda, nvalid,
                                            C.c_void_p(dinv16_ptr) if dinv16_ptr else None,
                                            C.c_void_p(logdet_ptr) if logdet_ptr else None,
                                            C.c_void_p(info_ptr) if info_ptr else None), "gmb_blk_potrf")

    def blk_invert(self, l_ptr, lda, nvalid, dinv16_ptr, inv_ptr):
        self._check(self._lib.gmb_blk_invert(self._h, C.c_void_p(l_ptr), lda, nvalid, C.c_void_p(dinv16_ptr),
                                             C.c_void_p(inv_ptr)), "gmb_blk_invert")

    def blk_covariance(self, out_ptr, ldo):
        self._check(self._lib.gmb_blk_covariance(self._h, C.c_void_p(out_ptr), ldo), "gmb_blk_covariance")

    def blk_trsm(self, b_ptr, ldb, nrows, l_ptr, ldl, dinv16_ptr, nvalid=128):
        self._check(self._lib.gmb_blk_trsm(self._h, C.c_void_p(b_ptr), ldb, nrows, C.c_void_p(l_ptr), ldl,
                                           C.c_void_p(dinv16_ptr), nvalid), "gmb_blk_trsm")

    def blk_gemm_nt(self, c_ptr, ldc, a_ptr, lda, b_ptr, ldb, m, n, k, alpha, beta, tri=0, tri_shift=0):
        self._check(self._lib.gmb_blk_gemm_nt(self._h, C.c_void_p(c_ptr), ldc, C.c_void_p(a_ptr), lda,
                                              C.c_void_p(b_ptr), ldb, m, n, k, alpha, beta, tri, tri_shift),
                    "gmb_blk_gemm_nt")


def chol_task(t: int, nct: int, nrt: int):
    lib = load_library()
    i, j = C.c_int32(), C.c_int32()
    n = lib.gmb_debug_chol_task(int(t), int(nct), int(nrt), C.byref(i), C.byref(j))
    if n < 0:
        raise ValueError("gmb_debug_chol_task: bad arguments")
    return i.value, j.value


def eval_task_list(nct: int, nrt: int, with_chol: bool = True, lag: int = 1, pairs: bool = False) -> list:
    lib = load_library()
    mode = int(bool(with_chol)) | (2 if pairs else 0)
    n = lib.gmb_debug_eval_tasks(int(nct), int(nrt), mode, int(lag), None, 0)
    if n < 0:
        raise ValueError("gmb_debug_eval_tasks: bad arguments")
    buf = (C.c_uint32 * n)()
    lib.gmb_debug_eval_tasks(int(nct), int(nrt), mode, int(lag), buf, n)
    return [(w >> 30, (w >> 15) & 0x7FFF, w & 0x7FFF) for w in buf]


def chol_task_count(nct: int, nrt: int) -> int:
    return int(load_library().gmb_debug_chol_task(-1, int(nct), int(nrt), None, None))


def gemm_tile_list(mt, nt, bm=128, bn=128, k=1024, tri=0, tri_off=0, nblk_stride=1, klo_n=0, khi_n=0, order=0, strip=0):
    lib = load_library()
    args = [int(v) for v in (mt, nt, bm, bn, k, tri, tri_off, nblk_stride, klo_n, khi_n, order, strip)]
    grid = C.c_int32()
    n = lib.gmb_debug_tile_list(*args, None, 0, C.byref(grid))
    if n < 0:
        raise ValueError("gmb_debug_tile_list: bad arguments")
    buf = (C.c_int32 * (3 * n))()
    lib.gmb_debug_tile_list(*args, buf, n, C.byref(grid))
    arr = np.frombuffer(buf, dtype=np.int32).reshape(n, 3)
    return int(grid.value), [tuple(int(v) for v in row) for row in arr]


def cov_grid(ti, tj, strip=1, tri_grid=1, row_first=0, row_stride=0, keep_order=1):
    lib = load_library()
    args = [int(v) for v in (ti, tj, strip, tri_grid, row_first, row_stride, keep_order)]
    grid = C.c_int64()
    n = lib.gmb_debug_cov_grid(*args, None, 0, C.byref(grid))
    if n < 0:
        raise ValueError("gmb_debug_cov_grid: bad arguments")
    buf = (C.c_int32 * max(3 * n, 1))()
    lib.gmb_debug_cov_grid(*args, buf, n, C.byref(grid))
    return int(grid.value), np.frombuffer(buf, dtype=np.int32)[: 3 * n].reshape(n, 3).copy()


def dist_plan(N: int, rank: int, world: int, panel_blocks: int = 0) -> list:
    lib = load_library()
    n = lib.gmb_dist_plan(int(N), int(rank), int(world), int(panel_blocks), None, 0)
    if n < 0:
        raise ValueError(f"gmb_dist_plan: bad arguments (N={N}, rank={rank}, world={world})")
    buf = (DistStep * n)()
    lib.gmb_dist_plan(int(N), int(rank), int(world), int(panel_blocks), buf, n)
    return [st.as_dict() for st in buf]


def ls_limits(X, ard: bool, device: int = 0):
    lib = load_library()
    X = np.ascontiguousarray(X, dtype=np.float64)
    n_groups = X.shape[1] if ard else 1
    lo = np.empty(n_groups)
    hi = np.empty(n_groups)
    rc = lib.gmb_ls_limits(int(device), _dptr(X), X.shape[0], X.shape[1], X.shape[1], int(bool(ard)), _dptr(lo),
                           _dptr(hi))
    if rc == GMB_ENODEVICE:
        raise GumbiHipError("gmb_ls_limits: no HIP device (no CPU fallback exists)")
    if rc != GMB_OK:
        raise GumbiHipError(f"gmb_ls_limits failed with status {rc}")
    return lo, hi


def mfma_f64_sustained(device: int = 0, seconds: float = 1.0) -> dict:
    mean, worst, mhz, n = C.c_double(), C.c_double(), C.c_double(), C.c_int64()
    rc = load_library().gmb_mfma_f64_sustained(int(device), float(seconds), C.byref(mean), C.byref(worst), C.byref(mhz),
                                                C.byref(n))
    if rc != GMB_OK:
        raise GumbiHipError(f"gmb_mfma_f64_sustained failed with status {rc}")
    return {"tflops_mean": mean.value, "tflops_min": worst.value, "shader_mhz": mhz.value, "launches": int(n.value),
            "seconds": float(seconds)}


def mfma_f64_peak(device: int = 0):
    out, cyc = C.c_double(), C.c_double()
    rc = load_library().gmb_mfma_f64_peak(int(device), C.byref(out), C.byref(cyc))
    if rc != GMB_OK:
        raise GumbiHipError(f"gmb_mfma_f64_peak failed with status {rc}")
    return out.value, cyc.value
```

include/gumbi_hip.h:

```cpp
#ifndef GUMBI_HIP_H
#define GUMBI_HIP_H

#include <stdint.h>

#ifdef __cplusplus
extern "C" {
#endif

#define GMB_ABI_VERSION 12
#define GMB_MAX_DIMS 16
#define GMB_MAX_LIN 8
#define GMB_MAX_COREG 4
#define GMB_MAX_LEVELS 32

typedef enum gmb_status {
  GMB_OK = 0,
  GMB_EINVAL = -1,
  GMB_ENOMEM = -2,
  GMB_EHIP = -3,
  GMB_ENOTPD = -4,
  GMB_ENODEVICE = -5
} gmb_status;

typedef enum gmb_kernel_kind {
  GMB_EXPQUAD = 0,
  GMB_MATERN52 = 1,
  GMB_MATERN32 = 2,
  GMB_MATERN12 = 3,
  GMB_EXPONENTIAL = 4
} gmb_kernel_kind;

typedef enum gmb_memspace { GMB_HOST = 0, GMB_DEVICE = 1 } gmb_memspace;

typedef struct gmb_kernel_spec {
  int32_t kind;
  int32_t ard;
  int32_t n_cont;
  int32_t idx_cont[GMB_MAX_DIMS];
  int32_t n_lin;
  int32_t idx_lin[GMB_MAX_LIN];
  int32_t n_coreg;
  int32_t coreg_col[GMB_MAX_COREG];
  int32_t coreg_levels[GMB_MAX_COREG];
  int32_t out_col;
  int32_t n_out;
  int32_t hetero_noise;
  int32_t additive;
  double jitter;
} gmb_kernel_spec;

typedef struct gmb_timings {
  double kbuild_ms;
  double chol_ms;
  double chol_gemm_ms;
  double chol_gemm_flops;
  int64_t chol_gemm_launches;
  double chol_leaf_ms;
  double chol_trsm_ms;
  double predict_ms;
  double predict_gemm_ms;
  double predict_gemm_flops;
  int64_t predict_gemm_launches;
  double grad_ms;
  double grad_gemm_ms;
  double grad_gemm_flops;
  double kbuild_bytes;
  double total_gemm_ms;
  double total_gemm_flops;
  int64_t total_gemm_launches;
  double total_kbuild_ms;
  double total_kbuild_bytes;
  int64_t total_kbuild_launches;
  double masked_gemm_ms;
  double masked_gemm_flops;
  int64_t masked_cus;
  double total_gemm_wall_ms;
  double total_chol_gemm_ms;
  double total_chol_gemm_flops;
  int64_t total_chol_gemm_launches;
  double total_chol_gemm_wall_ms;
  double total_chol_panel_gemm_ms;
  double total_chol_panel_gemm_flops;
  int64_t dist_world;
  int64_t dist_chol_collectives;
  double dist_chol_comm_bytes;
  double dist_chol_comm_ms;
  double dist_chol_comm_exposed_ms;
  double dist_chol_main_wait_ms;
  double dist_chol_bulk_wait_ms;
  int64_t dist_grad_collectives;
  double dist_grad_comm_bytes;
  double dist_grad_comm_ms;
  double dist_grad_comm_exposed_ms;
  int64_t dist_lockstep_repairs;
  double total_chol_tile_ms;
  double total_chol_tile_flops;
  int64_t total_chol_tile_launches;
  double total_eval_tile_ms;
  double total_eval_tile_flops;
  int64_t total_eval_tile_launches;
  double total_chol_update_all_ms;
  double total_chol_update_all_flops;
  int64_t total_chol_update_all_launches;
  int64_t predict_gemm_form;
  double total_chol_panel_tile_ms;
  double total_chol_panel_tile_flops;
  int64_t total_chol_panel_tile_launches;
} gmb_timings;

typedef struct gmb_engine gmb_engine;


int gmb_device_count(void);
int gmb_abi_version(void);

int gmb_create(gmb_engine** out, int32_t device, void* stream);
int gmb_create_sibling(gmb_engine** out, const gmb_engine* peer);
void gmb_destroy(gmb_engine* e);
const char* gmb_last_error(const gmb_engine* e);
void* gmb_stream(const gmb_engine* e);

int gmb_set_data(gmb_engine* e, const double* X, int64_t N, int32_t D, int64_t ldx,
                 const double* y, int32_t memspace);
int gmb_set_y(gmb_engine* e, const double* y, int32_t memspace);

int gmb_set_kernel(gmb_engine* e, const gmb_kernel_spec* spec);
int gmb_theta_size(const gmb_kernel_spec* spec);
int gmb_set_periodic(gmb_engine* e, int32_t mode, const double* periods, int32_t n);

int gmb_set_theta(gmb_engine* e, const double* theta, int32_t n);

int gmb_factorize(gmb_engine* e);
int64_t gmb_notpd_index(const gmb_engine* e);
int gmb_factor_valid(const gmb_engine* e);

int gmb_evaluate(gmb_engine* e, const double* theta, int32_t n, double* nlml, double* grad);
int gmb_nlml(gmb_engine* e, double* nlml, double* grad);

int gmb_predict(gmb_engine* e, const double* Xs, int64_t M, int64_t ldxs, int32_t with_noise,
                double* mean, double* var, int32_t memspace);

int gmb_predict_joint(gmb_engine* e, const double* Xs, int64_t M, int64_t ldxs, int32_t with_noise, double jitter,
                      double* mean, double* cov, int64_t ldc, int32_t memspace);

int gmb_draw_joint(gmb_engine* e, const double* Xs, int64_t M, int64_t ldxs, int32_t with_noise, double jitter,
                   const double* Z, int64_t S, int64_t ldz, double* Y, int64_t ldy, double* mean, int32_t memspace);

int gmb_ls_limits(int32_t device, const double* X, int64_t N, int32_t n_cols, int64_t ldx,
                  int32_t ard, double* lower, double* upper);

int gmb_set_profiling(gmb_engine* e, int32_t on);
int gmb_timings_get(const gmb_engine* e, gmb_timings* out);

int gmb_mfma_f64_peak(int32_t device, double* tflops, double* cycles_per_mfma);
int gmb_mfma_f64_sustained(int32_t device, double seconds, double* mean_tflops, double* min_tflops,
                           double* shader_mhz, int64_t* launches);

int gmb_copy_factor(const gmb_engine* e, int64_t r0, int64_t nr, int64_t c0, int64_t nc,
                    double* out);
int gmb_copy_v(const gmb_engine* e, double* out);
int gmb_copy_alpha(const gmb_engine* e, double* out);

int64_t gmb_debug_tile_list(int32_t mt, int32_t nt, int32_t bm, int32_t bn, int32_t k, int32_t tri,
                            int32_t tri_off, int32_t nblk_stride, int32_t klo_n, int32_t khi_n, int32_t order,
                            int32_t strip, int32_t* out, int64_t cap, int32_t* grid);
int64_t gmb_debug_cov_grid(int32_t ti, int32_t tj, int32_t strip, int32_t tri_grid, int32_t row_first,
                           int32_t row_stride, int32_t keep_order, int32_t* out, int64_t cap, int64_t* grid);
int64_t gmb_debug_chol_task(int32_t t, int32_t nct, int32_t nrt, int32_t* I, int32_t* J);
int64_t gmb_chol_task_trace(gmb_engine* e, int32_t enable, uint64_t* out, int64_t cap_tasks);
int gmb_debug_chol_lose_tickets(gmb_engine* e, int32_t n);
int gmb_debug_assume_factored(gmb_engine* e);
int gmb_set_chol_scheme(gmb_engine* e, int32_t scheme);
int gmb_set_grad_scheme(gmb_engine* e, int32_t scheme, int32_t lag);
int64_t gmb_debug_eval_tasks(int32_t nct, int32_t nrt, int32_t with_chol, int32_t lag, uint32_t* out, int64_t cap);
int gmb_set_eval_pairs(gmb_engine* e, int32_t mode);
int gmb_set_predict_form(gmb_engine* e, int32_t form);
int gmb_reserve(gmb_engine* e, int32_t gradient, int64_t M);
int gmb_blk_covariance(gmb_engine* e, double* out, int64_t ldo);
int gmb_blk_potrf(gmb_engine* e, double* Akk, int64_t lda, int32_t nvalid, double* dinv16,
                  double* logdet_accum, int32_t* info);
int gmb_blk_invert(gmb_engine* e, const double* Lkk, int64_t lda, int32_t nvalid,
                   const double* dinv16, double* invLkk);
int gmb_blk_trsm(gmb_engine* e, double* B, int64_t ldb, int64_t nrows, const double* Lkk,
                 int64_t ldl, const double* dinv16, int32_t nvalid);
int gmb_blk_gemm_nt(gmb_engine* e, double* C, int64_t ldc, const double* A, int64_t lda,
                    const double* B, int64_t ldb, int64_t m, int64_t n, int64_t k, double alpha,
                    double beta, int32_t tri, int64_t tri_shift);
typedef struct gmb_comm {
  int32_t rank, world;
  void* ctx;
  int32_t (*all_gather)(void* ctx, const void* send, void* recv, int64_t count, void* stream);
} gmb_comm;

int gmb_rccl_unique_id(const char* librccl_path, void* id128);
int gmb_rccl_comm_create(gmb_comm** out, const char* librccl_path, const void* id128, int32_t rank,
                         int32_t world, int32_t device);
void gmb_rccl_comm_destroy(gmb_comm* c);
int gmb_rccl_comm_ranks(const gmb_comm* c);
int gmb_rccl_comm_split(const gmb_comm* c);
const char* gmb_rccl_last_error(void);

typedef struct gmb_dist_step {
  int32_t op, c0, c1, lo, hi, first, count, maxcount, stream;
  int64_t elems;
} gmb_dist_step;
int64_t gmb_dist_plan(int64_t N, int32_t rank, int32_t world, int32_t panel_blocks, gmb_dist_step* out,
                      int64_t cap);

int gmb_dist_set_mode(gmb_engine* e, int32_t mode);
int64_t gmb_resident_bytes(const gmb_engine* e, int32_t peak);

int gmb_dist_factorize(gmb_engine* e, const gmb_comm* comm, int32_t panel_blocks);
int gmb_dist_nlml(gmb_engine* e, const gmb_comm* comm, double* nlml, double* grad);
int gmb_dist_predict(gmb_engine* e, const gmb_comm* comm, const double* Xs, int64_t M, int64_t ldxs,
                     int32_t with_noise, double* mean, double* var, int32_t memspace);

#ifdef __cplusplus
}
#endif
#endif
```

Measured before the change: 70580 GFLOP/s.

## Solve predict panels with tile kernel and fuse inverse transpose into GEMM store

Adds a panel triangular-solve form for prediction. When the training matrix has more blocks than the full tile scheme allows (N=50k gives about 390 blocks), the recursive column solve finishes panels of up to 16 block columns with a single dependency-tracked tile kernel, which replaces many small strip and GEMM launches. If a panel launch times out, the solve falls back to launches only. The inverse-tree GEMM also writes its transposed result directly through a new Ct pointer, which removes the separate transpose kernel but adds strided uncoalesced stores.

```diff
diff --git a/gumbi_amd/csrc/engine.hip b/gumbi_amd/csrc/engine.hip
--- a/gumbi_amd/csrc/engine.hip
+++ b/gumbi_amd/csrc/engine.hip
@@ -164,13 +164,10 @@
     int grid_x[2] = {0, 0};
     int count = 0;
     int64_t off[2] = {0, 0};
-    int64_t toff = 0;
-    int tr_rows = 0, tr_cols = 0;
     double flops[2] = {0.0, 0.0};
   };
   std::vector<InvLevelPlan> inv_plan;
   GemmArgs* dplan_gemm = nullptr;
-  TransposeJob* dplan_tr = nullptr;
   int64_t plan_N = -1, plan_ld = -1, plan_Np = -1;
   const double* plan_W = nullptr;
   const double* plan_A = nullptr;
@@ -200,6 +197,8 @@
   bool ct_trace = false;
   CholResult chol;
   bool tt_used = false;
+  bool tp_used = false;
+  bool solve_launches_only = false;
   int ct_lose = 0;
   bool fact_in_flight = false;
   struct HostLanding {
@@ -236,6 +235,8 @@
   int et_min_blocks = 1;
   int panel_tiles_w = 16;
   bool panel_tiles_veto = false;
+  int solve_panel_w = 16;
+  int solve_panel_max_ntm = 160;
   int tiles_min_blocks = 6, tiles_max_blocks = 224;
   int tiles_trsm_min_blocks = 16;
   int masked_max_blocks = 128;
@@ -1070,6 +1071,31 @@
   return GMB_OK;
 }
 
+int trsm_tiles_panel(gmb_engine* e, const FactorRef& f, double* V, int64_t ldv, int ntm, int c0, int c1, EvKind ev_kind) {
+  const int nct = c1 - c0;
+  const long long ntasks = (long long)ntm * nct;
+  if (ntasks <= 0) return GMB_OK;
+  const int64_t words = 4 + (int64_t)ntm * nct;
+  if (!*f.ct || *f.cap_ct < words) return fail(e, GMB_EINVAL, "internal: the panel solve's control block was not sized by its caller");
+  HIP_TRY(e, hipMemsetAsync(*f.ct, 0, sizeof(uint32_t), e->cur));
+  HIP_TRY(e, hipMemsetAsync(*f.ct + 2, 0, (size_t)(words - 2) * sizeof(uint32_t), e->cur));
+  CholTilesArgs a = tiles_args(f, c0, nct, nct, (int)ntasks, false);
+  a.V = V + (int64_t)c0 * TILE * ldv;
+  a.ldv = ldv;
+  a.ntm = ntm;
+  const bool last = c1 == (int)(f.Np / TILE);
+  double flops = 0.0;
+  for (int c = 0; c < nct; ++c)
+    flops += (double)ntm * (2.0 * TILE * TILE * TILE * c * (last && c == nct - 1 ? ragged_col_frac(f) : 1.0) + (double)TILE * TILE * TILE);
+  const int grid = (int)std::min<long long>(ntasks, e->wg_slots / 2);
+  ev_begin(e, ev_kind, flops, nct, ntm, nct * TILE, 0);
+  hipLaunchKernelGGL(trsm_tiles_kernel<8>, dim3(grid), dim3(512), 0, e->cur, a);
+  ev_end(e);
+  HIP_TRY(e, hipGetLastError());
+  e->tt_used = e->tp_used = true;
+  return GMB_OK;
+}
+
 int grad_workspace(gmb_engine* e);
 int64_t eval_tiles_words(int nct, int nrt) { return 4 + (int64_t)nrt * nct + 3 * (int64_t)nct + (int64_t)nct * nct + nct; }
 
@@ -1244,13 +1270,14 @@
 }
 
 int trsm_cols(gmb_engine* e, const FactorRef& f, double* V, int64_t ldz, int ntm, int c0, int c1, EvKind kind_gemm, EvKind kind_strip,
-              int lfirst = -1, int lstride = 0) {
+              int lfirst = -1, int lstride = 0, int panel_w = 0) {
+  if (panel_w >= 2 && lstride == 0 && c1 - c0 >= 2 && c1 - c0 <= panel_w) return trsm_tiles_panel(e, f, V, ldz, ntm, c0, c1, kind_gemm);
   if (c1 - c0 == 1)
     return launch_trsm_strip(e, V + (int64_t)c0 * TILE * ldz, ldz, (int64_t)ntm * TILE,
                              f.A + (int64_t)c0 * TILE * (f.ld + 1), f.ld, f.dinv16 + (int64_t)c0 * 8 * 256,
                              (int)std::min<int64_t>(TILE, f.N - (int64_t)c0 * TILE), kind_strip);
   const int mid = c0 + (c1 - c0 + 1) / 2;
-  int rc = trsm_cols(e, f, V, ldz, ntm, c0, mid, kind_gemm, kind_strip, lfirst, lstride);
+  int rc = trsm_cols(e, f, V, ldz, ntm, c0, mid, kind_gemm, kind_strip, lfirst, lstride, panel_w);
   if (rc) return rc;
   GemmArgs g{};
   g.C = V + (int64_t)mid * TILE * ldz;
@@ -1271,7 +1298,7 @@
   }
   rc = launch_gemm(e, g, kind_gemm);
   if (rc) return rc;
-  return trsm_cols(e, f, V, ldz, ntm, mid, c1, kind_gemm, kind_strip, lfirst, lstride);
+  return trsm_cols(e, f, V, ldz, ntm, mid, c1, kind_gemm, kind_strip, lfirst, lstride, panel_w);
 }
 
 int launch_transpose(gmb_engine* e, const double* src, int64_t lds_, double* dst, int64_t ldd, int rows,
@@ -1341,7 +1368,7 @@
   return GMB_OK;
 }
 
-void winv_node_products(gmb_engine* e, int c0, int c1, GemmArgs& gt, GemmArgs& gw, TransposeJob& tr) {
+void winv_node_products(gmb_engine* e, int c0, int c1, GemmArgs& gt, GemmArgs& gw) {
   const int64_t ldw = e->Np, lda = e->ld;
   double* W = e->dW;
   double* A = e->dA;
@@ -1375,10 +1402,8 @@
   gw.alpha = -1.0;
   gw.beta = 0.0;
   gw.nblk_stride = 1;
-  tr.src = W + (int64_t)mid * TILE + (int64_t)c0 * TILE * ldw;
-  tr.dst = A + (int64_t)c0 * TILE + (int64_t)mid * TILE * lda;
-  tr.rows = n2 * TILE;
-  tr.cols = n1 * TILE;
+  gw.Ct = A + (int64_t)c0 * TILE + (int64_t)mid * TILE * lda;
+  gw.ldct = lda;
 }
 
 int winv_node(gmb_engine* e, int c0, int c1, bool recurse) {
@@ -1390,11 +1415,9 @@
     if ((rc = winv_node(e, mid, c1, true))) return rc;
   }
   GemmArgs gt, gw;
-  TransposeJob tr;
-  winv_node_products(e, c0, c1, gt, gw, tr);
+  winv_node_products(e, c0, c1, gt, gw);
   if ((rc = launch_gemm(e, gt, EV_GRAD_GEMM))) return rc;
-  if ((rc = launch_gemm(e, gw, EV_GRAD_GEMM))) return rc;
-  return launch_transpose(e, tr.src, e->Np, tr.dst, e->ld, tr.rows, tr.cols);
+  return launch_gemm(e, gw, EV_GRAD_GEMM);
 }
 
 constexpr int MIN_BATCH_NODES = 4;
@@ -1403,7 +1426,6 @@
   if (e->plan_N == e->N && e->plan_ld == e->ld && e->plan_Np == e->Np && e->plan_W == e->dW && e->plan_A == e->dA)
     return GMB_OK;
   std::vector<GemmArgs> hg;
-  std::vector<TransposeJob> ht;
   e->inv_plan.assign(levels.size(), gmb_engine::InvLevelPlan{});
   static const int BMs[3] = {128, 64, 128}, BNs[3] = {128, 64, 64};
   static const double rate[3] = {73.0, 63.0, 65.0};
@@ -1416,16 +1438,11 @@
     gmb_engine::InvLevelPlan& lp = e->inv_plan[depth];
     lp.count = (int)nodes.size();
     std::vector<GemmArgs> gs[2];
-    lp.toff = (int64_t)ht.size();
     for (const InvNode& nd : nodes) {
       GemmArgs gt, gw;
-      TransposeJob tr;
-      winv_node_products(e, nd.c0, nd.c1, gt, gw, tr);
+      winv_node_products(e, nd.c0, nd.c1, gt, gw);
       gs[0].push_back(gt);
       gs[1].push_back(gw);
-      ht.push_back(tr);
-      lp.tr_rows = std::max(lp.tr_rows, tr.rows);
-      lp.tr_cols = std::max(lp.tr_cols, tr.cols);
     }
     for (int b = 0; b < 2; ++b) {
       long long nact = 0;
@@ -1455,15 +1472,11 @@
     }
   }
   if (e->dplan_gemm) (void)hipFree(e->dplan_gemm);
-  if (e->dplan_tr) (void)hipFree(e->dplan_tr);
   e->dplan_gemm = nullptr;
-  e->dplan_tr = nullptr;
   e->plan_N = -1;
   if (!hg.empty()) {
     HIP_TRY(e, hipMalloc((void**)&e->dplan_gemm, hg.size() * sizeof(GemmArgs)));
-    HIP_TRY(e, hipMalloc((void**)&e->dplan_tr, ht.size() * sizeof(TransposeJob)));
     HIP_TRY(e, hipMemcpy(e->dplan_gemm, hg.data(), hg.size() * sizeof(GemmArgs), hipMemcpyHostToDevice));
-    HIP_TRY(e, hipMemcpy(e->dplan_tr, ht.data(), ht.size() * sizeof(TransposeJob), hipMemcpyHostToDevice));
   }
   e->plan_N = e->N;
   e->plan_ld = e->ld;
@@ -1487,9 +1500,6 @@
     ev_end(e);
     HIP_TRY(e, hipGetLastError());
   }
-  hipLaunchKernelGGL(transpose_batched_kernel, dim3((lp.tr_rows + 31) / 32, (lp.tr_cols + 31) / 32, lp.count),
-                     dim3(256), 0, e->cur, e->dplan_tr + lp.toff, e->Np, e->ld);
-  HIP_TRY(e, hipGetLastError());
   return GMB_OK;
 }
 
@@ -2034,6 +2044,8 @@
   const char* mb = getenv("GMB_MASKED_MAX_BLOCKS");
   if (mb) e->masked_max_blocks = atoi(mb);
   if (const char* pw = getenv("GMB_PANEL_TILES_W")) e->panel_tiles_w = std::max(0, std::min(64, atoi(pw)));
+  if (const char* sw = getenv("GMB_SOLVE_PANEL_W")) e->solve_panel_w = std::max(0, std::min(64, atoi(sw)));
+  if (const char* sm = getenv("GMB_SOLVE_PANEL_MAX_NTM")) e->solve_panel_max_ntm = std::max(0, atoi(sm));
   const char* pc = getenv("GMB_PART_CUS");
   if (pc) part = atoi(pc);
 #endif
@@ -2101,7 +2113,7 @@
   if (e->stream) (void)hipStreamSynchronize(e->stream);
   for (int a = 0; a < 3; ++a)
     if (e->aux[a]) (void)hipStreamSynchronize(e->aux[a]);
-  void* ptrs[] = {e->dct, e->dct_trace, e->dstat, e->dDiagSave, e->dsend, e->drecv, e->dplan_gemm, e->dplan_tr, e->dDinv16, e->dX, e->dy, e->dA, e->xs, e->xl, e->cat, e->dtabs,
+  void* ptrs[] = {e->dct, e->dct_trace, e->dstat, e->dDiagSave, e->dsend, e->drecv, e->dplan_gemm, e->dDinv16, e->dX, e->dy, e->dA, e->xs, e->xl, e->cat, e->dtabs,
                   e->dnoise, e->dscal, e->dv, e->dV, e->dXs, e->txs, e->txl,
                   e->tcat, e->dkss, e->dpart, e->dmean, e->dvar, e->dW, e->dalpha, e->dgred, e->dgbig, e->det_tasks, e->dUdiag, e->dApart,
                   e->dAown, e->dPanel, e->dV2, e->dsend2, e->drecv2,
@@ -2574,15 +2586,55 @@
   return GMB_OK;
 }
 
-int predict_solve_v(gmb_engine* e, int64_t mpad, bool use_gemm_form) {
+enum SolveForm { SOLVE_LAUNCHES = 0, SOLVE_TILES = 1, SOLVE_PANELS = 2 };
+struct SolveKnobs {
+  int scheme = -1;
+  bool naive_leaf = false, veto = false, launches_only = false;
+  int w = 16, panel_max_ntm = 160, trsm_min_blocks = 16, tiles_max_blocks = 224;
+};
+SolveForm solve_form(const SolveKnobs& k, int nblocks, int ntm) {
+  const bool by_size = nblocks >= k.trsm_min_blocks && nblocks <= k.tiles_max_blocks && (ntm >= 32 || (long long)ntm * nblocks >= 576);
+  if (!k.naive_leaf && !k.launches_only && ntm <= 96 && (k.scheme == 3 || (k.scheme < 0 && by_size))) return SOLVE_TILES;
+  const bool panels_by_size = nblocks > k.tiles_max_blocks && ntm <= k.panel_max_ntm;
+  if (!k.naive_leaf && !k.veto && !k.launches_only && k.w >= 2 && nblocks >= 2 && (k.scheme == 4 || (k.scheme < 0 && panels_by_size)))
+    return SOLVE_PANELS;
+  return SOLVE_LAUNCHES;
+}
+void solve_panel_ranges(int c0, int c1, int w, std::vector<int>& out) {
+  if (c1 - c0 < 2) return;
+  if (c1 - c0 <= w) {
+    out.push_back(c0);
+    out.push_back(c1);
+    return;
+  }
+  const int mid = c0 + (c1 - c0 + 1) / 2;
+  solve_panel_ranges(c0, mid, w, out);
+  solve_panel_ranges(mid, c1, w, out);
+}
+bool solve_redo_on_launches(bool tp_used, bool launches_only, uint32_t abort_word) { return tp_used && !launches_only && abort_word != 0; }
+
+SolveKnobs solve_knobs(const gmb_engine* e) {
+  SolveKnobs k;
+  k.scheme = e->chol_scheme;
+  k.naive_leaf = e->naive_leaf;
+  k.veto = e->panel_tiles_veto;
+  k.launches_only = e->solve_launches_only;
+  k.w = e->solve_panel_w;
+  k.panel_max_ntm = e->solve_panel_max_ntm;
+  k.trsm_min_blocks = e->tiles_trsm_min_blocks;
+  k.tiles_max_blocks = e->tiles_max_blocks;
+  return k;
+}
+
+int predict_solve_v(gmb_engine* e, int64_t mpad, bool use_gemm_form, bool* redo = nullptr) {
   int rc;
   const int nblocks = (int)(e->Np / TILE);
   const int ntm = (int)(mpad / TILE);
-  const bool by_size = nblocks >= e->tiles_trsm_min_blocks && nblocks <= e->tiles_max_blocks &&
-                       (ntm >= 32 || (long long)ntm * nblocks >= 576);
-  const bool tiles = !e->naive_leaf && ntm <= 96 && (e->chol_scheme == 3 || (e->chol_scheme < 0 && by_size));
+  const SolveForm form = (e->solve_hook || use_gemm_form) ? SOLVE_LAUNCHES : solve_form(solve_knobs(e), nblocks, ntm);
+  const bool tiles = form == SOLVE_TILES;
   e->cur = e->stream;
-  e->tt_used = false;
+  e->tt_used = e->tp_used = false;
+  if (redo) *redo = false;
   if (e->solve_hook) {
     if ((rc = e->solve_hook(e->dV, mpad, (int)(mpad / TILE)))) return rc;
   } else if (use_gemm_form) {
@@ -2612,6 +2664,11 @@
     g.beta = 0.0;
     g.khi_n = 1;
     if ((rc = launch_gemm(e, g, EV_PREDICT_GEMM))) return rc;
+  } else if (form == SOLVE_PANELS) {
+    const int w = std::min(e->solve_panel_w, nblocks);
+    if ((rc = ensure(e, &e->dct, &e->cap_ct, 4 + (int64_t)ntm * w))) return rc;
+    HIP_TRY(e, hipMemsetAsync(e->dct, 0, 4 * sizeof(uint32_t), e->stream));
+    if ((rc = trsm_cols(e, train_factor(e), e->dV, mpad, ntm, 0, nblocks, EV_PREDICT_GEMM, EV_SOLVE_STRIP, -1, 0, w))) return rc;
   } else if ((rc = tiles ? trsm_tiles(e, train_factor(e), e->dV, mpad, (int)(mpad / TILE), EV_PREDICT_GEMM)
                          : trsm_cols(e, train_factor(e), e->dV, mpad, (int)(mpad / TILE), 0, nblocks, EV_PREDICT_GEMM, EV_SOLVE_STRIP)))
     return rc;
@@ -2619,9 +2676,27 @@
     uint32_t ab = 0;
     HIP_TRY(e, hipMemcpyAsync(&ab, e->dct + 1, sizeof(uint32_t), hipMemcpyDeviceToHost, e->stream));
     HIP_TRY(e, hipStreamSynchronize(e->stream));
+    if (redo && solve_redo_on_launches(e->tp_used, e->solve_launches_only, ab)) {
+      *redo = true;
+      return GMB_OK;
+    }
     if (ab != 0) return fail(e, GMB_EHIP, "tile triangular solve: a workgroup waited longer than its time-out for a tile (launch abandoned)");
   }
   return GMB_OK;
+}
+
+int predict_v(gmb_engine* e, const double* Xs, int64_t mc, int64_t mpad, int64_t ldxs, int32_t with_noise, hipMemcpyKind in_kind,
+              bool use_gemm_form) {
+  int rc;
+  bool redo = false;
+  if ((rc = predict_cross_cov(e, Xs, mc, mpad, ldxs, with_noise, in_kind))) return rc;
+  if ((rc = predict_solve_v(e, mpad, use_gemm_form, &redo)) || !redo) return rc;
+  fprintf(stderr, "libgumbi_hip: panel triangular solve abandoned after a time-out; solving again with launches only\n");
+  e->solve_launches_only = true;
+  rc = predict_cross_cov(e, Xs, mc, mpad, ldxs, with_noise, in_kind);
+  if (!rc) rc = predict_solve_v(e, mpad, use_gemm_form);
+  e->solve_launches_only = false;
+  return rc;
 }
 
 int predict_reduce(gmb_engine* e, int64_t mc, int64_t mpad, bool gemm_form) {
@@ -2701,8 +2776,7 @@
   JointState& jt = e->jt;
   const int64_t Mr = jt.Mr, Mp = jt.Mp;
   int rc;
-  if ((rc = predict_cross_cov(e, Xs, M, Mr, ldxs, with_noise, in_kind))) return rc;
-  if ((rc = predict_solve_v(e, Mr, gemm_form))) return rc;
+  if ((rc = predict_v(e, Xs, M, Mr, ldxs, with_noise, in_kind, gemm_form))) return rc;
   if ((rc = predict_reduce(e, M, Mr, gemm_form))) return rc;
   if (gemm_form && (rc = launch_transpose(e, e->dV2, e->Np, e->dV, Mr, (int)e->Np, (int)Mr))) return rc;
   if (e->Np > e->N)
@@ -2826,8 +2900,7 @@
   for (int64_t m0 = 0; m0 < M; m0 += Mt) {
     const int64_t mc = std::min<int64_t>(Mt, M - m0);
     const int64_t mpad = round_up(mc, TILE);
-    if ((rc = predict_cross_cov(e, Xs + m0 * ldxs, mc, mpad, ldxs, with_noise, in_kind))) return rc;
-    if ((rc = predict_solve_v(e, mpad, use_gemm_form))) return rc;
+    if ((rc = predict_v(e, Xs + m0 * ldxs, mc, mpad, ldxs, with_noise, in_kind, use_gemm_form))) return rc;
     if ((rc = predict_reduce(e, mc, mpad, use_gemm_form))) return rc;
     HIP_TRY(e, hipMemcpyAsync(mean + m0, e->dmean, mc * sizeof(double), out_kind, e->stream));
     HIP_TRY(e, hipMemcpyAsync(var + m0, e->dvar, mc * sizeof(double), out_kind, e->stream));
@@ -3169,6 +3242,22 @@
   return GMB_OK;
 }
 
+int64_t gmb_debug_solve_plan(int32_t nblocks, int32_t ntm, int32_t scheme, int32_t w, int32_t panels_ran, int32_t abort_word,
+                             int32_t* ranges, int64_t cap) {
+  if (nblocks < 1 || ntm < 1 || !chol_scheme_valid(scheme)) return GMB_EINVAL;
+  SolveKnobs k;
+  k.scheme = scheme;
+  if (w >= 0) k.w = w;
+  const SolveForm form = solve_form(k, nblocks, ntm);
+  std::vector<int> r;
+  if (form == SOLVE_PANELS) solve_panel_ranges(0, nblocks, std::min(k.w, nblocks), r);
+  for (size_t i = 0; i < r.size() && ranges && (int64_t)i < 2 * cap; ++i) ranges[i] = r[i];
+  const bool redo = solve_redo_on_launches(panels_ran != 0, false, (uint32_t)abort_word);
+  k.launches_only = true;
+  const bool second_is_launches = solve_form(k, nblocks, ntm) == SOLVE_LAUNCHES;
+  return (int64_t)form | (redo ? 4 : 0) | (second_is_launches ? 8 : 0) | ((int64_t)(r.size() / 2) << 8);
+}
+
 int gmb_set_chol_scheme(gmb_engine* e, int32_t scheme) {
   if (!e) return GMB_EINVAL;
   if (!chol_scheme_valid(scheme)) return fail(e, GMB_EINVAL, "Cholesky scheme %d: valid are -1 (by size), 0, 2, 3, 4", scheme);
diff --git a/gumbi_amd/csrc/gemm_f64.hpp b/gumbi_amd/csrc/gemm_f64.hpp
--- a/gumbi_amd/csrc/gemm_f64.hpp
+++ b/gumbi_amd/csrc/gemm_f64.hpp
@@ -33,6 +33,8 @@
   int32_t order;
   int32_t strip;
   int32_t xs_t0[8], xs_base[8];
+  double* Ct;
+  int64_t ldct;
 };
 
 __host__ __device__ __forceinline__ int xcd_remap(int bid, int nwg) {
@@ -141,6 +143,18 @@
   }
 }
 
+template <int WTM, int WTN>
+__device__ __forceinline__ void gemm_store_transposed(const GemmArgs& g, const int64_t n0, const int64_t m0, const d4 (&acc)[WTM][WTN]) {
+#pragma unroll
+  for (int j = 0; j < WTN; ++j) {
+    double* col = g.Ct + (n0 + j * 16) * g.ldct + m0;
+#pragma unroll
+    for (int i = 0; i < WTM; ++i)
+#pragma unroll
+      for (int r = 0; r < 4; ++r) col[i * 16 + 4 * r] = g.alpha * acc[i][j][r];
+  }
+}
+
 template <int WGM, int WGN, int WTM, int WTN, bool PFC = false>
 __device__ __forceinline__ void gemm_f64_body(const GemmArgs& g, const int vbid) {
   constexpr int NT = 64 * WGM * WGN;
@@ -274,6 +288,7 @@
 #pragma unroll
         for (int j = 0; j < WTN; ++j) row[j * 16] = g.alpha * acc[i][j][r];
       }
+    if (g.Ct) gemm_store_transposed<WTM, WTN>(g, Cg - g.C, m0, acc);
   } else {
 #pragma unroll
     for (int i = 0; i < WTM; ++i)
@@ -401,6 +416,7 @@
 #pragma unroll
         for (int j = 0; j < WTN; ++j) row[j * 16] = g.alpha * acc[i][j][r];
       }
+    if (g.Ct) gemm_store_transposed<WTM, WTN>(g, Cg - g.C, m0, acc);
   } else {
 #pragma unroll
     for (int i = 0; i < WTM; ++i)
diff --git a/gumbi_amd/csrc/gradient.hpp b/gumbi_amd/csrc/gradient.hpp
--- a/gumbi_amd/csrc/gradient.hpp
+++ b/gumbi_amd/csrc/gradient.hpp
@@ -679,25 +679,6 @@
   if (ph == 0) alpha_rows[row] = (part[0][r] + part[1][r]) + (part[2][r] + part[3][r]);
 }
 
-struct TransposeJob {
-  const double* src;
-  double* dst;
-  int32_t rows, cols;
-};
-__global__ __launch_bounds__(256) void transpose_batched_kernel(const TransposeJob* __restrict__ jobs, int64_t lds_,
-                                                                int64_t ldd) {
-  __shared__ double tile[32][33];
-  const TransposeJob jb = jobs[blockIdx.z];
-  const int r0 = blockIdx.x * 32, c0 = blockIdx.y * 32;
-  if (r0 >= jb.rows || c0 >= jb.cols) return;
-  const int tx = threadIdx.x & 31, ty = threadIdx.x >> 5;
-  for (int j = ty; j < 32; j += 8)
-    if (r0 + tx < jb.rows && c0 + j < jb.cols) tile[j][tx] = jb.src[(r0 + tx) + (int64_t)(c0 + j) * lds_];
-  __syncthreads();
-  for (int j = ty; j < 32; j += 8)
-    if (c0 + tx < jb.cols && r0 + j < jb.rows) jb.dst[(c0 + tx) + (int64_t)(r0 + j) * ldd] = tile[tx][j];
-}
-
 __global__ void reset_pad_cols_kernel(double* U, int64_t ld, int64_t n, int64_t npad) {
   const int64_t i = (int64_t)blockIdx.x * blockDim.x + threadIdx.x;
   if (i >= npad) return;
diff --git a/gumbi_amd/engine.py b/gumbi_amd/engine.py
--- a/gumbi_amd/engine.py
+++ b/gumbi_amd/engine.py
@@ -274,6 +274,7 @@
     "gmb_debug_cov_grid": (C.c_int64, [C.c_int32] * 7 + [C.POINTER(C.c_int32), C.c_int64, C.POINTER(C.c_int64)]),
     "gmb_debug_tile_list": (C.c_int64, [C.c_int32] * 12 + [C.POINTER(C.c_int32), C.c_int64, C.POINTER(C.c_int32)]),
     "gmb_debug_chol_task": (C.c_int64, [C.c_int32, C.c_int32, C.c_int32, C.POINTER(C.c_int32), C.POINTER(C.c_int32)]),
+    "gmb_debug_solve_plan": (C.c_int64, [C.c_int32, C.c_int32, C.c_int32, C.c_int32, C.c_int32, C.c_int32, C.POINTER(C.c_int32), C.c_int64]),
     "gmb_chol_task_trace": (C.c_int64, [C.c_void_p, C.c_int32, C.c_void_p, C.c_int64]),
     "gmb_set_chol_scheme": (C.c_int, [C.c_void_p, C.c_int32]),
     "gmb_debug_assume_factored": (C.c_int, [C.c_void_p]),
@@ -315,7 +316,7 @@
         pass
 
 
-ABI_VERSION = 12
+ABI_VERSION = 13
 
 
 def load_library():
@@ -681,6 +682,17 @@
     return i.value, j.value
 
 
+def solve_plan(nblocks: int, ntm: int, scheme: int = -1, w: int = -1, panels_ran: bool = False, abort_word: int = 0) -> dict:
+    cap = max(1, int(nblocks))
+    buf = (C.c_int32 * (2 * cap))()
+    r = int(load_library().gmb_debug_solve_plan(int(nblocks), int(ntm), int(scheme), int(w), int(bool(panels_ran)), int(abort_word), buf, cap))
+    if r < 0:
+        raise ValueError("gmb_debug_solve_plan: bad arguments")
+    n = r >> 8
+    return {"form": ("launches", "tiles", "panels")[r & 3], "panels": [(buf[2 * i], buf[2 * i + 1]) for i in range(n)],
+            "redo": bool(r & 4), "redo_on_launches": bool(r & 8)}
+
+
 def eval_task_list(nct: int, nrt: int, with_chol: bool = True, lag: int = 1, pairs: bool = False) -> list:
     lib = load_library()
     mode = int(bool(with_chol)) | (2 if pairs else 0)
diff --git a/include/gumbi_hip.h b/include/gumbi_hip.h
--- a/include/gumbi_hip.h
+++ b/include/gumbi_hip.h
@@ -7,7 +7,7 @@
 extern "C" {
 #endif
 
-#define GMB_ABI_VERSION 12
+#define GMB_ABI_VERSION 13
 #define GMB_MAX_DIMS 16
 #define GMB_MAX_LIN 8
 #define GMB_MAX_COREG 4
@@ -171,6 +171,8 @@
 int gmb_debug_chol_lose_tickets(gmb_engine* e, int32_t n);
 int gmb_debug_assume_factored(gmb_engine* e);
 int gmb_set_chol_scheme(gmb_engine* e, int32_t scheme);
+int64_t gmb_debug_solve_plan(int32_t nblocks, int32_t ntm, int32_t scheme, int32_t w, int32_t panels_ran, int32_t abort_word,
+                             int32_t* ranges, int64_t cap);
 int gmb_set_grad_scheme(gmb_engine* e, int32_t scheme, int32_t lag);
 int64_t gmb_debug_eval_tasks(int32_t nct, int32_t nrt, int32_t with_chol, int32_t lag, uint32_t* out, int64_t cap);
 int gmb_set_eval_pairs(gmb_engine* e, int32_t mode);
```

Result: no change. 70570 GFLOP/s, median of 2 (-0.0%).
